# insight-platform/Similari

Hardware: NVIDIA H100
Metric: pair_associations_per_sec (higher is better)
Workload: dtype f32

## Files before the change

### similari_b200/csrc/engine.cu

```cuda
#include <cuda_runtime.h>

#include <algorithm>
#include <array>
#include <chrono>
#include <cmath>
#include <cstddef>
#include <cstdlib>
#include <cstdio>
#include <cstring>
#include <map>
#include <string>
#include <type_traits>
#include <unordered_map>
#include <utility>
#include <vector>

#include "../../include/similari_b200.h"
#include "sb_blob.cuh"
#include "sb_engine.cuh"
#include "sb_host.cuh"
#include "sb_wstore.cuh"

#include <atomic>

namespace sb {
static std::atomic<unsigned long long> g_launches{0};
void note_launch(int n) { g_launches.fetch_add((unsigned long long)n, std::memory_order_relaxed); }
unsigned long long launch_count() { return g_launches.load(std::memory_order_relaxed); }
}

using sb::DBuf;
using sb::HBuf;
using sb::fail;

namespace {

enum ColRows { kRowTrack, kRowBlock, kRowFree, kRowWasted, kRowHistTop, kRowHistFree, kRowTrackHist };
enum ColBlob { kBlobNo, kBlobAll, kBlobTrackerOnly };
enum ColTag { kTagNone, kTagFblk, kTagHblk, kTagObsN, kTagObsPhys, kTagOwner, kTagFree };
struct Col {
  DBuf* buf;
  void (*point)(sb200_tracker&, void*);
  size_t w;
  bool zero = false;
  int rows = kRowTrack;
  int blob = kBlobAll;
  int tag = kTagNone;
};

int make_params(const sb200_options& o, sb::Params* out) {
  sb::Params p;
  memset(&p, 0, sizeof(p));
  if (o.kind < 0 || o.kind > 3) return fail(SB200_ERR_INVALID, "unknown tracker kind %d", o.kind);
  if (o.positional_kind != SB200_POS_MAHA && o.positional_kind != SB200_POS_IOU)
    return fail(SB200_ERR_INVALID, "unknown positional metric %d", o.positional_kind);
  p.kind = o.kind;
  p.positional_kind = o.positional_kind;
  p.visual_kind = o.visual_kind;
  p.iou_threshold = o.iou_threshold;
  p.min_confidence = o.min_confidence;
  p.pos_weight = o.kalman_position_weight;
  p.vel_weight = o.kalman_velocity_weight;
  p.max_idle_epochs = o.max_idle_epochs;
  if (o.max_idle_epochs < 0) return fail(SB200_ERR_INVALID, "max_idle_epochs must be >= 0");
  if (o.n_constraints < 0 || o.n_constraints > SB200_MAX_CONSTRAINTS)
    return fail(SB200_ERR_INVALID, "at most %d spatio-temporal constraints", SB200_MAX_CONSTRAINTS);
  std::vector<std::pair<int, float>> c;
  for (int i = 0; i < o.n_constraints; ++i) {
    if (!(o.constraint_max_dist[i] > 0.0f))
      return fail(SB200_ERR_INVALID, "The distance is expected to be a positive float");
    c.emplace_back(o.constraint_epochs[i], o.constraint_max_dist[i]);
  }
  std::stable_sort(c.begin(), c.end(), [](const std::pair<int, float>& a, const std::pair<int, float>& b) { return a.first < b.first; });
  c.erase(std::unique(c.begin(), c.end(), [](const std::pair<int, float>& a, const std::pair<int, float>& b) { return a.first == b.first; }), c.end());
  p.n_constraints = (int)c.size();
  for (size_t i = 0; i < c.size(); ++i) { p.constraint_epochs[i] = c[i].first; p.constraint_max_dist[i] = c[i].second; }
  p.is_visual = o.kind == SB200_KIND_VISUAL_SORT || o.kind == SB200_KIND_BATCH_VISUAL_SORT;
  p.is_batch = o.kind == SB200_KIND_BATCH_SORT || o.kind == SB200_KIND_BATCH_VISUAL_SORT;
  if (p.is_visual) {
    if (o.visual_kind != SB200_VIS_EUCLIDEAN && o.visual_kind != SB200_VIS_COSINE)
      return fail(SB200_ERR_INVALID, "unknown visual metric %d", o.visual_kind);
    if (o.feature_dim <= 0) return fail(SB200_ERR_INVALID, "feature_dim must be > 0 for visual trackers");
    if (o.visual_max_observations < 1 || o.visual_max_observations > sb::kMaxObsWide)
      return fail(SB200_ERR_CAPACITY, "visual_max_observations must be in [1, %d]", sb::kMaxObsWide);
    p.visual_threshold = o.visual_threshold;
    p.feature_dim = o.feature_dim;
    p.d8 = (o.feature_dim + 7) / 8 * 8;
    p.vis_rel_err = sb::screen_rel_err(o.feature_dim);
    p.vis_rel_err8 = sb::screen_rel_err_fp8(o.feature_dim);
    p.max_obs = o.visual_max_observations;
    p.min_votes = o.visual_min_votes;
    p.min_track_length = o.visual_minimal_track_length;
    p.min_area = o.visual_minimal_area;
    p.min_quality_use = o.visual_minimal_quality_use;
    p.min_quality_collect = o.visual_minimal_quality_collect;
    p.min_own_use = o.visual_minimal_own_area_percentage_use;
    p.min_own_collect = o.visual_minimal_own_area_percentage_collect;
    p.use_own_area = (o.visual_minimal_own_area_percentage_collect + o.visual_minimal_own_area_percentage_use) > 0.0f;
  } else {
    p.max_obs = 1;
    p.d8 = 8;
  }
  *out = p;
  return 0;
}

}

struct sb200_tracker {
  sb200_options opts{};
  sb::Params P{};
  int device = 0;
  cudaStream_t stream = nullptr;
  cudaStream_t user_stream = nullptr;
  bool has_user_stream = false;
  bool join_per_call = true;
  cudaEvent_t ev_join_req = nullptr;
  cudaEvent_t ev_user_in = nullptr, ev_user_out = nullptr;
  cudaStream_t prep_stream = nullptr;
  cudaEvent_t ev_prep_done = nullptr, ev_set_free[2]{}, ev_inputs = nullptr;
  cudaEvent_t ev_cost_done = nullptr;
  bool cost_done_valid = false;
  bool set_busy[2]{};
  unsigned long long frame_seq = 0;
  float kernel_ms[2]{};
  bool tc_timed = false;
  cudaStream_t copy_stream = nullptr;
  static constexpr int kDepth = 3;
  struct FrameBack {
    sb::FrameDyn dyn;
    int dense_scenes;
    int hpool[2];
    int screen[3];
  };
  static_assert(offsetof(FrameBack, dense_scenes) == sizeof(sb::FrameDyn) && sizeof(FrameBack) == sizeof(sb::FrameDyn) + 24,
                "FrameBack: FrameDyn followed by the counters, without padding");
  static size_t back_offset(int n_scenes) { return ((size_t)n_scenes * 16 + 15) / 16 * 16; }
  struct Pending {
    bool active = false;
    int n_scenes = 0, total = 0;
    std::vector<int> slots, m;
    long long live_ub = 0;
    HBuf h_req;
    HBuf h_out;
    FrameBack* back() const { return reinterpret_cast<FrameBack*>(h_out.as<char>() + back_offset(n_scenes)); }
    cudaEvent_t done = nullptr;
    cudaEvent_t ev[6]{}, ev_k[3]{}, ev_pos[2]{};
    bool tc_timed = false, pos_forked = false;
    int mode = 0;
    bool fp8 = false;
  } pend[kDepth];
  int pend_head = 0, pend_count = 0;
  std::vector<int> pending_add;
  long long inflight_live_ub = 0;
  int async_rc = 0;
  std::string async_err;
  unsigned long long acc_units_mn = 0, acc_units_rows = 0, acc_frames = 0;
  double host_ms_total = 0.0, host_ms_blocked = 0.0;
  unsigned long long host_calls = 0;
  double acc_stage_ms[5]{}, acc_kernel_ms[2]{};
  unsigned long long acc_tc_frames = 0;
  static constexpr int kFp8Hold = 64;
  int fp8_hold = 0;
  unsigned long long acc_screen[4] = {0, 0, 0, 0};
  cudaStream_t side_stream = nullptr;
  cudaEvent_t ev_fork[2]{}, ev_join = nullptr;
  float stage_ms[5]{};
  std::unordered_map<uint64_t, int> slot_of;
  std::vector<uint64_t> scene_of_slot;
  std::vector<uint32_t> epoch;
  std::vector<int> n_tracks;
  std::vector<int> n_hidden;
  std::vector<int> arena_top;
  std::vector<uint64_t> last_req_scenes;
  std::vector<int> last_req_slots;
  int64_t revealed = 0;
  int scene_cap = 0, track_cap = 0;
  DBuf b_idc;
  int auto_waste_counter = 100, auto_waste_periodicity = 100;
  int64_t wasted_count = 0;
  sb::TrackStore ts{};
  DBuf b_id, b_epoch, b_length, b_custom, b_vt, b_pred, b_obs, b_radius, b_kst, b_vert, b_hpred, b_hobs, b_feat, b_feat_bf16, b_fnorm2, b_obs_phys,
      b_feat_fp8, b_fscale, b_obs_hasf, b_obs_q, b_obs_n, b_feat_cnt, b_fblk, b_blk_owner, b_blk_free;
  DBuf b_ntracks, b_cur_epoch, b_scene_ids, b_nfree, b_atop;
  sb::WastedBuf wb{};
  DBuf w_count, w_id, w_scene, w_epoch, w_length, w_pred, w_obs, w_hpred, w_hobs;
  int hist_len = 1;
  bool fhist_on = false;
  DBuf b_hblk, b_hrows, b_hpresent, b_hfree, b_hpool, w_hblk, f_histdst;
  long long hpool_cap = 0;
  long long hpool_top = 0;
  long long hpool_free = 0;
  long long hpool_pend = 0;
  enum InColumn { kBoxes, kFeat, kHasf, kQuality, kCustom, kOwn, kInCols };
  using InPtrs = std::array<const void*, kInCols>;
  InPtrs in_ptrs(const void* boxes, const void* feat, const void* hasf, const void* quality, const void* custom,
                 const void* own) const {
    if (!P.is_visual) return {boxes, nullptr, nullptr, nullptr, custom, nullptr};
    return {boxes, feat, feat ? hasf : nullptr, quality, custom, own};
  }
  template <auto F> static void to_frame(sb::Frame& f, const void* p) { f.*F = static_cast<std::remove_reference_t<decltype(f.*F)>>(const_cast<void*>(p)); }
  struct InCol { void (*bind)(sb::Frame&, const void*); size_t w; const char* name; };
  std::array<InCol, kInCols> in_cols() const {
    using F = sb::Frame;
    return {{{to_frame<&F::in_boxes>, 24, "S.boxes"}, {to_frame<&F::in_feat>, (size_t)P.feature_dim * feat_bytes(), "S.feat"},
             {to_frame<&F::in_hasf>, 1, "S.hasf"}, {to_frame<&F::in_quality>, 4, "S.quality"},
             {to_frame<&F::in_custom>, 8, "S.custom"}, {to_frame<&F::in_own>, 4, "S.own"}}};
  }
  static constexpr int kOutCols = 6;
  struct OutCol { void* host; void (*bind)(sb::Frame&, const void*); size_t w; const char* name; };
  static std::array<OutCol, kOutCols> out_cols(const sb200_predict_out& o) {
    using F = sb::Frame;
    return {{{o.ids, to_frame<&F::o_ids>, 8, "o_ids"}, {o.epochs, to_frame<&F::o_epochs>, 4, "o_epochs"},
             {o.lengths, to_frame<&F::o_lengths>, 4, "o_lengths"}, {o.voting_types, to_frame<&F::o_vt>, 1, "o_vt"},
             {o.predicted_boxes, to_frame<&F::o_pred>, 24, "o_pred"}, {o.observed_boxes, to_frame<&F::o_obs>, 24, "o_obs"}}};
  }
  long long hint_dets(int n_scenes) const { return (long long)std::max(opts.max_scenes_hint, n_scenes) * opts.max_dets_per_scene_hint; }
  size_t frame_rows(int total, int n_scenes) const { return (size_t)std::max<long long>(std::max(total, 1), hint_dets(n_scenes)); }
  int hint_tracks() const { return opts.max_tracks_per_scene_hint > 0 ? track_cap : 0; }
  struct Staging {
    DBuf col[kInCols];
    InPtrs key{};
    int total = -1;
    int type = sb::kFeatF32;
    bool pending = false;
    cudaEvent_t ev = nullptr;
    cudaEvent_t ev0 = nullptr;
    cudaEvent_t ev_read = nullptr;
    bool read_pending = false;
  } stg[2];
  int stg_last = 1;
  struct CandBufs { DBuf box, radius, conf, vert, flags, norm2, bf16, decided, fp8, scale; } cand[2];
  DBuf f_winner, f_cvt, f_pos, f_vis, f_scenes, f_newcount,
      f_status, f_featdst, f_apprank, f_appmeta, f_frameout, f_excl, f_prewin, f_own, f_ownovf, f_dyn, f_ws, f_tmeta, f_rowinfo, f_slabc, f_slabm, f_slabmask,
      f_dscene, f_maxc, f_maxcval, f_drowb, f_dcolb, f_slabk, f_scene_max, f_tiles, f_pairs, f_colmeta, f_colgeo, f_colb, f_colvalid, f_rowmeta, f_poslist, f_counters, f_visval, f_colsb;
  int num_sms = 132;
  DBuf o_col[kOutCols];
  HBuf h_small;
  bool adapt_dense = false;
  unsigned long long acc_dense_scenes = 0;
  int last_dense_scenes = 0;
  bool seen_features = false;
  int feat_type = sb::kFeatF32;
  size_t feat_bytes() const { return feat_type == sb::kFeatF32 ? 4 : 2; }
  bool transferred = false;
  int last_n_scenes = 0;

  ~sb200_tracker() {
    cudaSetDevice(device);
    for (cudaStream_t s : {stream, prep_stream, side_stream, copy_stream}) if (s) cudaStreamSynchronize(s);
    for (auto& g : stg)
      for (cudaEvent_t e : {g.ev, g.ev0, g.ev_read}) if (e) cudaEventDestroy(e);
    for (auto& q : pend) {
      if (q.done) cudaEventDestroy(q.done);
      for (auto& e : q.ev) if (e) cudaEventDestroy(e);
      for (auto& e : q.ev_k) if (e) cudaEventDestroy(e);
      for (auto& e : q.ev_pos) if (e) cudaEventDestroy(e);
    }
    if (copy_stream) cudaStreamDestroy(copy_stream);
    if (side_stream) cudaStreamDestroy(side_stream);
    if (prep_stream) cudaStreamDestroy(prep_stream);
    for (cudaEvent_t e : {ev_user_in, ev_user_out, ev_prep_done, ev_set_free[0], ev_set_free[1], ev_inputs, ev_join_req, ev_cost_done}) if (e) cudaEventDestroy(e);
    for (auto& e : ev_fork) if (e) cudaEventDestroy(e);
    if (ev_join) cudaEventDestroy(ev_join);
    if (stream) cudaStreamDestroy(stream);
  }

  template <auto F> static void in_ts(sb200_tracker& t, void* p) { t.ts.*F = static_cast<std::remove_reference_t<decltype(t.ts.*F)>>(p); }
  template <auto F> static void in_wb(sb200_tracker& t, void* p) { t.wb.*F = static_cast<std::remove_reference_t<decltype(t.wb.*F)>>(p); }

  std::vector<Col> store_table() {
    using TS = sb::TrackStore;
    const size_t K = (size_t)P.max_obs, d8 = (size_t)P.d8, H = (size_t)hist_len;
    std::vector<Col> c = {{&b_id, in_ts<&TS::id>, 8}, {&b_epoch, in_ts<&TS::epoch>, 4}, {&b_length, in_ts<&TS::length>, 4},
                          {&b_custom, in_ts<&TS::custom>, 8}, {&b_vt, in_ts<&TS::vt>, 1}, {&b_pred, in_ts<&TS::pred>, 24},
                          {&b_obs, in_ts<&TS::obs>, 24}, {&b_radius, in_ts<&TS::radius>, 4},
                          {&b_kst, in_ts<&TS::kst>, 4 * (size_t)sb::kStateStride}};
    if (P.positional_kind == SB200_POS_IOU) c.push_back({&b_vert, in_ts<&TS::vert>, 64});
    if (H > 1) {
      c.push_back({&b_hpred, in_ts<&TS::hist_pred>, 24 * H, true});
      c.push_back({&b_hobs, in_ts<&TS::hist_obs>, 24 * H, true});
    }
    if (P.is_visual) {
      c.push_back({&b_obs_phys, in_ts<&TS::obs_phys>, K, false, kRowTrack, kBlobAll, kTagObsPhys});
      c.push_back({&b_obs_hasf, in_ts<&TS::obs_hasf>, K});
      c.push_back({&b_obs_q, in_ts<&TS::obs_q>, 4 * K});
      c.push_back({&b_obs_n, in_ts<&TS::obs_n>, 1, false, kRowTrack, kBlobAll, kTagObsN});
      c.push_back({&b_feat_cnt, in_ts<&TS::feat_cnt>, 1});
      c.push_back({&b_fblk, in_ts<&TS::fblk>, 4, false, kRowTrack, kBlobAll, kTagFblk});
      if (fhist_on) c.push_back({&b_hblk, in_ts<&TS::hblk>, 4, false, kRowTrack, kBlobTrackerOnly, kTagHblk});
      c.push_back({&b_feat, in_ts<&TS::feat>, 4 * K * d8, true, kRowBlock});
      c.push_back({&b_feat_bf16, in_ts<&TS::feat_bf16>, 2 * K * d8, true, kRowBlock});
      c.push_back({&b_fnorm2, in_ts<&TS::fnorm2>, 4 * K, false, kRowBlock});
      if (P.d8 <= sb::kFp8MaxD8) {
        c.push_back({&b_feat_fp8, in_ts<&TS::feat_fp8>, K * sb::fp8_pitch(P.d8), false, kRowBlock, kBlobNo});
        c.push_back({&b_fscale, in_ts<&TS::fscale>, 4 * K, false, kRowBlock, kBlobNo});
      }
      c.push_back({&b_blk_owner, in_ts<&TS::blk_owner>, 4, false, kRowBlock, kBlobAll, kTagOwner});
      c.push_back({&b_blk_free, in_ts<&TS::blk_free>, 4, false, kRowFree, kBlobAll, kTagFree});
    }
    return c;
  }

  std::vector<Col> slot_table() {
    using TS = sb::TrackStore;
    return {{&b_ntracks, nullptr, 4, true}, {&b_cur_epoch, nullptr, 4, true}, {&b_scene_ids, nullptr, 8, true},
            {&b_nfree, in_ts<&TS::n_free>, 4, true}, {&b_atop, in_ts<&TS::arena_top>, 4, true}};
  }

  std::vector<Col> wasted_table() {
    using WB = sb::WastedBuf;
    const size_t H = (size_t)hist_len;
    std::vector<Col> c = {{&w_id, in_wb<&WB::id>, 8, false, kRowWasted}, {&w_scene, in_wb<&WB::scene>, 8, false, kRowWasted},
                          {&w_epoch, in_wb<&WB::epoch>, 4, false, kRowWasted}, {&w_length, in_wb<&WB::length>, 4, false, kRowWasted},
                          {&w_pred, in_wb<&WB::pred>, 24, false, kRowWasted}, {&w_obs, in_wb<&WB::obs>, 24, false, kRowWasted}};
    if (H > 1) {
      c.push_back({&w_hpred, in_wb<&WB::hist_pred>, 24 * H, false, kRowWasted});
      c.push_back({&w_hobs, in_wb<&WB::hist_obs>, 24 * H, false, kRowWasted});
    }
    if (fhist_on) c.push_back({&w_hblk, in_wb<&WB::hblk>, 4, false, kRowWasted, kBlobAll, kTagHblk});
    return c;
  }

  std::vector<Col> pool_table() {
    using TS = sb::TrackStore;
    const size_t H = (size_t)hist_len;
    return {{&b_hrows, in_ts<&TS::hrows>, H * (size_t)P.d8 * 4, false, kRowHistTop},
            {&b_hpresent, in_ts<&TS::hpresent>, H, true, kRowHistTop},
            {&b_hfree, in_ts<&TS::hfree>, 4, false, kRowHistFree, kBlobAll, kTagHblk}};
  }

  int regrow(DBuf& b, size_t w, size_t groups, size_t rows, size_t old_groups, size_t old_rows, bool zero) {
    const size_t bytes = std::max<size_t>(1, groups * rows * w);
    DBuf nb;
    int rc = nb.ensure(bytes);
    if (rc) return rc;
    if (zero) CU(cudaMemsetAsync(nb.p, 0, bytes, stream));
    if (b.p && old_groups > 0 && old_rows > 0) {
      if (old_groups == 1)
        CU(cudaMemcpyAsync(nb.p, b.p, old_rows * w, cudaMemcpyDeviceToDevice, stream));
      else
        CU(cudaMemcpy2DAsync(nb.p, rows * w, b.p, old_rows * w, old_rows * w, old_groups, cudaMemcpyDeviceToDevice, stream));
      CU(cudaStreamSynchronize(stream));
    }
    b = std::move(nb);
    return 0;
  }

  int grow(const std::vector<Col>& cols, size_t groups, size_t rows, size_t old_groups, size_t old_rows) {
    for (const Col& c : cols) {
      const int rc = regrow(*c.buf, c.w, groups, rows, old_groups, old_rows, c.zero || c.blob != kBlobNo);
      if (rc) return rc;
      if (c.point) c.point(*this, c.buf->p);
    }
    return 0;
  }

  int regen_fp8(int slot, int top) {
    if (!ts.feat_fp8 || top <= 0) return 0;
    const long long r0 = (long long)slot * track_cap * P.max_obs, rows = (long long)top * P.max_obs;
    sb::launch_to_fp8(ts.feat + r0 * P.d8, P.d8, P.d8, P.d8, rows, ts.feat_fp8 + r0 * sb::fp8_pitch(P.d8), ts.fscale + r0, stream);
    return cudaGetLastError() == cudaSuccess ? 0 : fail(SB200_ERR_CUDA, "e4m3 row conversion failed");
  }

  static constexpr long long kBf16LogCap = 1 << 18;
  DBuf b_bf16log;
  long long bf16_log_n = 0;
  bool bf16_stale_all = false;
  int regen_bf16() {
    if (bf16_stale_all) sb::launch_bf16_regen(ts, P.d8, P.max_obs, nullptr, 0, scene_cap, stream);
    else if (bf16_log_n > 0) sb::launch_bf16_regen(ts, P.d8, P.max_obs, b_bf16log.as<int>(), bf16_log_n, 0, stream);
    else return 0;
    bf16_log_n = 0;
    bf16_stale_all = false;
    return cudaGetLastError() == cudaSuccess ? 0 : fail(SB200_ERR_CUDA, "BF16 row conversion failed");
  }

  int ensure_store(int need_scenes, int need_tracks) {
    if (need_scenes <= scene_cap && need_tracks <= track_cap) return 0;
    int ns = scene_cap, nt = track_cap;
    if (need_scenes > ns) ns = std::max(need_scenes, std::max(4, ns * 2));
    if (need_tracks > nt) nt = std::max(need_tracks, std::max(64, nt * 2));
    int rc = regen_bf16();
    if (rc) return rc;
    rc = grow(store_table(), ns, nt, scene_cap, track_cap);
    if (rc) return rc;
    if (ns != scene_cap && (rc = grow(slot_table(), ns, 1, scene_cap, 1))) return rc;
    ts.kst_stride = sb::kStateStride;
    if (hist_len > 1) ts.hist_len = hist_len;
    scene_cap = ns;
    track_cap = nt;
    ts.track_cap = nt;
    return 0;
  }

  int slot_for(uint64_t scene_id, bool create) {
    auto it = slot_of.find(scene_id);
    if (it != slot_of.end()) return it->second;
    if (!create) return -1;
    int s = (int)scene_of_slot.size();
    slot_of[scene_id] = s;
    scene_of_slot.push_back(scene_id);
    epoch.push_back(0);
    n_tracks.push_back(0);
    n_hidden.push_back(0);
    arena_top.push_back(0);
    pending_add.push_back(0);
    return s;
  }

  int ensure_wasted(int64_t need) {
    if (need <= wb.cap) return 0;
    int64_t ncap = std::max<int64_t>(need, std::max<int64_t>(1024, (int64_t)wb.cap * 3));
    int rc = grow(wasted_table(), 1, (size_t)ncap, 1, (size_t)wasted_count);
    if (rc) return rc;
    if (!w_count.p) {
      if ((rc = w_count.ensure(sizeof(int)))) return rc;
      CU(cudaMemsetAsync(w_count.p, 0, sizeof(int), stream));
    }
    wb.cap = (int)ncap;
    wb.count = w_count.as<int>();
    return 0;
  }

  int run_waste() {
    int n_slots = (int)scene_of_slot.size();
    if (n_slots == 0) return 0;
    int64_t active = 0;
    int max_n = 0;
    for (int v : n_tracks) { active += v; max_n = std::max(max_n, v); }
    if (active == 0) {
      revealed = wasted_count;
      std::fill(n_hidden.begin(), n_hidden.end(), 0);
      return 0;
    }
    int rc = ensure_wasted(wasted_count + active);
    if (rc) return rc;
    if ((rc = h_small.ensure((size_t)n_slots * 16))) return rc;
    unsigned int* he = h_small.as<unsigned int>();
    for (int s = 0; s < n_slots; ++s) he[s] = epoch[s];
    CU(cudaMemcpyAsync(b_cur_epoch.p, he, sizeof(unsigned int) * n_slots, cudaMemcpyHostToDevice, stream));
    CU(cudaStreamSynchronize(stream));
    unsigned long long* hs = h_small.as<unsigned long long>();
    for (int s = 0; s < n_slots; ++s) hs[s] = scene_of_slot[s];
    CU(cudaMemcpyAsync(b_scene_ids.p, hs, sizeof(unsigned long long) * n_slots, cudaMemcpyHostToDevice, stream));
    sb::launch_waste(P, ts, n_slots, b_cur_epoch.as<unsigned int>(), b_scene_ids.as<unsigned long long>(),
                     b_ntracks.as<int>(), wb, max_n, stream);
    CU(cudaGetLastError());
    int* hn = h_small.as<int>();
    CU(cudaStreamSynchronize(stream));
    CU(cudaMemcpyAsync(hn, b_ntracks.p, sizeof(int) * n_slots, cudaMemcpyDeviceToHost, stream));
    int hc = 0;
    CU(cudaMemcpyAsync(&hc, w_count.p, sizeof(int), cudaMemcpyDeviceToHost, stream));
    CU(cudaStreamSynchronize(stream));
    for (int s = 0; s < n_slots; ++s) n_tracks[s] = hn[s];
    wasted_count = hc;
    revealed = wasted_count;
    std::fill(n_hidden.begin(), n_hidden.end(), 0);
    return 0;
  }

  int drop_wasted_front(int64_t n) {
    if (n <= 0 || !w_count.p) return 0;
    n = std::min(n, wasted_count);
    const int64_t rest = wasted_count - n;
    cudaStream_t st = stream;
    int rc = 0;
    if (fhist_on) {
// ... 33 lines not shown
    int rc = grow(pool_table(), 1, (size_t)ncap, 1, (size_t)hpool_top);
    if (rc) return rc;
    hpool_cap = ncap;
    return 0;
  }

  int set_feature_history(bool on) {
    if (on == fhist_on) return 0;
    CU(cudaSetDevice(device));
    CU(cudaStreamSynchronize(stream));
    fhist_on = true;
    const int rc = on ? add_feature_history() : 0;
    if (on && rc == 0) return 0;
    std::vector<Col> cols = pool_table();
    for (const Col& c : store_table()) if (c.tag == kTagHblk) cols.push_back(c);
    for (const Col& c : wasted_table()) if (c.tag == kTagHblk) cols.push_back(c);
    for (const Col& c : cols) { c.buf->release(); c.point(*this, nullptr); }
    b_hpool.release();
    f_histdst.release();
    ts.hpool = nullptr;
    ts.fhist_len = 0;
    fhist_on = false;
    hpool_cap = hpool_top = hpool_free = hpool_pend = 0;
    return rc;
  }
  int add_feature_history() {
    int rc;
    if ((rc = b_hpool.ensure(2 * sizeof(int)))) return rc;
    CU(cudaMemsetAsync(b_hpool.p, 0, 2 * sizeof(int), stream));
    for (const Col& c : store_table())
      if (c.tag == kTagHblk && scene_cap > 0 && (rc = grow({c}, scene_cap, track_cap, 0, 0))) return rc;
    for (const Col& c : wasted_table())
      if (c.tag == kTagHblk && wb.cap > 0 && (rc = grow({c}, 1, wb.cap, 0, 0))) return rc;
    CU(cudaStreamSynchronize(stream));
    ts.hpool = b_hpool.as<int>();
    ts.fhist_len = hist_len;
    return 0;
  }

  int predict(int32_t n_scenes, const uint64_t* scene_ids, const int32_t* det_offsets, const float* boxes,
              const float* features, const uint8_t* has_feature, const float* quality, const int64_t* custom_ids,
              const float* own_area, const sb200_predict_out* out, bool device_io, bool wait);
  int absorb_oldest(bool block);
  int poll();
  int drain(const char* why = nullptr);
  int ens(DBuf& b, size_t need, const char* name = "") {
    if (need <= b.bytes) return 0;
    static const bool trace_ens = getenv("SB200_TRACE") != nullptr;
    if (trace_ens) fprintf(stderr, "[sb200] %s grows: %zu -> %zu bytes\n", name, b.bytes, need);
    int rc = drain("frame buffer grows");
    if (rc) return rc;
    return b.ensure(need);
  }
  template <class T> int ens(DBuf& b, size_t need, T*& to, const char* name) {
    const int rc = ens(b, need, name);
    if (rc == 0) to = static_cast<T*>(b.p);
    return rc;
  }
  static constexpr int kDenseVoteCap = 8192;

  struct Request {
    int n_scenes = 0, total = 0;
    const uint64_t* scene_ids = nullptr;
    const int32_t* det_offsets = nullptr;
    InPtrs in{};
    sb200_predict_out out{};
    bool device_io = false, same_req = false;
  };
  struct FramePlan {
    std::vector<int> m_of, nb_ub;
    int max_m = 0, max_n = 0, max_nb = 0, need_tracks = 0;
    long long live_ub = 0, pos_total = 0, vis_total = 0, col_total = 0, work = 0;
    long long pos_ub = 0, posl_total = 0, visl_total = 0;
    size_t T = 0;
    int cset = 0, vote_cap = 0, mstep = 0, cstep = 256;
    bool want_tc = false, want_dense = false, want_fp8 = false;
    Staging* sin = nullptr;
    bool prefetched = false, fork = false, derive_own = false;
  };
  void unbook(Pending& q) {
    for (int s = 0; s < q.n_scenes; ++s) pending_add[q.slots[s]] -= q.m[s];
    inflight_live_ub -= q.live_ub;
    if (fhist_on) hpool_pend -= q.total;
    q.active = false;
    pend_count -= 1;
  }
  struct Rollback { sb200_tracker* t; Pending* q; bool armed; ~Rollback() { if (armed) t->unbook(*q); } };
  int check_request(Request& rq) {
    const int n_scenes = rq.n_scenes;
    const uint64_t* scene_ids = rq.scene_ids;
    const int32_t* det_offsets = rq.det_offsets;
    if (n_scenes < 0) return fail(SB200_ERR_INVALID, "n_scenes must be >= 0");
    if (n_scenes > 0 && (!scene_ids || !det_offsets)) return fail(SB200_ERR_INVALID, "scene_ids / det_offsets are NULL");
    rq.total = n_scenes > 0 ? det_offsets[n_scenes] : 0;
    if (n_scenes > 0 && det_offsets[0] != 0) return fail(SB200_ERR_INVALID, "det_offsets[0] must be 0");
    for (int s = 0; s < n_scenes; ++s)
      if (det_offsets[s + 1] < det_offsets[s]) return fail(SB200_ERR_INVALID, "det_offsets must be non-decreasing");
    if (rq.total > 0 && !rq.in[kBoxes]) return fail(SB200_ERR_INVALID, "boxes is NULL");
    int rc = 0;
    poll();
    if (async_rc) { if ((rc = drain("error of an earlier frame"))) return rc; }
    rq.same_req = (int)last_req_scenes.size() == n_scenes && n_scenes > 0 &&
                memcmp(last_req_scenes.data(), scene_ids, sizeof(uint64_t) * (size_t)n_scenes) == 0;
    if (!rq.same_req && n_scenes > 0) {
      std::unordered_map<uint64_t, int> seen;
      for (int s = 0; s < n_scenes; ++s)
        if (!seen.emplace(scene_ids[s], s).second) return fail(SB200_ERR_INVALID, "scene %llu appears twice in one request", (unsigned long long)scene_ids[s]);
    }
    int max_m0 = 0, max_n0 = 0;
    auto fits = [&] {
      max_m0 = max_n0 = 0;
      for (int s = 0; s < n_scenes; ++s) {
        int slot = -1;
        if (rq.same_req) slot = last_req_slots[s];
        else { auto it = slot_of.find(scene_ids[s]); if (it != slot_of.end()) slot = it->second; }
        max_m0 = std::max(max_m0, det_offsets[s + 1] - det_offsets[s]);
        max_n0 = std::max(max_n0, slot >= 0 ? n_tracks[slot] + pending_add[slot] : 0);
      }
      return sb::voting_smem_need(max_m0, max_n0, P.is_visual ? kDenseVoteCap : 0) <= sb::kVotingSmemLimit;
    };
    bool ok = fits();
    if (!ok && pend_count > 0) { if ((rc = drain("assignment solver bound"))) return rc; ok = fits(); }
    if (!ok) return fail(SB200_ERR_CAPACITY, "scene too large for the on-chip assignment solver (m=%d, n=%d)", max_m0, max_n0);
    return 0;
  }

  void bounds(const Request& rq, FramePlan& pl) const {
    const int n_scenes = rq.n_scenes, K = P.max_obs;
    pl.m_of.resize(n_scenes);
    pl.nb_ub.resize(n_scenes);
    pl.max_m = pl.max_n = pl.max_nb = pl.need_tracks = 0;
    pl.live_ub = pl.pos_total = pl.vis_total = pl.col_total = pl.work = 0;
    for (int s = 0; s < n_scenes; ++s) {
      const int slot = last_req_slots[s];
      const int m = rq.det_offsets[s + 1] - rq.det_offsets[s];
      const int n = n_tracks[slot] + pending_add[slot];
      pl.m_of[s] = m;
      pl.nb_ub[s] = P.is_visual ? arena_top[slot] + pending_add[slot] : 0;
      pl.live_ub += n;
      pl.pos_total += (long long)m * n;
      if (P.is_visual) pl.vis_total += (long long)m * n * K;
      pl.col_total += ((long long)pl.nb_ub[s] * K + 127) / 128 * 128;
      pl.work += (long long)m * n * K;
      pl.max_m = std::max(pl.max_m, m);
      pl.max_n = std::max(pl.max_n, n);
      pl.max_nb = std::max(pl.max_nb, pl.nb_ub[s]);
      pl.need_tracks = std::max(pl.need_tracks, n + m);
    }
  }

  int reserve_state(const Request& rq, FramePlan& pl) {
    const int n_scenes = rq.n_scenes, total = rq.total;
    int rc = 0;
    bounds(rq, pl);
    const int pipe_room = kDepth * std::max(pl.max_m, opts.max_dets_per_scene_hint);
    int hint_s = std::max((int)scene_of_slot.size(), opts.max_scenes_hint);
    if (hint_s > scene_cap || pl.need_tracks > track_cap) {
      if ((rc = drain("track store bound"))) return rc;
      bounds(rq, pl);
      const int want_t = std::max(pl.need_tracks, opts.max_tracks_per_scene_hint) + pipe_room;
      if (hint_s > scene_cap || pl.need_tracks > track_cap)
        if ((rc = ensure_store(hint_s, std::max(want_t, track_cap + track_cap / 2)))) return rc;
    }
    if (wasted_count + inflight_live_ub + pl.live_ub + 1 > wb.cap) {
      const long long pipe_need = inflight_live_ub + pl.live_ub;
      if ((rc = drain("wasted buffer bound"))) return rc;
      bounds(rq, pl);
      const long long dets = std::max<long long>(total, hint_dets(n_scenes));
      const long long ring_need = (long long)(kDepth + 1) * (pl.live_ub + (long long)kDepth * dets);
      const long long rec_bytes = 72 + (hist_len > 1 ? 48ll * hist_len : 0);
      const long long base_need = std::max<long long>(ring_need, 2 * pipe_need);
      const long long mult = std::max<long long>(1, std::min<long long>(8, (2ll << 30) / std::max<long long>(1, base_need * rec_bytes)));
      if ((rc = ensure_wasted(2 * wasted_count + mult * base_need + 1))) return rc;
    }
    if (fhist_on && total > 0 && hpool_top + std::max<long long>(0, hpool_pend + total - hpool_free) > hpool_cap) {
      const long long frames = pend_count + 1;
      if ((rc = drain("feature history pool bound"))) return rc;
      const long long want = hpool_top + std::max<long long>(0, frames * total - hpool_free);
      if (want > hpool_cap && (rc = ensure_hpool(std::max<long long>(want, hpool_cap + hpool_cap / 2)))) return rc;
    }
    if (!b_idc.p) {
      if ((rc = b_idc.ensure(8))) return rc;
      CU(cudaMemsetAsync(b_idc.p, 0, 8, stream));
    }
    return 0;
  }

  int plan_frame(const Request& rq, Pending& q, FramePlan& pl) {
    const int n_scenes = rq.n_scenes, total = rq.total, K = P.max_obs;
    int rc = 0;
    if ((rc = q.h_req.ensure(sizeof(sb::SceneReq) * (size_t)n_scenes)) ||
        (rc = q.h_out.ensure(back_offset(n_scenes) + sizeof(FrameBack))))
      return rc;
    if (P.is_visual && rq.in[kFeat] != nullptr && total > 0) {
      const sb::VisKernel vk = sb::vis_kernel_env();
      const bool selective = sb::vis_selective(P.visual_kind == SB200_VIS_EUCLIDEAN, P.visual_threshold);
      const bool big = sb::vis_tc_worth(P.d8, pl.work);
      const bool dense_ok = P.n_constraints == 0;
      pl.want_dense = big && dense_ok && (!selective || adapt_dense);
      pl.want_tc = selective && big && !pl.want_dense;
      if (vk == sb::kVisSimt) { pl.want_tc = false; pl.want_dense = false; }
      else if (vk == sb::kVisTc || vk == sb::kVisTc8 || vk == sb::kVisTc16) { pl.want_tc = pl.work > 0; pl.want_dense = false; }
      else if (vk == sb::kVisDense) { pl.want_dense = pl.work > 0 && dense_ok; pl.want_tc = pl.work > 0 && !pl.want_dense; }
      const bool can8 = pl.want_tc && P.d8 <= sb::kFp8MaxD8 && ts.feat_fp8 != nullptr;
      const bool forced = vk == sb::kVisTc8 || vk == sb::kVisTc16;
      pl.want_fp8 = can8 && (forced ? vk == sb::kVisTc8 : fp8_hold == 0);
      if (!forced && can8 && fp8_hold > 0) fp8_hold -= 1;
    }
    pl.vote_cap = pl.want_dense ? kDenseVoteCap : sb::kVoteVisCap;
    sb::SceneReq* hreq = q.h_req.as<sb::SceneReq>();
    for (int s = 0; s < n_scenes; ++s) {
      sb::SceneReq& r = hreq[s];
      r.slot = last_req_slots[s];
      r.m = pl.m_of[s];
      r.det_base = rq.det_offsets[s];
      r.epoch = epoch[r.slot] + 1;
      r.scene_id = rq.scene_ids[s];
      r.pos_lbase = (int)pl.posl_total;
      r.pos_lcap = sb::pos_lcap(r.m);
      pl.posl_total += r.pos_lcap;
      r.vis_lbase = (int)pl.visl_total;
      r.vis_lcap = P.is_visual ? sb::vis_lcap(r.m, pl.vote_cap) : 0;
      pl.visl_total += r.vis_lcap;
    }
    pl.T = frame_rows(total, n_scenes);
    pl.pos_ub = pl.pos_total;
    const long long hint_pos = hint_dets(n_scenes) * hint_tracks();
    pl.pos_total = std::max(pl.pos_total, hint_pos);
    if (P.is_visual) pl.vis_total = std::max(pl.vis_total, hint_pos * K);
    pl.cset = (int)(frame_seq & 1);
    if (!pl.want_tc && !pl.want_dense) return 0;
    pl.mstep = 256;
    pl.cstep = pl.want_dense ? (256 / K) * K : sb::vis_screen_ucols(P.d8, num_sms, n_scenes, pl.m_of.data(), pl.nb_ub.data(), K);
    return 0;
  }

#define ENS(b, ...) ens(b, __VA_ARGS__, #b)
  int bind_frame(const Request& rq, FramePlan& pl, sb::Frame& f, sb::TcArgs& tc) {
    const int n_scenes = rq.n_scenes, total = rq.total, K = P.max_obs;
    const size_t T = pl.T;
    CandBufs& cb = cand[pl.cset];
    int rc = 0;
    if ((rc = ENS(cb.box, T * 24, f.c_box)) || (rc = ENS(cb.radius, T * 4, f.c_radius)) || (rc = ENS(cb.conf, T * 4, f.c_conf)) ||
        (rc = ENS(f_winner, T * 4, f.winner)) || (rc = ENS(f_cvt, T, f.c_vt)) ||
        (rc = ENS(f_scenes, sizeof(sb::SceneDesc) * n_scenes, f.scenes)) || (rc = ENS(f_newcount, 4 * (size_t)n_scenes, f.new_count)) ||
        (rc = ENS(f_dyn, sizeof(sb::FrameDyn), f.dyn)) || (rc = ENS(f_apprank, T * 8, f.app_rank)) ||
        (rc = ENS(f_appmeta, 16 * (size_t)n_scenes, f.app_meta)) || (rc = ENS(f_pos, std::max<size_t>(4, (size_t)pl.pos_total * 4), f.pos)))
      return rc;
    if (P.positional_kind == SB200_POS_IOU && (rc = ENS(cb.vert, T * 64, f.c_vert))) return rc;
    if (P.is_visual) {
      if (fhist_on && (rc = ENS(f_histdst, T * 4, f.hist_dst))) return rc;
      if ((rc = ENS(cb.flags, T, f.c_flags)) || (rc = ENS(cb.norm2, T * 4, f.c_norm2)) || (rc = ENS(f_featdst, T * 4, f.feat_dst)) ||
          (rc = ENS(f_vis, std::max<size_t>(4, (size_t)pl.vis_total * 4), f.vis)) ||
          (rc = ENS(f_scene_max, 4 * (size_t)n_scenes, f.scene_max)))
        return rc;
    }
    tc.num_sms = num_sms;
    const int hint_tr = hint_tracks();
    const long long hs = std::max(opts.max_scenes_hint, n_scenes), visl_alloc = std::max(pl.visl_total, hint_dets(n_scenes) * 64);
    if (pl.want_tc || pl.want_dense) {
      tc.use_tc = true;
      tc.dense = pl.want_dense;
// ... 13 lines not shown
      const bool alloc8 = !pl.want_dense && P.d8 <= sb::kFp8MaxD8 && ts.feat_fp8 != nullptr;
      if (alloc8 && ((rc = ENS(cb.fp8, T * sb::fp8_pitch(P.d8))) || (rc = ENS(cb.scale, T * 4)) || (rc = ENS(b_bf16log, kBf16LogCap * 4))))
        return rc;
      if ((rc = ENS(cb.bf16, T * P.d8 * 2)) ||
          (rc = ENS(f_tiles, sizeof(sb::TcTile) * (size_t)std::max<long long>(1, tiles_alloc), tc.d_tiles)) ||
          (rc = ENS(f_rowmeta, sizeof(sb::VisRowMeta) * (T + 256), tc.rowmeta)))
        return rc;
      tc.max_rows = pl.max_nb * K;
      tc.d_n_tiles = &f_dyn.as<sb::FrameDyn>()->n_tiles;
      tc.a_rows = total;
      tc.b_rows = (long long)scene_cap * track_cap * K;
      if (!tc.dense) {
        const size_t cols = (size_t)std::max(pl.col_total, hs * (((long long)hint_tr * K + 127) / 128 * 128));
        if ((rc = ENS(f_colmeta, sizeof(sb::VisColMeta) * (cols + 256), tc.colmeta)) || (rc = ENS(f_colb, 4 * (cols + 256), tc.colb)) ||
            (rc = ENS(f_colvalid, (cols + 256) / 8 + 16, tc.colvalid)) ||
            (rc = ENS(f_colgeo, sizeof(sb::VisColGeo) * std::max<size_t>(1, P.n_constraints > 0 ? cols : 1), tc.colgeo)))
          return rc;
        tc.total_cols = (int)pl.col_total;
        if (alloc8 && P.visual_kind != SB200_VIS_COSINE) {
          if ((rc = ENS(f_colsb, 4 * (cols + 256)))) return rc;
          if (pl.want_fp8) tc.colsb = f_colsb.as<float>();
        }
        tc.fp8 = pl.want_fp8;
      } else {
        const long long hd0 = std::max(opts.max_dets_per_scene_hint, 0);
        ws_ub = std::max(ws_ub, hs * (hint_tr + 256) * ((hd0 + 127) / 128 * 128));
        blk_ub = std::max(blk_ub, hs * (hint_tr + 256));
        slabs_ub = std::max(slabs_ub, hs * (((long long)hint_tr * K + cstep - 1) / cstep + 1));
        const size_t slabs = (size_t)std::max<long long>(1, slabs_ub), blks = (size_t)std::max<long long>(1, blk_ub);
        const size_t visl = (size_t)std::max<long long>(1, visl_alloc);
        if ((rc = ENS(f_drowb, 4 * 5 * T, tc.d_rowb)) || (rc = ENS(f_dcolb, 4 * blks, tc.d_colb)) ||
            (rc = ENS(f_slabk, 4 * 256 * slabs, tc.slab_ktf)) || (rc = ENS(f_ws, 4 * (size_t)std::max<long long>(1, ws_ub), tc.ws)) ||
            (rc = ENS(f_tmeta, sizeof(sb::DenseTrackMeta) * blks, tc.tmeta)) ||
            (rc = ENS(f_rowinfo, 8 * (size_t)std::max<long long>(1, blk_ub * K), tc.rowinfo)) ||
            (rc = ENS(f_slabc, 4 * 256 * slabs, tc.slab_colc)) || (rc = ENS(f_slabm, 4 * 256 * slabs, tc.slab_cmax)) ||
            (rc = ENS(f_slabmask, 2 * 32 * slabs, tc.slab_vmask)) || (rc = ENS(f_dscene, dscene_bytes(n_scenes))) ||
            (rc = ENS(f_maxc, sizeof(sb::VisPair) * visl, tc.maxc)) || (rc = ENS(f_maxcval, 4 * visl, tc.maxc_val)))
          return rc;
        tc.max_blocks = pl.max_nb;
        tc.n_slabs_ub = (int)slabs_ub;
        tc.blk_ub = blk_ub;
        tc.slab_bmask = tc.slab_vmask + (size_t)slabs_ub * 8;
        carve_dscene(f_dscene.p, n_scenes, tc);
      }
    }
    f.total = total;
    f.pos_total = pl.pos_ub;
    f.id_counter = b_idc.as<unsigned long long>();
    f.id_add = P.is_batch ? (long long)total : -1;
    f.dense_bad = tc.dense ? tc.dense_bad : nullptr;
    f.pos_dense_all = getenv("SB200_FULL_COSTS") != nullptr;
    f.feat_type = feat_type;
    const std::array<InCol, kInCols> ic = in_cols();
    if (rq.device_io) {
      for (int c = 0; c < kInCols; ++c) ic[c].bind(f, rq.in[c]);
    } else {
      int use = -1;
      for (int k = 0; k < 2; ++k)
        if (stg[k].pending && stg[k].total == total && stg[k].type == feat_type && stg[k].key == rq.in)
          use = k;
      if (use >= 0) {
        pl.prefetched = true;
        stg[use].pending = false;
        CU(cudaStreamWaitEvent(stream, stg[use].ev, 0));
      } else {
        use = stg[0].pending ? 1 : (stg[1].pending ? 0 : 1 - stg_last);
        stg[use].pending = false;
      }
      stg_last = use;
      Staging& S = stg[use];
      pl.sin = &S;
      for (int c = 0; c < kInCols; ++c) {
        if (c != kBoxes && !(rq.in[c] && total > 0)) continue;
        if (S.col[c].bytes < T * ic[c].w) pl.prefetched = false;
        if ((rc = ens(S.col[c], T * ic[c].w, ic[c].name))) return rc;
        ic[c].bind(f, S.col[c].p);
      }
    }
    f.new_count_all = f.new_count;
    if ((rc = ENS(f_frameout, sizeof(int) * 3 * (size_t)n_scenes, f.frame_out))) return rc;
    f.c_bf16 = tc.use_tc && !tc.fp8 ? cb.bf16.p : nullptr;
    f.c_fp8 = tc.fp8 ? cb.fp8.as<unsigned char>() : nullptr;
    f.c_scale = tc.fp8 ? cb.scale.as<float>() : nullptr;
    if ((rc = ENS(f_poslist, sizeof(sb::PosEntry) * (size_t)std::max<long long>(1, std::max(pl.posl_total, hint_dets(n_scenes) * 32)), f.pos_list)) ||
        (rc = ENS(f_counters, sizeof(int) * sb::counter_ints(n_scenes))))
      return rc;
    if (P.is_visual && ((rc = ENS(f_pairs, sizeof(sb::VisPair) * (size_t)std::max<long long>(1, visl_alloc), f.vis_pairs)) ||
                        (rc = ENS(f_visval, sizeof(float) * (size_t)std::max<long long>(1, visl_alloc), f.vis_val))))
      return rc;
    sb::carve_counters(f_counters.as<int>(), n_scenes, f);
    if (!tc.use_tc || tc.dense) f.screen_cnt = nullptr;
    const std::array<OutCol, kOutCols> oc = out_cols(rq.out);
    for (int c = 0; c < kOutCols; ++c) {
      if (!oc[c].host) continue;
      if (rq.device_io) { oc[c].bind(f, oc[c].host); continue; }
      if ((rc = ens(o_col[c], T * oc[c].w, oc[c].name))) return rc;
      oc[c].bind(f, o_col[c].p);
    }
    pl.fork = P.is_visual && tc.use_tc && tc.n_tiles > 0 && !f.pos_dense_all;
    if (pl.fork && ((rc = ENS(cb.decided, T, f.decided)) || (rc = ENS(f_excl, (size_t)scene_cap * track_cap + 16, f.excl)) ||
                    (rc = ENS(f_prewin, T * 4, f.pre_winner))))
      return rc;
    pl.derive_own = P.is_visual && P.use_own_area && f.in_own == nullptr && total > 0;
    if (pl.derive_own && ((rc = ENS(f_own, T * 4)) || (rc = ENS(f_ownovf, 16 + T * sizeof(int2))))) return rc;
    return 0;
  }
#undef ENS

  Rollback commit(const Request& rq, const FramePlan& pl, Pending& q) {
    const int n_scenes = rq.n_scenes;
    for (int s = 0; s < n_scenes; ++s) epoch[last_req_slots[s]] += 1;
    if (rq.in[kFeat] != nullptr && rq.total > 0) seen_features = true;
    frame_seq += 1;
    q.active = true;
    q.n_scenes = n_scenes;
    q.total = rq.total;
    q.slots.assign(last_req_slots.begin(), last_req_slots.end());
    q.m = pl.m_of;
    q.live_ub = pl.live_ub;
    q.tc_timed = false;
    q.pos_forked = false;
    q.mode = pl.want_dense ? 2 : (pl.want_tc ? 1 : 0);
    q.fp8 = pl.want_fp8;
    for (int s = 0; s < n_scenes; ++s) pending_add[last_req_slots[s]] += pl.m_of[s];
    inflight_live_ub += pl.live_ub;
    if (fhist_on) hpool_pend += rq.total;
    pend_count += 1;
    last_n_scenes = n_scenes;
    return Rollback{this, &q, true};
  }

  int enqueue(const Request& rq, const FramePlan& pl, Pending& q, sb::Frame& f, sb::TcArgs& tc) {
    const int n_scenes = rq.n_scenes, total = rq.total, max_m = pl.max_m, max_n = pl.max_n, cset = pl.cset;
    sb::Params Pf = P;
    Pf.vote_vis_cap = pl.vote_cap;
    if (has_user_stream) {
      CU(cudaEventRecord(ev_user_in, user_stream));
      CU(cudaStreamWaitEvent(stream, ev_user_in, 0));
    }
    if (!rq.device_io && !pl.prefetched && total > 0) {
      const std::array<InCol, kInCols> ic = in_cols();
      for (int c = 0; c < kInCols; ++c)
        if (rq.in[c]) CU(cudaMemcpyAsync(pl.sin->col[c].p, rq.in[c], (size_t)total * ic[c].w, cudaMemcpyHostToDevice, stream));
    }
    if (q.fp8 && f.in_feat) {
      f.skip_bf16 = true;
      if (!bf16_stale_all && bf16_log_n + total <= kBf16LogCap) {
        f.bf16_log = b_bf16log.as<int>() + bf16_log_n;
        bf16_log_n += total;
      } else {
        bf16_stale_all = true;
      }
    } else if (tc.use_tc && !tc.fp8) {
      if (const int rc = regen_bf16()) return rc;
    }
    const bool prep_ahead = !pl.derive_own && total > 0;
    const bool side_setup = !pl.derive_own && total > 0;
    cudaStream_t s_setup = stream;
    if (side_setup) {
      CU(cudaEventRecord(ev_fork[0], stream));
      CU(cudaStreamWaitEvent(side_stream, ev_fork[0], 0));
      s_setup = side_stream;
    }
    sb::launch_frame_setup(P, ts, f, reinterpret_cast<const sb::SceneReq*>(q.h_req.dp), n_scenes, b_ntracks.as<int>(), pl.mstep,
                           pl.cstep, tc.dense, f_tiles.as<sb::TcTile>(), f_dyn.as<sb::FrameDyn>(), f_counters.as<int>(),
                           (int)sb::counter_ints(n_scenes), s_setup);
    tc.max_init_done = 1;
    if (side_setup && Pf.is_visual && tc.use_tc && !tc.dense && tc.n_tiles > 0 && max_m > 0 && max_n > 0 && f.in_feat) {
      sb::launch_vis_colmeta(Pf, ts, f, n_scenes, max_n, tc, side_stream);
      tc.colmeta_done = 1;
    }
    if (side_setup) CU(cudaEventRecord(ev_join, side_stream));
    CU(cudaEventRecord(q.ev[0], stream));
    if (pl.derive_own) {
      sb::launch_own_area(f, n_scenes, max_m, f.in_boxes, f_own.as<float>(), f_ownovf.as<int>(),
                          reinterpret_cast<int2*>(f_ownovf.as<char>() + 16), stream);
      f.in_own = f_own.as<float>();
    }
    if (prep_ahead) {
      if (has_user_stream) CU(cudaStreamWaitEvent(prep_stream, ev_user_in, 0));
      if (!rq.device_io) {
        if (pl.prefetched) CU(cudaStreamWaitEvent(prep_stream, pl.sin->ev, 0));
        else { CU(cudaEventRecord(ev_inputs, stream)); CU(cudaStreamWaitEvent(prep_stream, ev_inputs, 0)); }
      }
      if (set_busy[cset]) CU(cudaStreamWaitEvent(prep_stream, ev_set_free[cset], 0));
      if (cost_done_valid) CU(cudaStreamWaitEvent(prep_stream, ev_cost_done, 0));
      sb::launch_prep(Pf, f, n_scenes, max_m, prep_stream);
      CU(cudaEventRecord(ev_prep_done, prep_stream));
      CU(cudaStreamWaitEvent(stream, ev_prep_done, 0));
    } else {
      sb::launch_prep(Pf, f, n_scenes, max_m, stream);
    }
    if (side_setup) CU(cudaStreamWaitEvent(stream, ev_join, 0));
    CU(cudaEventRecord(q.ev[1], stream));
    sb::TcArgs tcc = tc;
    if (tc.use_tc && tc.n_tiles > 0) { tcc.ev_screen0 = q.ev_k[0]; tcc.ev_screen1 = q.ev_k[1]; tcc.ev_refine1 = q.ev_k[2]; q.tc_timed = true; }
    if (!pl.fork) {
      sb::launch_pos_cost(Pf, ts, f, n_scenes, max_m, max_n, stream);
      CU(cudaEventRecord(q.ev[2], stream));
      int vr0 = sb::launch_vis_cost(Pf, ts, f, n_scenes, max_m, max_n, tcc, stream);
      if (vr0 != 0) return fail(SB200_ERR_CUDA, "visual cost launch failed (%d)", vr0);
      if (!f.pos_dense_all) sb::launch_pos_scan_lazy(Pf, ts, f, n_scenes, max_m, max_n, 1, stream);
    } else {
      CU(cudaEventRecord(q.ev[2], stream));
      {
        int vr0 = sb::launch_vis_cost_a(Pf, ts, f, n_scenes, max_m, max_n, tcc, stream);
        if (vr0 != 0) return fail(SB200_ERR_CUDA, "visual cost launch failed (%d)", vr0);
        vr0 = sb::launch_vote_masks(Pf, ts, f, n_scenes, max_m, max_n, stream);
        if (vr0 != 0) return fail(SB200_ERR_CUDA, "voting launch failed: %s", cudaGetErrorString((cudaError_t)vr0));
      }
      CU(cudaEventRecord(q.ev_pos[0], stream));
      sb::launch_pos_scan_lazy(Pf, ts, f, n_scenes, max_m, max_n, 0, stream);
      CU(cudaEventRecord(q.ev_pos[1], stream));
      int vr1 = sb::launch_vis_cost_b(Pf, ts, f, n_scenes, max_m, max_n, tcc, stream);
      if (vr1 != 0) return fail(SB200_ERR_CUDA, "visual cost launch failed (%d)", vr1);
      sb::launch_pos_scan_lazy(Pf, ts, f, n_scenes, max_m, max_n, 1, stream);
      q.pos_forked = true;
    }
    CU(cudaEventRecord(q.ev[3], stream));
    CU(cudaEventRecord(ev_cost_done, stream));
    cost_done_valid = true;
    int vr = sb::launch_voting(Pf, ts, f, n_scenes, max_m, max_n, stream);
    if (vr != 0) return fail(SB200_ERR_CUDA, "voting launch failed: %s", cudaGetErrorString((cudaError_t)vr));
    CU(cudaEventRecord(q.ev[4], stream));
    sb::launch_apply(Pf, ts, f, n_scenes, max_m, 0ull, b_ntracks.as<int>(), stream);
    const bool side_sweep = Pf.is_visual && f.in_feat && total > 0;
    if (side_sweep) {
      CU(cudaEventRecord(ev_fork[1], stream));
      CU(cudaStreamWaitEvent(side_stream, ev_fork[1], 0));
      sb::launch_frame_sweep(Pf, ts, f, n_scenes, b_ntracks.as<int>(), wb, side_stream);
      CU(cudaEventRecord(ev_join, side_stream));
      sb::launch_feat_store(Pf, ts, f, stream);
      CU(cudaStreamWaitEvent(stream, ev_join, 0));
    } else {
      sb::launch_feat_store(Pf, ts, f, stream);
      sb::launch_frame_sweep(Pf, ts, f, n_scenes, b_ntracks.as<int>(), wb, stream);
    }
    CU(cudaEventRecord(q.ev[5], stream));
    CU(cudaGetLastError());

    if (!rq.device_io && total > 0) {
      const std::array<OutCol, kOutCols> oc = out_cols(rq.out);
      for (int c = 0; c < kOutCols; ++c)
        if (oc[c].host) CU(cudaMemcpyAsync(oc[c].host, o_col[c].p, (size_t)total * oc[c].w, cudaMemcpyDeviceToHost, stream));
    }
    FrameBack* back = q.back();
    sb::Frame cnt{};
    sb::carve_counters(f_counters.as<int>(), n_scenes, cnt);
    CU(cudaMemcpyAsync(q.h_out.p, f.frame_out, 12 * (size_t)n_scenes, cudaMemcpyDeviceToHost, stream));
    CU(cudaMemcpyAsync(q.h_out.as<char>() + 12 * (size_t)n_scenes, cnt.status, 4 * (size_t)n_scenes, cudaMemcpyDeviceToHost, stream));
    CU(cudaMemcpyAsync(&back->dyn, f_dyn.p, sizeof(back->dyn), cudaMemcpyDeviceToHost, stream));
    CU(cudaMemcpyAsync(&back->dense_scenes, cnt.dense_cnt, sizeof(back->dense_scenes), cudaMemcpyDeviceToHost, stream));
    if (fhist_on) CU(cudaMemcpyAsync(back->hpool, ts.hpool, sizeof(back->hpool), cudaMemcpyDeviceToHost, stream));
    CU(cudaMemcpyAsync(back->screen, cnt.screen_cnt, sizeof(back->screen), cudaMemcpyDeviceToHost, stream));
    static const bool trace_dense = getenv("SB200_TRACE") != nullptr && atoi(getenv("SB200_TRACE")) >= 2;
    if (trace_dense && tc.dense && tc.n_tiles > 0) {
      int hc[8] = {0};
      CU(cudaMemcpyAsync(hc, tc.dbg_counts, sizeof(hc), cudaMemcpyDeviceToHost, stream));
      CU(cudaStreamSynchronize(stream));
      std::vector<int> vcnt((size_t)n_scenes);
      CU(cudaMemcpy(vcnt.data(), f.vis_cnt, 4 * (size_t)n_scenes, cudaMemcpyDeviceToHost));
      long long tot = 0; int mx = 0;
      for (int v : vcnt) { tot += v; mx = std::max(mx, v); }
      fprintf(stderr, "[sb200] dense frame: fallback reasons threshold %d, max-list overflow %d, no maximum %d; max candidates %d; pairs to refine %lld (largest scene %d)\n",
              hc[0], hc[1], hc[2], hc[3], tot, mx);
    }
    CU(cudaEventRecord(q.done, stream));
    CU(cudaEventRecord(ev_set_free[cset], stream));
    set_busy[cset] = true;
    if (has_user_stream && join_per_call) {
      CU(cudaEventRecord(ev_user_out, stream));
      CU(cudaStreamWaitEvent(user_stream, ev_user_out, 0));
    }
    return 0;
  }

  static size_t dscene_bytes(int n) { return 4 * 6 * (size_t)n + 128; }
  static void carve_dscene(void* p, int n, sb::TcArgs& tc) {
    using A = sb::TcArgs;
    int* A::* const ints[] = {&A::maxc_cnt, &A::maxc_next, &A::dense_bad, &A::zeros};
    for (int i = 0; i < 4; ++i) tc.*ints[i] = static_cast<int*>(p) + (size_t)i * n;
    tc.scene_l0 = reinterpret_cast<float*>(tc.maxc_cnt + 4 * (size_t)n);
    tc.scene_cmax = tc.scene_l0 + n;
    tc.dbg_counts = reinterpret_cast<int*>(tc.scene_cmax + n) + 4;
  }
};

int sb200_tracker::absorb_oldest(bool block) {
  if (pend_count == 0) return 1;
  Pending& q = pend[pend_head];
  cudaError_t e;
  if (block) {
    const auto w0 = std::chrono::steady_clock::now();
    e = cudaEventSynchronize(q.done);
    host_ms_blocked += std::chrono::duration<double, std::milli>(std::chrono::steady_clock::now() - w0).count();
  } else {
    e = cudaEventQuery(q.done);
  }
  if (e == cudaErrorNotReady) { cudaGetLastError(); return 1; }
  const int n = q.n_scenes;
  if (e != cudaSuccess) {
    cudaGetLastError();
    if (!async_rc) { async_rc = SB200_ERR_CUDA; async_err = std::string("a frame in flight failed: ") + cudaGetErrorString(e); }
  } else {
    const int* h_fo = q.h_out.as<int>();
    const int* h_status = h_fo + 3 * (size_t)n;
    const FrameBack& back = *q.back();
    for (int s = 0; s < n; ++s) {
      const int slot = q.slots[s];
      if (h_status[s] && !async_rc) {
        async_rc = (h_status[s] & 2) ? SB200_ERR_CAPACITY : SB200_ERR_INTERNAL;
        char buf[160];
        snprintf(buf, sizeof(buf), (h_status[s] & 2) ? "more than 2800 boxes overlap one detection of scene %llu (own-area shares)"
                                                      : "track store overflow in scene %llu",
                 (unsigned long long)scene_of_slot[slot]);
        async_err = buf;
      }
      n_tracks[slot] = h_fo[3 * s];
      arena_top[slot] = h_fo[3 * s + 1];
      n_hidden[slot] += h_fo[3 * s + 2];
      wasted_count += h_fo[3 * s + 2];
    }
    if (fhist_on) {
      hpool_free = back.hpool[0];
      hpool_top = back.hpool[1];
    }
    acc_units_mn += back.dyn.units_mn;
    acc_units_rows += back.dyn.units_rows;
    acc_frames += 1;
    {
      const int dense_scenes = back.dense_scenes;
      if (q.mode != 0) acc_dense_scenes += (unsigned long long)dense_scenes;
      last_dense_scenes = dense_scenes;
      if (q.mode == 1 && !q.fp8 && n >= 1 && dense_scenes * 4 > n) adapt_dense = true;
      if (q.mode == 2 && n >= 1 && dense_scenes * 4 > n) adapt_dense = false;
      if (q.mode == 1) {
        const unsigned long long kept = (unsigned int)back.screen[0], cut = (unsigned int)back.screen[1],
                                 ovf = (unsigned int)back.screen[2];
        acc_screen[q.fp8 ? 0 : 1] += 1;
        acc_screen[2] += kept;
        acc_screen[3] += cut;
        if (q.fp8 && (ovf > 0 || 2 * cut > kept)) fp8_hold = kFp8Hold;
      }
    }
    for (int i = 0; i < 5; ++i) cudaEventElapsedTime(&stage_ms[i], q.ev[i], q.ev[i + 1]);
    if (q.pos_forked) {
      float fill_ms = stage_ms[1], scan_ms = 0.0f;
      cudaEventElapsedTime(&scan_ms, q.ev_pos[0], q.ev_pos[1]);
      stage_ms[1] = scan_ms;
      stage_ms[2] += fill_ms - scan_ms;
    }
    tc_timed = q.tc_timed;
    kernel_ms[0] = kernel_ms[1] = 0.0f;
    if (tc_timed) { cudaEventElapsedTime(&kernel_ms[0], q.ev_k[0], q.ev_k[1]); cudaEventElapsedTime(&kernel_ms[1], q.ev_k[1], q.ev_k[2]); }
    for (int i = 0; i < 5; ++i) acc_stage_ms[i] += stage_ms[i];
    if (tc_timed) { acc_kernel_ms[0] += kernel_ms[0]; acc_kernel_ms[1] += kernel_ms[1]; acc_tc_frames += 1; }
    static const bool trace_abs = getenv("SB200_TRACE") != nullptr;
    if (trace_abs)
      fprintf(stderr, "[sb200] frame absorbed: mode %d, %d of %d scenes on the exact SIMT fallback; prep %.3f pos %.3f vis %.3f vote %.3f apply %.3f ms (main kernel %.3f, refine %.3f)\n",
              q.mode, last_dense_scenes, n, stage_ms[0], stage_ms[1], stage_ms[2], stage_ms[3], stage_ms[4], kernel_ms[0], kernel_ms[1]);
    cudaGetLastError();
  }
  unbook(q);
  pend_head = (pend_head + 1) % kDepth;
  return 0;
}

int sb200_tracker::poll() {
  while (pend_count > 0 && absorb_oldest(false) == 0) {}
  return 0;
}

int sb200_tracker::drain(const char* why) {
  static const bool trace_dr = getenv("SB200_TRACE") != nullptr;
  if (trace_dr && why && pend_count > 0) fprintf(stderr, "[sb200] predict waits for %d frame(s) in flight: %s\n", pend_count, why);
  while (pend_count > 0) absorb_oldest(true);
  if (async_rc) {
    const int rc = async_rc;
    async_rc = 0;
    return fail(rc, "%s", async_err.c_str());
  }
  return 0;
}

int sb200_tracker::predict(int32_t n_scenes, const uint64_t* scene_ids, const int32_t* det_offsets, const float* boxes,
                           const float* features, const uint8_t* has_feature, const float* quality,
                           const int64_t* custom_ids, const float* own_area, const sb200_predict_out* out,
                           bool device_io, bool wait) {
  CU(cudaSetDevice(device));
  static const bool trace = getenv("SB200_TRACE") != nullptr;
  const auto t_begin = std::chrono::steady_clock::now();
  auto since = [&] { return std::chrono::duration<double, std::milli>(std::chrono::steady_clock::now() - t_begin).count(); };
  Request rq{n_scenes, 0, scene_ids, det_offsets, in_ptrs(boxes, features, has_feature, quality, custom_ids, own_area),
             out ? *out : sb200_predict_out{}, device_io};
  int rc = check_request(rq);
  if (rc) return rc;
  if (auto_waste_counter == 0) {
    if ((rc = drain("auto-waste tick"))) return rc;
    if ((rc = run_waste())) return rc;
    auto_waste_counter = auto_waste_periodicity;
  } else auto_waste_counter -= 1;
  if (n_scenes == 0) return wait ? drain() : 0;

  if (!rq.same_req) {
    last_req_slots.resize(n_scenes);
// ... 77 lines not shown
  cudaError_t e = cudaStreamCreateWithPriority(&t->stream, cudaStreamNonBlocking, prio_hi < prio_lo ? prio_hi + 1 : prio_lo);
  if (e != cudaSuccess) { delete t; return fail(SB200_ERR_CUDA, "cudaStreamCreate failed: %s", cudaGetErrorString(e)); }
  for (auto& g : t->stg) {
    e = cudaEventCreate(&g.ev);
    if (e == cudaSuccess) e = cudaEventCreate(&g.ev0);
    if (e == cudaSuccess) e = cudaEventCreateWithFlags(&g.ev_read, cudaEventDisableTiming);
    if (e != cudaSuccess) { delete t; return fail(SB200_ERR_CUDA, "cudaEventCreate failed: %s", cudaGetErrorString(e)); }
  }
  e = cudaStreamCreateWithPriority(&t->side_stream, cudaStreamNonBlocking, prio_hi);
  if (e == cudaSuccess) e = cudaStreamCreateWithPriority(&t->prep_stream, cudaStreamNonBlocking, prio_lo);
  for (cudaEvent_t* p : {&t->ev_fork[0], &t->ev_fork[1], &t->ev_join, &t->ev_prep_done, &t->ev_inputs, &t->ev_cost_done,
                         &t->ev_set_free[0], &t->ev_set_free[1], &t->ev_user_in, &t->ev_user_out})
    if (e == cudaSuccess) e = cudaEventCreateWithFlags(p, cudaEventDisableTiming);
  for (auto& q : t->pend) {
    if (e == cudaSuccess) e = cudaEventCreateWithFlags(&q.done, cudaEventDisableTiming);
    for (auto& x : q.ev) if (e == cudaSuccess) e = cudaEventCreate(&x);
    for (auto& x : q.ev_k) if (e == cudaSuccess) e = cudaEventCreate(&x);
    for (auto& x : q.ev_pos) if (e == cudaSuccess) e = cudaEventCreate(&x);
  }
  if (e != cudaSuccess) { delete t; return fail(SB200_ERR_CUDA, "stream / event creation failed: %s", cudaGetErrorString(e)); }
  if (opts->max_scenes_hint > 0 || opts->max_tracks_per_scene_hint > 0) {
    rc = t->ensure_store(std::max(1, opts->max_scenes_hint),
                         std::max(64, opts->max_tracks_per_scene_hint + sb200_tracker::kDepth * std::max(0, opts->max_dets_per_scene_hint)));
    if (rc) { delete t; return rc; }
  }
  *out = t;
  return 0;
}

void sb200_tracker_destroy(sb200_tracker* t) { delete t; }

int sb200_tracker_set_stream(sb200_tracker* t, void* cuda_stream) {
  if (!t) return fail(SB200_ERR_INVALID, "tracker is NULL");
  CU(cudaSetDevice(t->device));
  int rc = t->drain();
  if (rc) return rc;
  CU(cudaStreamSynchronize(t->stream));
  t->user_stream = reinterpret_cast<cudaStream_t>(cuda_stream);
  t->has_user_stream = true;
  return 0;
}

int sb200_set_stream_join(sb200_tracker* t, int32_t per_call) {
  if (!t) return fail(SB200_ERR_INVALID, "tracker is NULL");
  t->join_per_call = per_call != 0;
  return 0;
}

int sb200_stream_join(sb200_tracker* t, void* cuda_stream) {
  if (!t) return fail(SB200_ERR_INVALID, "tracker is NULL");
  CU(cudaSetDevice(t->device));
  if (!t->ev_join_req) CU(cudaEventCreateWithFlags(&t->ev_join_req, cudaEventDisableTiming));
  CU(cudaEventRecord(t->ev_join_req, t->stream));
  CU(cudaStreamWaitEvent(reinterpret_cast<cudaStream_t>(cuda_stream), t->ev_join_req, 0));
  return 0;
}

int sb200_predict_batch(sb200_tracker* t, int32_t n_scenes, const uint64_t* scene_ids, const int32_t* det_offsets,
                        const float* boxes, const float* features, const uint8_t* has_feature, const float* quality,
                        const int64_t* custom_ids, const float* own_area, const sb200_predict_out* out) {
  if (!t) return fail(SB200_ERR_INVALID, "tracker is NULL");
  return t->predict(n_scenes, scene_ids, det_offsets, boxes, features, has_feature, quality, custom_ids, own_area, out, false, true);
}

int sb200_predict_batch_async(sb200_tracker* t, int32_t n_scenes, const uint64_t* scene_ids, const int32_t* det_offsets,
                              const float* boxes, const float* features, const uint8_t* has_feature, const float* quality,
                              const int64_t* custom_ids, const float* own_area, const sb200_predict_out* out) {
  if (!t) return fail(SB200_ERR_INVALID, "tracker is NULL");
  return t->predict(n_scenes, scene_ids, det_offsets, boxes, features, has_feature, quality, custom_ids, own_area, out, false, false);
}

int sb200_set_feature_dim(sb200_tracker* t, int32_t feature_dim) {
  if (!t || feature_dim <= 0) return fail(SB200_ERR_INVALID, "bad arguments");
  if (!t->P.is_visual) return fail(SB200_ERR_INVALID, "not a visual tracker");
  if (feature_dim == t->P.feature_dim) return 0;
  if (t->seen_features) return fail(SB200_ERR_INVALID, "features of dimension %d are already stored", t->P.feature_dim);
  CU(cudaSetDevice(t->device));
  int rc = t->drain();
  if (rc) return rc;
  CU(cudaStreamSynchronize(t->stream));
  auto d8_cols = [t] {
    std::vector<std::pair<Col, size_t>> v;
    for (const Col& c : t->store_table())
      if (c.buf == &t->b_feat || c.buf == &t->b_feat_bf16 || c.buf == &t->b_feat_fp8 || c.buf == &t->b_fscale)
        v.push_back({c, (size_t)t->scene_cap * t->track_cap});
    if (t->fhist_on)
      for (const Col& c : t->pool_table()) if (c.buf == &t->b_hrows) v.push_back({c, (size_t)t->hpool_cap});
    return v;
  };
  for (const auto& [c, rows] : d8_cols()) { c.buf->release(); c.point(*t, nullptr); }
  for (auto& cb : t->cand) { cb.bf16.release(); cb.fp8.release(); }
  t->P.feature_dim = feature_dim;
  t->P.d8 = (feature_dim + 7) / 8 * 8;
  t->P.vis_rel_err = sb::screen_rel_err(feature_dim);
  t->P.vis_rel_err8 = sb::screen_rel_err_fp8(feature_dim);
  t->opts.feature_dim = feature_dim;
  for (const auto& [c, rows] : d8_cols()) {
    if (rows == 0) continue;
    if ((rc = c.buf->ensure(rows * c.w))) return rc;
    c.point(*t, c.buf->p);
  }
  for (auto& g : t->stg) g.col[sb200_tracker::kFeat].release();
  return 0;
}

int sb200_feature_history_pool(sb200_tracker* t, int64_t* out3) {
  if (!t || !out3) return fail(SB200_ERR_INVALID, "bad arguments");
  if (!t->fhist_on) return fail(SB200_ERR_INVALID, "the feature history is off (sb200_set_feature_history)");
  CU(cudaSetDevice(t->device));
  { int rc_ = t->drain(); if (rc_) return rc_; }
  int h[2] = {0, 0};
  CU(cudaMemcpyAsync(h, t->ts.hpool, sizeof(h), cudaMemcpyDeviceToHost, t->stream));
  CU(cudaStreamSynchronize(t->stream));
  out3[0] = t->hpool_cap;
  out3[1] = h[1];
  out3[2] = h[0];
  return 0;
}

int sb200_set_feature_history(sb200_tracker* t, int32_t on) {
  if (!t) return fail(SB200_ERR_INVALID, "tracker is NULL");
  if (!t->P.is_visual) return fail(SB200_ERR_INVALID, "the feature history belongs to the visual trackers");
  if (t->frame_seq > 0 || t->transferred)
    return fail(SB200_ERR_INVALID, "the feature history is switched before the first predict, load or import");
  return t->set_feature_history(on != 0);
}

static_assert(SB200_FEATURE_F32 == sb::kFeatF32 && SB200_FEATURE_F16 == sb::kFeatF16 && SB200_FEATURE_BF16 == sb::kFeatBF16,
              "feature type codes of the ABI and the kernels differ");

int sb200_set_feature_type(sb200_tracker* t, int32_t type) {
  if (!t) return fail(SB200_ERR_INVALID, "tracker is NULL");
  if (!t->P.is_visual) return fail(SB200_ERR_INVALID, "the feature type belongs to the visual trackers");
  if (type != SB200_FEATURE_F32 && type != SB200_FEATURE_F16 && type != SB200_FEATURE_BF16)
    return fail(SB200_ERR_INVALID, "unknown feature type %d", (int)type);
  t->feat_type = type;
  return 0;
}

int sb200_sync(sb200_tracker* t) {
  if (!t) return fail(SB200_ERR_INVALID, "tracker is NULL");
  CU(cudaSetDevice(t->device));
  return t->drain();
}

int sb200_frames_in_flight(sb200_tracker* t) {
  if (!t) return fail(SB200_ERR_INVALID, "tracker is NULL");
  CU(cudaSetDevice(t->device));
  t->poll();
  return t->pend_count;
}

int sb200_work_counters(sb200_tracker* t, uint64_t* out3 , double* ms7 ) {
  if (!t) return fail(SB200_ERR_INVALID, "tracker is NULL");
  CU(cudaSetDevice(t->device));
  int rc = t->drain();
  if (rc) return rc;
  if (out3) { out3[0] = t->acc_units_mn; out3[1] = t->acc_units_rows; out3[2] = t->acc_frames; out3[3] = t->acc_dense_scenes; }
  if (ms7) {
    for (int i = 0; i < 5; ++i) ms7[i] = t->acc_stage_ms[i];
    ms7[5] = t->acc_kernel_ms[0]; ms7[6] = t->acc_kernel_ms[1]; ms7[7] = (double)t->acc_tc_frames;
  }
  return 0;
}

int sb200_screen_counters(sb200_tracker* t, uint64_t* out4) {
  if (!t || !out4) return fail(SB200_ERR_INVALID, "bad arguments");
  CU(cudaSetDevice(t->device));
  int rc = t->drain();
  if (rc) return rc;
  for (int i = 0; i < 4; ++i) out4[i] = t->acc_screen[i];
  return 0;
}

// ... 335 lines not shown
    const float qnan = std::nanf("");
    for (int64_t i = 0; i < cnt; ++i) out[i] = qnan;
    for (const sb::PosEntry& e : ents) {
      const int64_t idx = (int64_t)e.m * d.n + e.n;
      if (idx < cnt) out[idx] = e.v;
    }
    return cnt;
  }
  return 0;
}

int sb200_last_stage_ms(sb200_tracker* t, float* out5) {
  if (!t || !out5) return fail(SB200_ERR_INVALID, "bad arguments");
  { int rc_ = t->drain(); if (rc_) return rc_; }
  memcpy(out5, t->stage_ms, sizeof(float) * 5);
  return 0;
}

int sb200_last_kernel_ms(sb200_tracker* t, float* out2) {
  if (!t || !out2) return fail(SB200_ERR_INVALID, "bad arguments");
  { int rc_ = t->drain(); if (rc_) return rc_; }
  out2[0] = t->kernel_ms[0];
  out2[1] = t->kernel_ms[1];
  return 0;
}

}

namespace {

constexpr uint32_t kBlobMagic = 0x42534253u;
constexpr uint32_t kBlobVersion = 1;
constexpr uint32_t kBlobTracker = 1, kBlobScenes = 2;
constexpr int kMaxSections = 48;

struct BlobHeader {
  uint32_t magic, version, type, n_sections;
  uint64_t total_bytes;
  sb200_options opts;
  int32_t feature_history, hist_len, d8, n_scenes;
  int32_t seen_features, adapt_dense, auto_waste_counter, auto_waste_periodicity;
  int32_t scene_cap, track_cap, pad0, pad1;
  int64_t live_total, blk_total, free_total, wasted_count, revealed, hpool_top, hpool_free, hpool_cap;
  uint64_t id_counter;
  uint64_t sec_off[kMaxSections], sec_bytes[kMaxSections];
};
struct BlobScene { uint64_t scene_id; uint32_t epoch; int32_t n_tracks, n_hidden, arena_top; };

std::vector<Col> blob_cols(sb200_tracker* t, uint32_t type) {
  const bool tracker_blob = type == kBlobTracker;
  std::vector<Col> b;
  for (const Col& c : t->store_table())
    if (c.blob == kBlobAll || (c.blob == kBlobTrackerOnly && tracker_blob)) b.push_back(c);
  if (tracker_blob) {
    for (const Col& c : t->wasted_table()) b.push_back(c);
    if (t->fhist_on) for (const Col& c : t->pool_table()) b.push_back(c);
  } else if (t->fhist_on) {
    for (const Col& c : t->pool_table())
      if (c.rows == kRowHistTop) b.push_back({c.buf, nullptr, c.w, false, kRowTrackHist});
  }
  return b;
}

std::vector<uint64_t> section_bytes(sb200_tracker* t, uint32_t type, int64_t n_scenes, int64_t live, int64_t blk,
                                    int64_t fre, int64_t wasted, int64_t top, int64_t hfree) {
  std::vector<uint64_t> b = {(uint64_t)n_scenes * sizeof(BlobScene)};
  const int64_t cnt[] = {live, blk, fre, wasted, top, hfree, live};
  for (const Col& c : blob_cols(t, type)) b.push_back((uint64_t)cnt[c.rows] * c.w);
  return b;
}

int64_t tracker_rows(const BlobHeader& h, int rows) {
  return rows == kRowWasted ? h.wasted_count : (rows == kRowHistTop ? h.hpool_top : h.hpool_free);
}

struct SlotRows { int slot, n, blk, fre; };

int move_store(sb200_tracker* t, int dir, uint32_t type, const BlobHeader& h, char* dblob, const std::vector<SlotRows>& rows,
               int hist_base) {
  const size_t tc = (size_t)t->track_cap;
  std::vector<sb::XferSeg> segs;
  const std::vector<Col> cols = blob_cols(t, type);
  size_t hist_sec = 0;
  for (size_t c = 0; c < cols.size(); ++c) {
    const Col& col = cols[c];
    char* sec = dblob + h.sec_off[1 + c];
    if (col.rows == kRowTrackHist) {
      if (!hist_sec) hist_sec = 1 + c;
      continue;
    }
    if (col.rows >= kRowWasted) {
      sb::add_segment(segs, dir, col.buf->as<char>(), sec, (uint64_t)tracker_rows(h, col.rows) * col.w);
      continue;
    }
    int64_t pre = 0;
    for (const SlotRows& r : rows) {
      const int64_t cnt = col.rows == kRowTrack ? r.n : (col.rows == kRowBlock ? r.blk : r.fre);
      sb::add_segment(segs, dir, col.buf->as<char>() + (size_t)r.slot * tc * col.w, sec + (uint64_t)pre * col.w,
                      (uint64_t)cnt * col.w);
      pre += cnt;
    }
  }
  const cudaStream_t st = t->stream;
  if (int rc = sb::copy_segments(segs, t->num_sms, st)) return rc;
  if (type == kBlobScenes && t->fhist_on && h.live_total > 0) {
    std::vector<int> tab(2 * rows.size() + 1, 0);
    for (size_t i = 0; i < rows.size(); ++i) { tab[i] = rows[i].slot; tab[rows.size() + i + 1] = tab[rows.size() + i] + rows[i].n; }
    DBuf d_tab;
    int rc = d_tab.ensure(tab.size() * sizeof(int));
    if (rc) return rc;
    CU(cudaMemcpyAsync(d_tab.p, tab.data(), tab.size() * sizeof(int), cudaMemcpyHostToDevice, st));
    const int e = sb::launch_xfer_hist(t->ts, t->P.d8, d_tab.as<int>(), d_tab.as<int>() + rows.size(), (int)rows.size(),
                                       (int)h.live_total, dir, reinterpret_cast<float*>(dblob + h.sec_off[hist_sec]),
                                       reinterpret_cast<unsigned char*>(dblob + h.sec_off[hist_sec + 1]), hist_base, t->num_sms, st);
    if (e) return fail(SB200_ERR_CUDA, "history copy launch failed: %s", cudaGetErrorString((cudaError_t)e));
    CU(cudaStreamSynchronize(st));
  }
  return 0;
}

int check_indices(sb200_tracker* t, uint32_t type, const BlobHeader& h, const char* dblob,
                  const std::vector<BlobScene>& table) {
  std::vector<sb::XferCheck> ck;
  const std::vector<Col> cols = blob_cols(t, type);
  const int K = t->P.max_obs;
  const char* obs_n_sec = nullptr;
  for (size_t c = 0; c < cols.size(); ++c)
    if (cols[c].tag == kTagObsN) obs_n_sec = dblob + h.sec_off[1 + c];
  for (size_t c = 0; c < cols.size(); ++c) {
    const Col& col = cols[c];
    if (col.tag == kTagNone) continue;
    const char* sec = dblob + h.sec_off[1 + c];
    if (col.rows >= kRowWasted) {
      ck.push_back({sec, nullptr, tracker_rows(h, col.rows), 0, (int)h.hpool_top, 0});
      continue;
    }
    int64_t pre = 0;
    for (const BlobScene& s : table) {
      const int fre = s.arena_top - s.n_tracks;
      const int64_t cnt = col.rows == kRowTrack ? s.n_tracks : (col.rows == kRowBlock ? s.arena_top : fre);
      const char* p = sec + (uint64_t)pre * col.w;
      switch (col.tag) {
        case kTagFblk: case kTagFree: ck.push_back({p, nullptr, cnt, 0, s.arena_top, 0}); break;
        case kTagOwner: ck.push_back({p, nullptr, cnt, -1, s.n_tracks, 0}); break;
        case kTagHblk: ck.push_back({p, nullptr, cnt, 0, (int)h.hpool_top, 0}); break;
        case kTagObsN: ck.push_back({p, nullptr, cnt, 0, K + 1, 1}); break;
        case kTagObsPhys: ck.push_back({p, reinterpret_cast<const unsigned char*>(obs_n_sec) + pre, cnt, 0, K, 2}); break;
        default: break;
      }
      pre += cnt;
    }
  }
  ck.erase(std::remove_if(ck.begin(), ck.end(), [](const sb::XferCheck& x) { return x.n <= 0; }), ck.end());
  if (ck.empty()) return 0;
  DBuf d;
  int rc = d.ensure(ck.size() * sizeof(sb::XferCheck) + 16);
  if (rc) return rc;
  int* d_bad = reinterpret_cast<int*>(d.as<char>() + ck.size() * sizeof(sb::XferCheck));
  CU(cudaMemcpyAsync(d.p, ck.data(), ck.size() * sizeof(sb::XferCheck), cudaMemcpyHostToDevice, t->stream));
  CU(cudaMemsetAsync(d_bad, 0, sizeof(int), t->stream));
  const int e = sb::launch_xfer_check(d.as<sb::XferCheck>(), (int)ck.size(), K, d_bad, t->stream);
  if (e) return fail(SB200_ERR_CUDA, "index check launch failed: %s", cudaGetErrorString((cudaError_t)e));
  int bad = 0;
  CU(cudaMemcpyAsync(&bad, d_bad, sizeof(int), cudaMemcpyDeviceToHost, t->stream));
  CU(cudaStreamSynchronize(t->stream));
  if (bad) return fail(SB200_ERR_INVALID, "the blob holds %d out-of-range block or observation indices", bad);
  return 0;
}

int set_slots(sb200_tracker* t, const std::vector<sb::XferSlot>& tab, int free0, int free_add, int top_add,
              unsigned long long id_min, bool raise_ids) {
  if (tab.empty()) return 0;
  DBuf d_tab;
  int rc = d_tab.ensure(tab.size() * sizeof(sb::XferSlot));
  if (rc) return rc;
  CU(cudaMemcpyAsync(d_tab.p, tab.data(), tab.size() * sizeof(sb::XferSlot), cudaMemcpyHostToDevice, t->stream));
  const int e = sb::launch_xfer_slots(d_tab.as<sb::XferSlot>(), (int)tab.size(), t->b_ntracks.as<int>(), t->ts.n_free,
                                      t->ts.arena_top, t->ts, free0, free_add, top_add,
                                      raise_ids ? t->b_idc.as<unsigned long long>() : nullptr, id_min, t->stream);
  if (e) return fail(SB200_ERR_CUDA, "slot update launch failed: %s", cudaGetErrorString((cudaError_t)e));
  CU(cudaStreamSynchronize(t->stream));
  return 0;
}

uint64_t read_id_counter(sb200_tracker* t, int* rc) {
  uint64_t v = 0;
  *rc = 0;
// ... 154 lines not shown
  o.max_scenes_hint = o.max_tracks_per_scene_hint = o.max_dets_per_scene_hint = 0;
  sb200_tracker* t = nullptr;
  if ((rc = sb200_tracker_create(&o, &t))) return rc;
  struct Guard { sb200_tracker* t; ~Guard() { if (t) sb200_tracker_destroy(t); } } guard{t};
  t->opts = h.opts;
  t->opts.device = device;
  if (h.feature_history && !t->P.is_visual) return fail(SB200_ERR_INVALID, "feature history on a non-visual tracker");
  if (h.feature_history && (rc = t->set_feature_history(true))) return rc;
  if (h.hist_len != t->hist_len || h.d8 != t->P.d8) return fail(SB200_ERR_INVALID, "the blob's row sizes do not match its options");
  if ((rc = check_sections(t, h))) return rc;
  int max_rows = 0;
  for (const BlobScene& s : table) max_rows = std::max(max_rows, std::max(s.n_tracks, s.arena_top));
  if ((h.scene_cap > 0 || !table.empty()) &&
      (rc = t->ensure_store(std::max<int>(h.scene_cap, (int)table.size()), std::max(std::max(h.track_cap, max_rows), 64))))
    return rc;
  if (h.wasted_count > 0 && (rc = t->ensure_wasted(h.wasted_count))) return rc;
  if (t->fhist_on && h.hpool_cap > 0 && (rc = t->ensure_hpool(std::max(h.hpool_cap, h.hpool_top)))) return rc;
  if ((rc = t->b_idc.ensure(8))) return rc;
  const char* dblob = nullptr;
  DBuf tmp;
  if ((rc = sb::blob_on_device(src, h.total_bytes, t->device, t->stream, tmp, &dblob))) return rc;
  if ((rc = check_indices(t, h.type, h, dblob, table))) return rc;
  std::vector<SlotRows> rows(table.size());
  std::vector<sb::XferSlot> st(table.size());
  for (size_t i = 0; i < table.size(); ++i) {
    const BlobScene& s = table[i];
    const int fre = t->P.is_visual ? s.arena_top - s.n_tracks : 0;
    rows[i] = {(int)i, s.n_tracks, s.arena_top, fre};
    st[i] = {(int)i, s.n_tracks, fre, s.arena_top, 0, 0};
  }
  if ((rc = move_store(t, 1, kBlobTracker, h, const_cast<char*>(dblob), rows, 0))) return rc;
  if ((rc = set_slots(t, st, 0, 0, 0, 0, false))) return rc;
  for (size_t i = 0; i < table.size(); ++i)
    if ((rc = t->regen_fp8((int)i, table[i].arena_top))) return rc;
  CU(cudaMemcpyAsync(t->b_idc.p, &h.id_counter, 8, cudaMemcpyHostToDevice, t->stream));
  if (h.wasted_count > 0) {
    const int wc = (int)h.wasted_count;
    CU(cudaMemcpyAsync(t->w_count.p, &wc, sizeof(int), cudaMemcpyHostToDevice, t->stream));
  }
  if (t->fhist_on) {
    const int hp[2] = {(int)h.hpool_free, (int)h.hpool_top};
    CU(cudaMemcpyAsync(t->ts.hpool, hp, sizeof(hp), cudaMemcpyHostToDevice, t->stream));
  }
  CU(cudaStreamSynchronize(t->stream));
  for (const BlobScene& s : table) {
    const int slot = t->slot_for(s.scene_id, true);
    t->epoch[slot] = s.epoch; t->n_tracks[slot] = s.n_tracks; t->n_hidden[slot] = s.n_hidden; t->arena_top[slot] = s.arena_top;
  }
  t->wasted_count = h.wasted_count; t->revealed = h.revealed;
  t->hpool_top = h.hpool_top; t->hpool_free = h.hpool_free;
  t->auto_waste_counter = h.auto_waste_counter; t->auto_waste_periodicity = h.auto_waste_periodicity;
  t->adapt_dense = h.adapt_dense != 0; t->seen_features = h.seen_features != 0;
  t->transferred = true;
  guard.t = nullptr;
  *out = t;
  return 0;
}

int sb200_scenes_export(sb200_tracker* t, int32_t n_scenes, const uint64_t* scene_ids, int32_t remove, void* dst,
                        size_t cap, size_t* bytes) {
  if (!t || !bytes || n_scenes < 1 || !scene_ids) return fail(SB200_ERR_INVALID, "bad arguments");
  int rc = sb::check_device(0);
  if (rc) return rc;
  CU(cudaSetDevice(t->device));
  if ((rc = t->drain())) return rc;
  std::vector<int> slots((size_t)n_scenes);
  std::unordered_map<uint64_t, int> seen;
  for (int i = 0; i < n_scenes; ++i) {
    if (!seen.emplace(scene_ids[i], i).second) return fail(SB200_ERR_INVALID, "scene %llu is listed twice", (unsigned long long)scene_ids[i]);
    slots[i] = t->slot_for(scene_ids[i], false);
    if (slots[i] < 0) return fail(SB200_ERR_INVALID, "unknown scene %llu", (unsigned long long)scene_ids[i]);
  }
  if ((rc = join_caller(t))) return rc;
  if ((rc = save_blob(t, kBlobScenes, slots, dst, cap, bytes))) return rc;
  if (!remove) return 0;
  std::vector<sb::XferSlot> st((size_t)n_scenes);
  int pushed = 0;
  for (int i = 0; i < n_scenes; ++i) {
    const int n = t->fhist_on ? t->n_tracks[slots[i]] : 0;
    st[i] = {slots[i], 0, 0, 0, n, pushed};
    pushed += n;
  }
  if ((rc = set_slots(t, st, (int)t->hpool_free, pushed, 0, 0, false))) return rc;
  for (int s : slots) { t->n_tracks[s] = 0; t->arena_top[s] = 0; t->epoch[s] = 0; }
  t->hpool_free += pushed;
  return 0;
}

int sb200_scenes_import(sb200_tracker* t, const void* src, size_t bytes) {
  if (!t || !src) return fail(SB200_ERR_INVALID, "tracker / src is NULL");
  int rc = sb::check_device(0);
  if (rc) return rc;
  CU(cudaSetDevice(t->device));
  if ((rc = t->drain())) return rc;
  BlobHeader h;
  std::vector<BlobScene> table;
  if ((rc = join_caller(t))) return rc;
  if ((rc = parse_blob(src, bytes, kBlobScenes, t->stream, &h, &table))) return rc;
  if (!same_options(h.opts, t->opts)) return fail(SB200_ERR_INVALID, "the blob's tracker options differ from this tracker's");
  if ((h.feature_history != 0) != t->fhist_on)
    return fail(SB200_ERR_INVALID, "the feature history is %s in the blob and %s here", h.feature_history ? "on" : "off", t->fhist_on ? "on" : "off");
  if ((rc = check_sections(t, h))) return rc;
  std::vector<int> dst_slot(table.size());
  int next = (int)t->scene_of_slot.size(), max_rows = 0;
  for (size_t i = 0; i < table.size(); ++i) {
    const int s = t->slot_for(table[i].scene_id, false);
    if (s >= 0 && (t->epoch[s] != 0 || t->n_tracks[s] != 0 || t->arena_top[s] != 0))
      return fail(SB200_ERR_INVALID, "scene %llu already exists in this tracker", (unsigned long long)table[i].scene_id);
    dst_slot[i] = s >= 0 ? s : next++;
    max_rows = std::max(max_rows, std::max(table[i].n_tracks, table[i].arena_top));
  }
  if ((rc = t->ensure_store(std::max(next, t->scene_cap), std::max(std::max(max_rows, t->track_cap), 64)))) return rc;
  if (!t->b_idc.p) {
    if ((rc = t->b_idc.ensure(8))) return rc;
    CU(cudaMemsetAsync(t->b_idc.p, 0, 8, t->stream));
  }
  const long long hist_base = t->fhist_on ? t->hpool_top : 0;
  if (t->fhist_on && hist_base + h.live_total > t->hpool_cap &&
      (rc = t->ensure_hpool(std::max(hist_base + h.live_total, t->hpool_cap + t->hpool_cap / 2))))
    return rc;
  const char* dblob = nullptr;
  DBuf tmp;
  if ((rc = sb::blob_on_device(src, h.total_bytes, t->device, t->stream, tmp, &dblob))) return rc;
  if ((rc = check_indices(t, h.type, h, dblob, table))) return rc;
  std::vector<SlotRows> rows(table.size());
  std::vector<sb::XferSlot> st(table.size());
  for (size_t i = 0; i < table.size(); ++i) {
    const BlobScene& s = table[i];
    const int fre = t->P.is_visual ? s.arena_top - s.n_tracks : 0;
    rows[i] = {dst_slot[i], s.n_tracks, s.arena_top, fre};
    st[i] = {dst_slot[i], s.n_tracks, fre, s.arena_top, 0, 0};
  }
  if ((rc = move_store(t, 1, kBlobScenes, h, const_cast<char*>(dblob), rows, (int)hist_base))) return rc;
  if ((rc = set_slots(t, st, 0, 0, t->fhist_on ? (int)h.live_total : 0, h.id_counter, true))) return rc;
  for (size_t i = 0; i < table.size(); ++i)
    if ((rc = t->regen_fp8(dst_slot[i], table[i].arena_top))) return rc;
  for (size_t i = 0; i < table.size(); ++i) {
    const int slot = t->slot_for(table[i].scene_id, true);
    t->epoch[slot] = table[i].epoch; t->n_tracks[slot] = table[i].n_tracks; t->arena_top[slot] = table[i].arena_top;
  }
  if (t->fhist_on) t->hpool_top += h.live_total;
  if (h.seen_features) t->seen_features = true;
  t->transferred = true;
  return 0;
}

int sb200_tracker_options(sb200_tracker* t, sb200_options* out, int32_t* feature_dim_fixed) {
  if (!t || !out) return fail(SB200_ERR_INVALID, "tracker / out is NULL");
  *out = t->opts;
  if (feature_dim_fixed) *feature_dim_fixed = t->seen_features ? 1 : 0;
  return 0;
}

void* sb200_host_alloc(size_t bytes) {
  void* p = nullptr;
  if (cudaMallocHost(&p, bytes) != cudaSuccess) { cudaGetLastError(); fail(SB200_ERR_CUDA, "cudaMallocHost failed"); return nullptr; }
  return p;
}
void sb200_host_free(void* p) { if (p) cudaFreeHost(p); }

}

namespace sb {

TrackerFeatureInfo tracker_feature_info(sb200_tracker* t) {
  return {t->device, t->P.is_visual, t->fhist_on, t->P.feature_dim, t->seen_features};
// ... 23 lines not shown
```

### similari_b200/csrc/kernels_cost.cu

```cuda
#include <cuda_bf16.h>

#include <algorithm>
#include <cstdlib>
#include <type_traits>

#include "sb_engine.cuh"

namespace sb {

__global__ void prep_kernel(Params p, Frame f) {
  int i = blockIdx.x * blockDim.x + threadIdx.x;
  if (i >= f.total) return;
  i += f.det0;
  if (f.decided) f.decided[i] = 0;
  const float* b = f.in_boxes + (size_t)i * 6;
  float xc = b[0], yc = b[1], ang = b[2], asp = b[3], h = b[4], conf = b[5];
  if (ang == 0.0f) ang = nanf("");
  float* cb = f.c_box + (size_t)i * 6;
  cb[0] = xc; cb[1] = yc; cb[2] = ang; cb[3] = asp; cb[4] = h; cb[5] = conf;
  f.c_radius[i] = box_radius(asp, h);
  f.c_conf[i] = conf < p.min_confidence ? p.min_confidence : conf;
  if (p.positional_kind == 1) box_vertices(xc, yc, ang, asp, h, f.c_vert + (size_t)i * 8);
  if (p.is_visual) {
    bool hasf = f.in_feat != nullptr && (f.in_hasf == nullptr || f.in_hasf[i] != 0);
    float q = f.in_quality ? f.in_quality[i] : 1.0f;
    bool ok = q >= p.min_quality_use;
    if (p.use_own_area && f.in_own) ok = ok && (f.in_own[i] >= p.min_own_use);
    ok = ok && (box_area(asp, h) >= p.min_area);
    f.c_flags[i] = (unsigned char)((hasf ? 1 : 0) | ((hasf && ok) ? 2 : 0));
  }
}

template <class T>
__global__ void cand_norm_kernel(Params p, Frame f, __nv_bfloat16* __restrict__ bf16_out) {
  int w = (blockIdx.x * blockDim.x + threadIdx.x) >> 5;
  int lane = threadIdx.x & 31;
  if (w >= f.total) return;
  w += f.det0;
  const int nblk = p.d8 / 8;
  const T* __restrict__ row = static_cast<const T*>(f.in_feat) + (size_t)w * p.feature_dim;
  constexpr bool kF32 = std::is_same<T, float>::value;
  const bool vec = (p.feature_dim % (kF32 ? 4 : 8) == 0) && (reinterpret_cast<uintptr_t>(f.in_feat) & 15) == 0;
  float acc = 0.0f;
  for (int base = 0; base < nblk; base += 64) {
    float x[2][8];
    bool have[2];
#pragma unroll
    for (int h = 0; h < 2; ++h) {
      const int blk = base + h * 32 + lane;
      have[h] = blk < nblk;
#pragma unroll
      for (int l = 0; l < 8; ++l) x[h][l] = 0.0f;
      if (have[h]) {
        if (vec && blk * 8 + 8 <= p.feature_dim) {
          if constexpr (kF32) {
            const float4 a = __ldcs(reinterpret_cast<const float4*>(row + blk * 8));
            const float4 b = __ldcs(reinterpret_cast<const float4*>(row + blk * 8 + 4));
            x[h][0] = a.x; x[h][1] = a.y; x[h][2] = a.z; x[h][3] = a.w; x[h][4] = b.x; x[h][5] = b.y; x[h][6] = b.z; x[h][7] = b.w;
          } else {
            feat_widen8(__ldcs(reinterpret_cast<const uint4*>(row + blk * 8)), row, x[h]);
          }
        } else {
#pragma unroll
          for (int l = 0; l < 8; ++l) { int d = blk * 8 + l; x[h][l] = d < p.feature_dim ? feat_elem(row, d) : 0.0f; }
        }
      }
    }
    if (f.c_fp8) {
      const float s = fp8_row_store(x, p.d8, f.c_fp8 + (size_t)w * fp8_pitch(p.d8));
      if (lane == 0) f.c_scale[w] = s;
    }
#pragma unroll
    for (int h = 0; h < 2; ++h) {
      float bs = 0.0f;
      if (have[h]) {
        const int blk = base + h * 32 + lane;
        float t[8];
#pragma unroll
        for (int l = 0; l < 8; ++l) t[l] = x[h][l] * x[h][l];
        bs = reduce_add8(t);
        if (bf16_out) {
          __nv_bfloat162 hh[4];
#pragma unroll
          for (int l = 0; l < 4; ++l) hh[l] = __floats2bfloat162_rn(x[h][2 * l], x[h][2 * l + 1]);
          *reinterpret_cast<uint4*>(bf16_out + (size_t)w * p.d8 + blk * 8) = *reinterpret_cast<uint4*>(hh);
        }
      }
      const int cnt = min(32, nblk - (base + h * 32));
      for (int j = 0; j < cnt; ++j) {
        float v = __shfl_sync(0xffffffffu, bs, j);
        acc = acc + v;
      }
    }
  }
  if (lane == 0) f.c_norm2[w] = acc;
}

void launch_prep(const Params& p, const Frame& f, int n_scenes, int max_m, cudaStream_t st) {
  (void)n_scenes; (void)max_m;
  if (f.total == 0) return;
  prep_kernel<<<(f.total + 255) / 256, 256, 0, st>>>(p, f);
  note_launch();
  if (p.is_visual && f.in_feat) {
    long long threads = (long long)f.total * 32;
    feat_dispatch(f.feat_type, [&](auto t) {
      cand_norm_kernel<decltype(t)><<<(unsigned)((threads + 255) / 256), 256, 0, st>>>(p, f, reinterpret_cast<__nv_bfloat16*>(f.c_bf16));
    });
    note_launch();
  }
}

constexpr int TN = 128;
constexpr int TM = 16;
constexpr int TY = 2;

struct CandTile {
  float xc[TM], yc[TM], ang0[TM], asp[TM], h[TM], r[TM], conf[TM];
  double vert[TM][8];
};

template <int POS>
__global__ void __launch_bounds__(TN * TY) pos_cost_kernel(Params p, TrackStore ts, Frame f) {
  const SceneDesc sc = f.scenes[blockIdx.z];
  const int n0 = blockIdx.x * TN, m0 = blockIdx.y * TM;
  if (n0 >= sc.n || m0 >= sc.m) return;
  __shared__ CandTile ct;
  const int tid = threadIdx.y * TN + threadIdx.x;
  for (int i = tid; i < TM; i += TN * TY) {
    int m = m0 + i;
    if (m < sc.m) {
      int g = sc.det_base + m;
      const float* cb = f.c_box + (size_t)g * 6;
      ct.xc[i] = cb[0]; ct.yc[i] = cb[1]; ct.ang0[i] = angle_or0(cb[2]); ct.asp[i] = cb[3]; ct.h[i] = cb[4];
      ct.r[i] = f.c_radius[g]; ct.conf[i] = f.c_conf[g];
    }
  }
  if (POS == 1) {
    for (int i = tid; i < TM * 8; i += TN * TY) {
      int m = m0 + i / 8;
      if (m < sc.m) ct.vert[i / 8][i % 8] = f.c_vert[(size_t)(sc.det_base + m) * 8 + (i % 8)];
    }
  }
  __syncthreads();
  const int n = n0 + threadIdx.x;
  if (n >= sc.n) return;
  const size_t ti = (size_t)sc.slot * ts.track_cap + n;
  const float* tb = ts.pred + ti * 6;
  const float txc = tb[0], tyc = tb[1], tasp = tb[3], th = tb[4];
  const float tr = ts.radius[ti];
  const unsigned int tep = ts.epoch[ti];
  float mean5[5], l5[5];
  double tv[8];
  if (POS == 0) {
    const float* st = ts.kst + ti * ts.kst_stride;
    const float hh = st[4];
#pragma unroll
    for (int i = 0; i < 5; ++i) {
      mean5[i] = st[i];
      l5[i] = sqrtf(kalman_proj_var(p.pos_weight, hh, st[10 + 4 * i], i));
    }
  } else {
#pragma unroll
    for (int i = 0; i < 8; ++i) tv[i] = ts.vert[ti * 8 + i];
// ... 320 lines not shown
}

constexpr int VM = 64, VN = 64, VK = 32, VT = 256;

template <class T>
__device__ void vis_cost_tile(const Params& p, const TrackStore& ts, const Frame& f, int scene, int bx, int by);

template <class T>
__global__ void __launch_bounds__(VT) vis_cost_kernel(Params p, TrackStore ts, Frame f, int n_scenes, int tiles_x, int tiles_y) {
  if (f.dense_cnt && *f.dense_cnt == 0) return;
  const long long per_scene = (long long)tiles_x * tiles_y;
  for (int scene = 0; scene < n_scenes; ++scene) {
    if (f.scene_mode[scene] == 0) continue;
    for (long long t = blockIdx.x; t < per_scene; t += gridDim.x) {
      vis_cost_tile<T>(p, ts, f, scene, (int)(t % tiles_x), (int)(t / tiles_x));
      __syncthreads();
    }
  }
}

template <class T>
__device__ void vis_cost_tile(const Params& p, const TrackStore& ts, const Frame& f, int scene, int bx, int by) {
  const SceneDesc sc = f.scenes[scene];
  const int K = p.max_obs;
  const int ncols = sc.n * K;
  const int c0 = bx * VN, m0 = by * VM;
  if (c0 >= ncols || m0 >= sc.m) return;
  __shared__ float sa[VM][VK + 1];
  __shared__ float sb_[VN][VK + 1];
  __shared__ int col_row[VN];
  __shared__ float col_norm[VN];
  __shared__ unsigned char col_ok[VN];
  __shared__ unsigned char row_ok[VM];
  __shared__ float row_norm[VM];
  const int tid = threadIdx.x;
  const bool cosine = p.visual_kind == 1;
  if (tid < VN) {
    int c = c0 + tid;
    int row = -1; float nrm = 0.0f; unsigned char ok = 0;
    if (c < ncols) {
      int n = c / K, k = c % K;
      size_t ti = (size_t)sc.slot * ts.track_cap + n;
      if (k < ts.obs_n[ti] && ts.obs_hasf[ti * K + k] && ts.feat_cnt[ti] >= p.min_track_length) {
        int phys = ts.obs_phys[ti * K + k];
        row = (int)(feat_block(ts, sc.slot, ti) * K + phys);
        nrm = cosine ? ts.fnorm2[row] : 0.0f;
        ok = 1;
      }
    }
    col_row[tid] = row; col_norm[tid] = nrm; col_ok[tid] = ok;
  }
  if (tid >= 64 && tid < 64 + VM) {
    int i = tid - 64;
    int m = m0 + i;
    unsigned char ok = 0; float nrm = 0.0f;
    if (m < sc.m) {
      int g = sc.det_base + m;
      ok = (f.c_flags[g] & 2) ? 1 : 0;
      nrm = cosine ? f.c_norm2[g] : 0.0f;
    }
    row_ok[i] = ok; row_norm[i] = nrm;
  }
  __syncthreads();
  const int tx = tid % 16, ty = tid / 16;
  float acc[4][4];
#pragma unroll
  for (int a = 0; a < 4; ++a)
#pragma unroll
    for (int b = 0; b < 4; ++b) acc[a][b] = 0.0f;
  const int D = p.feature_dim, D8 = p.d8;
  for (int k0 = 0; k0 < D8; k0 += VK) {
    for (int e = tid; e < VM * VK; e += VT) {
      int r = e / VK, c = e % VK;
      int m = m0 + r, d = k0 + c;
      float v = 0.0f;
      if (m < sc.m && d < D && row_ok[r]) v = feat_elem(static_cast<const T*>(f.in_feat), (size_t)(sc.det_base + m) * D + d);
      sa[r][c] = v;
    }
    for (int e = tid; e < VN * VK; e += VT) {
      int r = e / VK, c = e % VK;
      int d = k0 + c;
      float v = 0.0f;
      int row = col_row[r];
      if (row >= 0 && d < D8) v = ts.feat[(size_t)row * D8 + d];
      sb_[r][c] = v;
    }
    __syncthreads();
#pragma unroll
    for (int blk = 0; blk < VK / 8; ++blk) {
      float av[4][8], bv[4][8];
#pragma unroll
      for (int a = 0; a < 4; ++a)
#pragma unroll
        for (int l = 0; l < 8; ++l) av[a][l] = sa[ty * 4 + a][blk * 8 + l];
#pragma unroll
      for (int b = 0; b < 4; ++b)
#pragma unroll
        for (int l = 0; l < 8; ++l) bv[b][l] = sb_[tx * 4 + b][blk * 8 + l];
#pragma unroll
      for (int a = 0; a < 4; ++a)
#pragma unroll
        for (int b = 0; b < 4; ++b) {
          float t[8];
          if (cosine) {
#pragma unroll
            for (int l = 0; l < 8; ++l) t[l] = av[a][l] * bv[b][l];
          } else {
#pragma unroll
            for (int l = 0; l < 8; ++l) { float df = av[a][l] - bv[b][l]; t[l] = df * df; }
          }
          acc[a][b] = acc[a][b] + reduce_add8(t);
        }
    }
    __syncthreads();
  }
  float* out = f.vis + sc.vis_off;
  const float qnan = nanf("");
#pragma unroll
  for (int a = 0; a < 4; ++a) {
    int r = ty * 4 + a, m = m0 + r;
    if (m >= sc.m) continue;
    int g = sc.det_base + m;
    const float cx = f.c_box[(size_t)g * 6], cy = f.c_box[(size_t)g * 6 + 1], cr = f.c_radius[g];
#pragma unroll
    for (int b = 0; b < 4; ++b) {
      int cc = tx * 4 + b, c = c0 + cc;
      if (c >= ncols) continue;
      float v = qnan;
      if (row_ok[r] && col_ok[cc]) {
        int n = c / K;
        size_t ti = (size_t)sc.slot * ts.track_cap + n;
        const float* tb = ts.pred + ti * 6;
        if (compat_ok(p, sc.epoch, ts.epoch[ti], cx, cy, cr, tb[0], tb[1], ts.radius[ti])) {
          if (cosine) {
            float d = acc[a][b] / sqrtf(row_norm[r] * col_norm[cc]);
            if (d >= p.visual_threshold) v = 1.0f - d;
          } else {
            float d = sqrtf(acc[a][b]);
            if (d <= p.visual_threshold) v = d;
          }
        }
      }
      out[(size_t)m * ncols + c] = v;
    }
  }
}

int launch_vis_cost_a(const Params& p, const TrackStore& ts, const Frame& f, int n_scenes, int max_m, int max_n,
                      const TcArgs& tc, cudaStream_t st) {
  if (n_scenes == 0 || !p.is_visual) return 0;
  const bool any = max_m > 0 && max_n > 0 && f.in_feat != nullptr;
  const bool use_tc = tc.use_tc && any;
  if (!tc.max_init_done) launch_scene_max(p, f, n_scenes, true, st);
  if (use_tc && tc.dense) {
    int rc = launch_vis_dense(p, ts, f, n_scenes, max_m, tc, st);
    if (rc != 0) return rc;
  } else if (use_tc) {
    int rc = launch_vis_cost_tc(p, ts, f, n_scenes, max_n, tc, 0, st);
    if (rc != 0) return rc;
  }
  launch_vis_mode(p, f, n_scenes, use_tc, st);
  if (use_tc) {
    int rc = launch_vis_cost_tc(p, ts, f, n_scenes, max_n, tc, 1, st);
    if (rc != 0) return rc;
  }
  return 0;
}
// ... 31 lines not shown
```

### similari_b200/csrc/kernels_feat_dense.cu

```cuda
#include <cuda.h>
#include <cuda_bf16.h>
#include <cuda_fp16.h>
#include <cuda_runtime.h>
#include <stdint.h>

#include <algorithm>
#include <cstdlib>
#include <cstring>

#include "sb_engine.cuh"
#include "sb_tc.cuh"

namespace sb {

__device__ __forceinline__ float dense_err(const Params& p) { return p.vis_rel_err + 2e-4f; }

__device__ __forceinline__ bool dense_norm_ok(const Params& p, float n2) {
  return n2 <= 0.25f * 3.402823466e38f && (p.visual_kind != 1 || n2 > 0.0f);
}

constexpr int DS_STAGES = 4;
constexpr int DS_STAGE_BYTES = TC_A_BYTES + TC_B_BYTES;
constexpr int DS_CH = 16;
constexpr int DS_PITCH = DS_CH + 1;
// ... 386 lines not shown
  float cmax = use ? nb2 : 0.0f;
#pragma unroll
  for (int o = 16; o > 0; o >>= 1) cmax = fmaxf(cmax, __shfl_xor_sync(all, cmax, o));
  const int kt = __popc(__ballot_sync(all, use));
  __syncwarp();
  if (lane == 0) {
    DenseTrackMeta tm;
    tm.n = n; tm.kt = n >= 0 ? kt : 0; tm.cmax = n >= 0 ? cmax : 0.0f; tm.pad = 0;
    tmeta[sc.blk_off + b] = tm;
    if (cmax > 0.0f) atomicMax(reinterpret_cast<int*>(scene_cmax) + s, __float_as_int(cmax));
  }
  const int need_votes = p.min_votes > 1 ? p.min_votes : 1;
  const float ktf = (n >= 0 && kt >= need_votes) ? (float)kt : 0.0f;
  const int ph = lane;
  if (ph < K) {
    const int2 ri = s_ri[wi][ph];
    const int prow = b * K + ph;
    rowinfo[(size_t)sc.blk_off * K + prow] = ri;
    const int j = prow / cstep, cc = prow - j * cstep;
    const size_t slab = (size_t)sc.slab_off + j;
    slab_colc[slab * TC_BN + cc] = s_colc[wi][ph];
    slab_cmax[slab * TC_BN + cc] = cmax;
    slab_ktf[slab * TC_BN + cc] = ktf;
    if (ri.y >= 0) atomicOr(&slab_vmask[slab * (TC_BN / 32) + (cc >> 5)], 1u << (cc & 31));
    if (ph == K - 1) atomicOr(&slab_bmask[slab * (TC_BN / 32) + (cc >> 5)], 1u << (cc & 31));
  }
}

__global__ void vis_dense_rowmeta_kernel(Params p, Frame f, VisRowMeta* rowmeta) {
  int g = blockIdx.x * blockDim.x + threadIdx.x;
  if (g >= f.total) return;
  g += f.det0;
  const float na = f.c_norm2[g];
  VisRowMeta rm;
  rm.ok = (f.c_flags[g] & 2) ? 1 : 0;
  rm.rowk = p.visual_kind == 1 ? rsqrtf(na) : na;
  rm.rowi = 1.0f; rm.pad = 0;
  rowmeta[g] = rm;
}

constexpr int DSAMP = 32;
template <class T>
__global__ void __launch_bounds__(256) vis_dense_sample_kernel(Params p, TrackStore ts, Frame f, const int2* rowinfo, float* scene_l0,
                                                                int* dense_bad) {
  __shared__ int s_q[DSAMP], s_r[DSAMP];
  __shared__ int s_nq, s_nr;
  __shared__ float s_w[8];
  const int s = blockIdx.x;
  const SceneDesc sc = f.scenes[s];
  const int K = p.max_obs;
  const int tid = threadIdx.x, lane = tid & 31, wid = tid >> 5;
  if (tid == 0) { s_nq = 0; s_nr = 0; }
  __syncthreads();
  const int rows = sc.nb * K;
  for (int i = tid; i < sc.m; i += 256) {
    const int g = sc.det_base + i;
    if ((f.c_flags[g] & 2) && !dense_norm_ok(p, f.c_norm2[g])) dense_bad[s] = 1;
  }
  if (tid < DSAMP) {
    if (sc.m > 0) {
      const int m = (int)(((long long)tid * sc.m) / DSAMP);
      const bool dup = tid > 0 && (int)(((long long)(tid - 1) * sc.m) / DSAMP) == m;
      if (!dup && (f.c_flags[sc.det_base + m] & 2)) s_q[atomicAdd(&s_nq, 1)] = sc.det_base + m;
    }
  } else if (tid < 2 * DSAMP) {
    const int i = tid - DSAMP;
    if (rows > 0) {
      int pr = (int)(((long long)i * rows) / DSAMP);
      int fr = -1;
      for (int step = 0; step < 2 * K && pr < rows; ++step, ++pr) {
        fr = rowinfo[(size_t)sc.blk_off * K + pr].y;
        if (fr >= 0) break;
      }
      if (fr >= 0) s_r[atomicAdd(&s_nr, 1)] = fr;
    }
  }
  __syncthreads();
  const int nq = s_nq, nr = s_nr;
  float best = 0.0f;
  const int D = p.feature_dim;
  for (int pi = wid; pi < nq * nr; pi += 8) {
    const int g = s_q[pi / nr], fr = s_r[pi % nr];
    const T* a = static_cast<const T*>(f.in_feat) + (size_t)g * D;
    const float* b = ts.feat + (size_t)fr * p.d8;
    float dot = 0.0f;
    for (int d = lane; d < D; d += 32) dot = __fmaf_rn(feat_elem(a, d), b[d], dot);
#pragma unroll
    for (int o = 16; o > 0; o >>= 1) dot += __shfl_xor_sync(0xffffffffu, dot, o);
    const float na = f.c_norm2[g], nb2 = ts.fnorm2[fr];
    float v;
    if (p.visual_kind == 1) v = 1.0f - dot * rsqrtf(na) * rsqrtf(nb2) - 1e-4f;
    else v = (na + nb2 - 2.0f * dot) - 1e-4f * (na + nb2);
    best = fmaxf(best, v);
  }
  if (lane == 0) s_w[wid] = best;
  __syncthreads();
  if (tid == 0) {
    for (int w = 1; w < 8; ++w) best = fmaxf(best, s_w[w]);
    scene_l0[s] = best;
  }
}

constexpr int SEL_T = 512;
template <bool WIDE>
__global__ void __launch_bounds__(SEL_T) vis_dense_select_kernel(Params p, Frame f, const __half2* ws, const DenseTrackMeta* tmeta,
                                                                 const int2* rowinfo, const int* maxc_cnt, const int* max_nan,
                                                                 int* dense_bad, int* dbg_counts, const unsigned int* rowb,
                                                                 const unsigned int* colb, int fused) {
  extern __shared__ unsigned char sel_smem[];
  const int s = blockIdx.x;
  const SceneDesc sc = f.scenes[s];
  const int tid = threadIdx.x, lane = tid & 31;
  const int K = p.max_obs;
  const int nb = sc.nb, M = sc.m;
  if (M == 0 || nb == 0) return;
  const unsigned int um = f.scene_max[s];
  const float maxd = __uint_as_float((um & 0x80000000u) ? (um & 0x7fffffffu) : ~um);
  const int reason = (max_nan[s] != 0 ? 1 : 0) | (maxc_cnt[s] > sc.vis_lcap ? 2 : 0) | (!(maxd >= 0.0f) ? 4 : 0);
  if (tid == 0) {
    if (reason & 1) atomicAdd(&dbg_counts[0], 1);
    if (reason & 2) atomicAdd(&dbg_counts[1], 1);
    if (reason & 4) atomicAdd(&dbg_counts[2], 1);
    atomicAdd(&dbg_counts[3], maxc_cnt[s]);
  }
  if (reason) { if (tid == 0) dense_bad[s] = reason; return; }
  unsigned int* lcol = reinterpret_cast<unsigned int*>(sel_smem);
  short* kt = reinterpret_cast<short*>(lcol + nb);
  const int need_votes = p.min_votes > 1 ? p.min_votes : 1;
  for (int b = tid; b < nb; b += SEL_T) {
    const DenseTrackMeta tm = tmeta[sc.blk_off + b];
    const int kb = (tm.n >= 0 && tm.kt >= need_votes) ? tm.kt : 0;
    kt[b] = (short)kb;
    unsigned int u = 0x00800000u;
    if (fused && kb > 0) {
      const unsigned int cb = colb[sc.blk_off + b];
      if (cb != 0u) u = enc_ord(((float)kb * maxd * (1.0f - 2e-6f) - 1e-7f) + dec_ord(cb));
    }
    lcol[b] = u;
  }
  __syncthreads();
  const int mpad = (M + 127) / 128 * 128;
  const __half2* w0 = ws + sc.ws_off;
  const float fneg = -3.0e38f;
  for (int pass = fused ? 1 : 0; pass < 2; ++pass) {
    for (int m0 = 0; m0 < mpad; m0 += SEL_T) {
      const int m = m0 + tid;
      const bool row_ok = m < M && (f.c_flags[sc.det_base + m] & 2);
      float lrow = fneg;
      if (pass == 1 && row_ok) {
        if (!fused) lrow = f.vis_val[sc.vis_lbase + m];
        else {
          const unsigned int* rb = rowb + (size_t)(sc.det_base + m) * kDenseKClasses;
#pragma unroll
          for (int kc = 0; kc < kDenseKClasses; ++kc) {
            const unsigned int u = rb[kc];
            if (u != 0u) lrow = fmaxf(lrow, ((float)(kc + 1) * maxd * (1.0f - 2e-6f) - 1e-7f) + dec_ord(u));
          }
        }
      }
      const __half2* wrow = w0 + m;
      constexpr int UB = 8;
      for (int b0 = 0; b0 < nb; b0 += UB) {
        int kk[UB];
        float2 ee[UB];
#pragma unroll
        for (int u = 0; u < UB; ++u) {
          kk[u] = b0 + u < nb ? (int)kt[b0 + u] : 0;
// ... 157 lines not shown
```

### similari_b200/csrc/kernels_feat_tc.cu

```cuda
#include <cuda.h>
#include <cuda_bf16.h>
#include <cuda_runtime.h>
#include <stdint.h>

#include <algorithm>
#include <cstdlib>
#include <cstring>

#include "sb_engine.cuh"
#include "sb_tc.cuh"

namespace sb {

constexpr int TC_STAGES = 4;
constexpr int TC_STAGE_BYTES = TC_A_BYTES + TC_B_BYTES;

struct TcHdr { int scene, m0, ncols_left, m, det_base, col0, epoch, vis_lbase, vis_lcap, pad; };
struct TcSmem {
  unsigned char stage[TC_STAGES][TC_STAGE_BYTES];
  VisColMeta meta[4][TC_BN];
  VisRowMeta rowm[4][TC_BM];
  float colb[4][TC_BN];
  unsigned int colvalid[4][TC_BN / 32];
  TcHdr hdr[4];
// ... 448 lines not shown
              }
            }
          }
        }
      }
      __syncwarp();
      if (lane == 0) mbar_arrive(&S.meta_empty[ms]);
    }
  }
  __syncthreads();
  cluster_sync_all();
}


constexpr int RF_WARPS = 4;
constexpr int RF_SEG = 64;
constexpr int RF_PITCH = RF_SEG + 1;
constexpr int RF_CLAIM = 16;

template <bool TAIL>
__device__ __forceinline__ void refine_load_a(const float* __restrict__ a, int blk, int D, float* av) {
  if (!TAIL) {
    const float4 a0 = *reinterpret_cast<const float4*>(a + blk * 8);
    const float4 a1 = *reinterpret_cast<const float4*>(a + blk * 8 + 4);
    av[0] = a0.x; av[1] = a0.y; av[2] = a0.z; av[3] = a0.w; av[4] = a1.x; av[5] = a1.y; av[6] = a1.z; av[7] = a1.w;
  } else {
#pragma unroll
    for (int l = 0; l < 8; ++l) av[l] = blk * 8 + l < D ? a[blk * 8 + l] : 0.0f;
  }
}
template <bool TAIL, class T>
__device__ __forceinline__ void refine_load_a(const T* __restrict__ a, int blk, int D, float* av) {
  if (!TAIL) {
    feat_widen8(*reinterpret_cast<const uint4*>(a + blk * 8), a, av);
  } else {
#pragma unroll
    for (int l = 0; l < 8; ++l) av[l] = blk * 8 + l < D ? feat_elem(a, blk * 8 + l) : 0.0f;
  }
}
template <bool COSINE>
__device__ __forceinline__ float refine_block_sum(const float* av, const float* __restrict__ b, int blk) {
  const float4 b0 = *reinterpret_cast<const float4*>(b + blk * 8);
  const float4 b1 = *reinterpret_cast<const float4*>(b + blk * 8 + 4);
  const float bb[8] = {b0.x, b0.y, b0.z, b0.w, b1.x, b1.y, b1.z, b1.w};
  float t[8];
#pragma unroll
  for (int l = 0; l < 8; ++l) {
    if (COSINE) t[l] = av[l] * bb[l];
    else { const float df = av[l] - bb[l]; t[l] = df * df; }
  }
  return reduce_add8(t);
}

template <bool COSINE, bool TAIL, class T>
__global__ void __launch_bounds__(RF_WARPS * 32, 8) vis_refine_kernel(Params p, TrackStore ts, Frame f, int* nan_flag) {
  __shared__ float s_bs[RF_WARPS][RF_CLAIM][RF_PITCH];
  __shared__ int s_cnt[2];
  const int scene = blockIdx.y;
  if (f.vis_mode[scene] != 0) {
    if (f.screen_cnt && blockIdx.x == 0 && threadIdx.x == 0) atomicAdd(f.screen_cnt + 2, 1);
    return;
  }
  const SceneDesc sc = f.scenes[scene];
  const int lane = threadIdx.x & 31, w = threadIdx.x >> 5;
  if (f.screen_cnt) {
    if (threadIdx.x < 2) s_cnt[threadIdx.x] = 0;
    __syncthreads();
  }
  int n_ref = 0, n_cut = 0;
  const int n_pairs = min(f.vis_cnt[scene], sc.vis_lcap);
  const int nblk = p.d8 / 8;
  const int D = p.feature_dim;
  float (*bs)[RF_PITCH] = s_bs[w];
  float vmax = nanf("");
  for (;;) {
    int i0 = 0;
    if (lane == 0) i0 = atomicAdd(f.refine_next + scene, RF_CLAIM);
    i0 = __shfl_sync(0xffffffffu, i0, 0);
    if (i0 >= n_pairs) break;
    const int npair = min(RF_CLAIM, n_pairs - i0);
    VisPair mine;
    mine.g = 0; mine.row = 0; mine.scene = 0; mine.outcol = 0;
    if (lane < npair) mine = f.vis_pairs[sc.vis_lbase + i0 + lane];
    float acc = 0.0f;
    for (int seg0 = 0; seg0 < nblk; seg0 += RF_SEG) {
      const int segn = min(RF_SEG, nblk - seg0);
      int g_prev = -1;
      float av[RF_SEG / 32][8];
#pragma unroll 4
      for (int pp = 0; pp < npair; ++pp) {
        const int g = __shfl_sync(0xffffffffu, mine.g, pp);
        const int row = __shfl_sync(0xffffffffu, mine.row, pp);
        const float* b = ts.feat + (size_t)row * p.d8;
        if (g != g_prev) {
          const T* a = static_cast<const T*>(f.in_feat) + (size_t)g * D;
#pragma unroll
          for (int h = 0; h < RF_SEG / 32; ++h)
            if (h * 32 + lane < segn) refine_load_a<TAIL>(a, seg0 + h * 32 + lane, D, av[h]);
          g_prev = g;
        }
#pragma unroll
        for (int h = 0; h < RF_SEG / 32; ++h) {
          const int j = h * 32 + lane;
          if (j < segn) bs[pp][j] = refine_block_sum<COSINE>(av[h], b, seg0 + j);
        }
      }
      __syncwarp();
      if (lane < npair)
        for (int j = 0; j < segn; ++j) acc = acc + bs[lane][j];
      __syncwarp();
    }
    if (lane < npair) {
      float v = nanf("");
      if (COSINE) {
        const float d = acc / sqrtf(f.c_norm2[mine.g] * ts.fnorm2[mine.row]);
        if (d >= p.visual_threshold) v = 1.0f - d;
      } else {
        const float d = sqrtf(acc);
        if (d <= p.visual_threshold) v = d;
      }
      f.vis_val[sc.vis_lbase + i0 + lane] = v;
      n_ref += 1;
      n_cut += is_nan(v) ? 1 : 0;
      if (!is_nan(v) && !(v <= vmax)) vmax = v;
      if (nan_flag && is_nan(v)) nan_flag[scene] = 1;
    }
  }
  unsigned int u = 0u;
  if (!is_nan(vmax)) {
    u = __float_as_uint(vmax);
    u = (u & 0x80000000u) ? ~u : (u | 0x80000000u);
  }
#pragma unroll
  for (int o = 16; o > 0; o >>= 1) u = max(u, __shfl_xor_sync(0xffffffffu, u, o));
  if (lane == 0 && u != 0u) atomicMax(f.scene_max + scene, u);
  if (f.screen_cnt) {
    n_ref = __reduce_add_sync(0xffffffffu, n_ref);
    n_cut = __reduce_add_sync(0xffffffffu, n_cut);
    if (lane == 0 && n_ref) { atomicAdd(&s_cnt[0], n_ref); atomicAdd(&s_cnt[1], n_cut); }
    __syncthreads();
    if (threadIdx.x == 0 && s_cnt[0]) { atomicAdd(f.screen_cnt, s_cnt[0]); if (s_cnt[1]) atomicAdd(f.screen_cnt + 1, s_cnt[1]); }
  }
}

__global__ void vis_fill_none_kernel(Params p, Frame f) {
  const int scene = blockIdx.y;
  if (f.scene_mode[scene] != 0) return;
  const SceneDesc sc = f.scenes[scene];
  const long long cnt = (long long)sc.m * sc.n * p.max_obs;
  float* out = f.vis + sc.vis_off;
  const float qnan = nanf("");
  for (long long i = (long long)blockIdx.x * blockDim.x + threadIdx.x; i < cnt; i += (long long)gridDim.x * blockDim.x) out[i] = qnan;
}
__global__ void vis_scatter_kernel(Params p, Frame f) {
  const int scene = blockIdx.y;
  if (f.scene_mode[scene] != 0) return;
  const SceneDesc sc = f.scenes[scene];
  const int n_pairs = min(f.vis_cnt[scene], sc.vis_lcap);
  float* out = f.vis + sc.vis_off;
  for (int i = blockIdx.x * blockDim.x + threadIdx.x; i < n_pairs; i += gridDim.x * blockDim.x) {
    const VisPair vp = f.vis_pairs[sc.vis_lbase + i];
    out[(size_t)(vp.g - sc.det_base) * (sc.n * p.max_obs) + vp.outcol] = f.vis_val[sc.vis_lbase + i];
  }
}
void launch_vis_densify(const Params& p, const Frame& f, int n_scenes, cudaStream_t st) {
  if (n_scenes == 0) return;
  dim3 grid(64, n_scenes);
  vis_fill_none_kernel<<<grid, 256, 0, st>>>(p, f);
  vis_scatter_kernel<<<grid, 256, 0, st>>>(p, f);
  note_launch(2);
}

__global__ void to_bf16_kernel(const float* src, int src_pitch, int d, int d8, long long rows, __nv_bfloat16* dst) {
  long long i = (long long)blockIdx.x * blockDim.x + threadIdx.x;
  if (i >= rows * d8) return;
  long long r = i / d8;
  int c = (int)(i - r * d8);
  float x = c < d ? src[r * src_pitch + c] : 0.0f;
  dst[i] = __float2bfloat16_rn(x);
}

void launch_to_bf16(const float* src, int src_pitch, int d, int d8, long long rows, void* dst, cudaStream_t st) {
  if (rows == 0) return;
  long long n = rows * d8;
  to_bf16_kernel<<<(unsigned)((n + 255) / 256), 256, 0, st>>>(src, src_pitch, d, d8, rows, (__nv_bfloat16*)dst);
  note_launch();
}

__global__ void to_fp8_kernel(const float* src, int src_pitch, int d, int d8, long long rows, unsigned char* dst, float* scale) {
  const long long r = ((long long)blockIdx.x * blockDim.x + threadIdx.x) >> 5;
  if (r >= rows) return;
  const float s = fp8_row_from(src + r * src_pitch, d, d8, dst + r * fp8_pitch(d8));
  if ((threadIdx.x & 31) == 0) scale[r] = s;
}

void launch_to_fp8(const float* src, int src_pitch, int d, int d8, long long rows, unsigned char* dst, float* scale,
                   cudaStream_t st) {
  if (rows == 0) return;
  to_fp8_kernel<<<(unsigned)((rows * 32 + 255) / 256), 256, 0, st>>>(src, src_pitch, d, d8, rows, dst, scale);
  note_launch();
}

typedef CUresult (*EncodeTiledFn)(CUtensorMap*, CUtensorMapDataType, cuuint32_t, void*, const cuuint64_t*, const cuuint64_t*,
                                  const cuuint32_t*, const cuuint32_t*, CUtensorMapInterleave, CUtensorMapSwizzle,
                                  CUtensorMapL2promotion, CUtensorMapFloatOOBfill);

static EncodeTiledFn get_encode() {
  static EncodeTiledFn fn = nullptr;
  if (!fn) {
    void* p = nullptr;
    cudaDriverEntryPointQueryResult qr;
    if (cudaGetDriverEntryPoint("cuTensorMapEncodeTiled", &p, cudaEnableDefault, &qr) == cudaSuccess && p) fn = (EncodeTiledFn)p;
  }
  return fn;
}

int make_map(CUtensorMap* m, const void* base, long long rows, int d8, int box_rows, bool fp8) {
  EncodeTiledFn enc = get_encode();
  if (!enc) return -1;
  cuuint64_t dims[2] = {(cuuint64_t)d8, (cuuint64_t)rows};
  cuuint64_t strides[1] = {fp8 ? (cuuint64_t)fp8_pitch(d8) : (cuuint64_t)d8 * 2};
  cuuint32_t box[2] = {(cuuint32_t)(fp8 ? 2 * TC_BK : TC_BK), (cuuint32_t)box_rows};
  cuuint32_t estr[2] = {1, 1};
  CUresult r = enc(m, fp8 ? CU_TENSOR_MAP_DATA_TYPE_UINT8 : CU_TENSOR_MAP_DATA_TYPE_BFLOAT16, 2, (void*)base, dims, strides, box, estr, CU_TENSOR_MAP_INTERLEAVE_NONE,
                   CU_TENSOR_MAP_SWIZZLE_128B, CU_TENSOR_MAP_L2_PROMOTION_L2_256B, CU_TENSOR_MAP_FLOAT_OOB_FILL_NONE);
  return r == CUDA_SUCCESS ? 0 : -2;
}

static bool screen_fp8(const Params& p, const TcArgs& tc) { return tc.fp8 && !tc.dense && p.d8 <= kFp8MaxD8; }

__global__ void vis_meta_kernel(Params p, TrackStore ts, Frame f, int n_scenes, int max_rows, VisColMeta* colmeta,
                                VisColGeo* colgeo, float* colb, float* colsb, unsigned int* colvalid, bool fp8) {
  const int s = blockIdx.y;
  const SceneDesc sc = f.scenes[s];
  const int K = p.max_obs;
  const int prow = blockIdx.x * blockDim.x + threadIdx.x;
  const bool in = prow < sc.nb * K && prow < max_rows;
  VisColMeta cm;
  cm.colb = 0.0f; cm.colc = 0.0f; cm.outcol = -1; cm.row = -1;
  float csb = 1.0f;
  if (in) {
    const int b = prow / K, ph = prow - b * K;
    const size_t sbase = (size_t)sc.slot * ts.track_cap;
    const int n = ts.blk_owner ? ts.blk_owner[sbase + b] : b;
    const size_t ti = sbase + (n >= 0 ? n : 0);
    const size_t frow = (sbase + b) * K + ph;
    unsigned int tep = 0u;
    if (n >= 0) {
      const int on = ts.obs_n[ti];
      int k_of = -1, live_mask = 0;
      for (int k = 0; k < K; ++k) {
        if (k < on && ts.obs_hasf[ti * K + k]) {
          int pp = ts.obs_phys[ti * K + k];
          live_mask |= 1 << pp;
          if (pp == ph) k_of = k;
        }
      }
      tep = ts.epoch[ti];
      if (k_of >= 0) {
        const unsigned int delta = sc.epoch > tep ? sc.epoch - tep : tep - sc.epoch;
        cm.outcol = n * K + k_of;
        const bool valid = (ts.feat_cnt[ti] >= p.min_track_length) && ((unsigned int)p.max_idle_epochs >= delta);
        const float nb = ts.fnorm2[frow];
        const float E = fp8 ? p.vis_rel_err8 : p.vis_rel_err;
        cm.colb = p.visual_kind == 1 ? sqrtf(nb) : 0.5f * nb * (1.0f - 1e-5f - E);
        if (fp8) {
          if (fp8_norm_ok(nb)) { csb = ts.fscale[frow]; cm.colb *= csb; }
          else cm.colb = nanf("");
        }
        cm.row = valid ? (int)frow : -1;
      } else {
        int dead_rank = 0;
        for (int pp = 0; pp < ph; ++pp) dead_rank += ((live_mask >> pp) & 1) ? 0 : 1;
        int seen = 0;
        for (int k = 0; k < K; ++k) {
          bool lv = k < on && ts.obs_hasf[ti * K + k];
          if (!lv) { if (seen == dead_rank) { cm.outcol = n * K + k; break; } ++seen; }
        }
      }
    }
    colmeta[sc.col_off + prow] = cm;
    colb[sc.col_off + prow] = cm.colb;
// ... 145 lines not shown
```

### similari_b200/csrc/kernels_state.cu

```cuda
#include <cuda_bf16.h>

#include <algorithm>
#include <type_traits>

#include "sb_engine.cuh"

namespace sb {

constexpr int AT = 512;

__device__ __forceinline__ void write_box(float* dst, const Box& b) {
  dst[0] = b.xc; dst[1] = b.yc; dst[2] = b.angle; dst[3] = b.aspect; dst[4] = b.height; dst[5] = b.conf;
}
__device__ __forceinline__ void write_box_row(float* dst, const Box& b) {
  float2* d2 = reinterpret_cast<float2*>(dst);
  d2[0] = make_float2(b.xc, b.yc); d2[1] = make_float2(b.angle, b.aspect); d2[2] = make_float2(b.height, b.conf);
}

__global__ void __launch_bounds__(AT) apply_rank_kernel(Params p, TrackStore ts, Frame f, int n_scenes, int* n_tracks) {
  __shared__ int s_warp[AT / 32];
  __shared__ int s_carry;
  __shared__ int s_newbefore;
  const int sidx = blockIdx.x;
  const SceneDesc sc = f.scenes[sidx];
// ... 237 lines not shown
      ts.hpresent[hrow] = flags & 1;
      f.hist_dst[g] = (flags & 1) ? (int)hrow : -1;
    }
    if (ts.hist_len > 1) {
      const size_t hslot = (idx * ts.hist_len + (size_t)((o_len - 1u) % (unsigned int)ts.hist_len)) * 6;
      write_box_row(ts.hist_pred + hslot, pred);
      if (isnew) {
        const float* rb2 = f.in_boxes + (size_t)g * 6;
        write_box_row(ts.hist_obs + hslot, Box{rb2[0], rb2[1], rb2[2], rb2[3], rb2[4], rb2[5]});
      } else write_box_row(ts.hist_obs + hslot, cb);
    }
    if (f.o_ids) f.o_ids[g] = o_id;
    if (f.o_epochs) f.o_epochs[g] = sc.epoch;
    if (f.o_lengths) f.o_lengths[g] = o_len;
    if (f.o_vt) f.o_vt[g] = p.is_visual ? (o_vt < 0 ? (unsigned char)1 : (unsigned char)o_vt) : (unsigned char)1;
    if (f.o_pred) write_box(f.o_pred + (size_t)g * 6, pred);
    if (f.o_obs) write_box(f.o_obs + (size_t)g * 6, isnew ? Box{f.in_boxes[(size_t)g * 6], f.in_boxes[(size_t)g * 6 + 1], f.in_boxes[(size_t)g * 6 + 2], f.in_boxes[(size_t)g * 6 + 3], f.in_boxes[(size_t)g * 6 + 4], f.in_boxes[(size_t)g * 6 + 5]} : cb);
  }
}

__global__ void __launch_bounds__(256) apply_obs_wide_kernel(Params p, TrackStore ts, Frame f) {
  const int w = (int)((blockIdx.x * blockDim.x + threadIdx.x) >> 5), lane = threadIdx.x & 31;
  if (w >= f.total) return;
  const int g = f.det0 + w;
  const int win = f.winner[g];
  if (win < 0) return;
  const int K = p.max_obs;
  const unsigned int all = 0xffffffffu;
  const SceneDesc& sc = f.scenes[f.app_rank[g].x];
  const size_t idx = (size_t)sc.slot * ts.track_cap + win;
  const unsigned char flags = f.c_flags[g];
  const float quality = f.in_quality ? f.in_quality[g] : 1.0f;
  bool keep = (flags & 1) != 0;
  if (keep) {
    const float* cbp = f.c_box + (size_t)g * 6;
    bool ok = quality >= p.min_quality_collect;
    if (p.use_own_area && f.in_own) ok = ok && (f.in_own[g] >= p.min_own_collect);
    ok = ok && (box_area(cbp[3], cbp[4]) >= p.min_area);
    keep = ok;
  }
  const int on = ts.obs_n[idx];
  const bool have = lane < on && lane < K;
  const bool retain = have && ts.obs_hasf[idx * K + lane];
  const int ph0 = retain ? ts.obs_phys[idx * K + lane] : 0;
  const float q0 = retain ? ts.obs_q[idx * K + lane] : 0.0f;
  const unsigned int rmask = __ballot_sync(all, retain);
  int cnt = __popc(rmask);
  int src = 0;
  for (int b = 16; b > 0; b >>= 1)
    if (__popc(rmask & ((2u << (src + b - 1)) - 1u)) < lane + 1) src += b;
  int ph = __shfl_sync(all, ph0, src);
  float q = __shfl_sync(all, q0, src);
  for (int a = 1; a < cnt; ++a) {
    const float qa = __shfl_sync(all, q, a);
    const int pa = __shfl_sync(all, ph, a);
    const unsigned int stop = __ballot_sync(all, lane < a && !(q < qa));
    const int pos = stop ? 32 - __clz((int)stop) : 0;
    const float qu = __shfl_up_sync(all, q, 1);
    const int pu = __shfl_up_sync(all, ph, 1);
    if (lane > pos && lane <= a) { q = qu; ph = pu; }
    if (lane == pos) { q = qa; ph = pa; }
  }
  if (cnt >= K && cnt > 0) --cnt;
  const unsigned int used = __reduce_or_sync(all, lane < cnt ? 1u << ph : 0u);
  const int freep = __ffs((int)~used) - 1;
  unsigned char hasf = lane < cnt ? 1 : 0;
  if (lane == cnt) { ph = freep; q = quality; hasf = keep ? 1 : 0; }
  ++cnt;
  const int from = lane == 0 ? cnt - 1 : (lane == cnt - 1 ? 0 : lane);
  ph = __shfl_sync(all, ph, from);
  q = __shfl_sync(all, q, from);
  hasf = (unsigned char)__shfl_sync(all, (int)hasf, from);
  if (lane < cnt) {
    ts.obs_phys[idx * K + lane] = (unsigned char)ph; ts.obs_q[idx * K + lane] = q; ts.obs_hasf[idx * K + lane] = hasf;
  }
  const int fc = __popc(__ballot_sync(all, lane < cnt && hasf));
  if (lane == 0) {
    ts.obs_n[idx] = (unsigned char)cnt;
    ts.feat_cnt[idx] = (unsigned char)fc;
    if (f.feat_dst) f.feat_dst[g] = keep ? (int)(feat_block(ts, sc.slot, idx) * K + freep) : -1;
  }
}

template <class T>
__global__ void feat_store_kernel(Params p, TrackStore ts, Frame f) {
  int w = (blockIdx.x * blockDim.x + threadIdx.x) >> 5;
  int lane = threadIdx.x & 31;
  if (w >= f.total) return;
  if (lane == 0 && f.bf16_log) f.bf16_log[w] = f.feat_dst[f.det0 + w];
  w += f.det0;
  const int dst = f.feat_dst[w];
  const int hdst = f.hist_dst ? f.hist_dst[w] : -1;
  if (dst < 0 && hdst < 0) return;
  const T* src = static_cast<const T*>(f.in_feat) + (size_t)w * p.feature_dim;
  float* d = ts.feat + (size_t)max(dst, 0) * p.d8;
  __nv_bfloat16* db = reinterpret_cast<__nv_bfloat16*>(ts.feat_bf16) + (size_t)max(dst, 0) * p.d8;
  const bool wb = dst >= 0 && !f.skip_bf16;
  float* hd = hdst >= 0 ? ts.hrows + (size_t)hdst * p.d8 : nullptr;
  unsigned char* d8p = dst >= 0 && ts.feat_fp8 ? ts.feat_fp8 + (size_t)dst * fp8_pitch(p.d8) : nullptr;
  if constexpr (!std::is_same<T, float>::value) {
    if (p.feature_dim == p.d8 && (reinterpret_cast<uintptr_t>(f.in_feat) & 15) == 0) {
      const uint4* s8 = reinterpret_cast<const uint4*>(src);
      float4* d4 = reinterpret_cast<float4*>(d);
      float4* h4 = reinterpret_cast<float4*>(hd);
      uint4* b8 = reinterpret_cast<uint4*>(db);
      const int n8 = p.d8 >> 3;
      uint4 r[4];
      for (int i0 = 0; i0 < n8; i0 += 128) {
#pragma unroll
        for (int u = 0; u < 4; ++u) {
          const int i = i0 + u * 32 + lane;
          if (i < n8) r[u] = __ldcs(s8 + i);
        }
#pragma unroll
        for (int u = 0; u < 4; ++u) {
          const int i = i0 + u * 32 + lane;
          if (i < n8) {
            float x[8];
            feat_widen8(r[u], src, x);
            const float4 lo = make_float4(x[0], x[1], x[2], x[3]), hi = make_float4(x[4], x[5], x[6], x[7]);
            if (dst >= 0) {
              d4[2 * i] = lo;
              d4[2 * i + 1] = hi;
            }
            if (wb) {
              __nv_bfloat162 bb[4];
#pragma unroll
              for (int l = 0; l < 4; ++l) bb[l] = __floats2bfloat162_rn(x[2 * l], x[2 * l + 1]);
              b8[i] = *reinterpret_cast<const uint4*>(bb);
            }
            if (h4) { __stcs(h4 + 2 * i, lo); __stcs(h4 + 2 * i + 1, hi); }
          }
        }
      }
      if (d8p) {
        float x[2][8];
#pragma unroll
        for (int h = 0; h < 2; ++h) {
          if (h * 32 + lane < n8) feat_widen8(r[h], src, x[h]);
          else
#pragma unroll
            for (int l = 0; l < 8; ++l) x[h][l] = 0.0f;
        }
        const float s = fp8_row_store(x, p.d8, d8p);
        if (lane == 0) ts.fscale[dst] = s;
      }
    } else {
      for (int i = lane; i < p.d8; i += 32) {
        float x = i < p.feature_dim ? feat_elem(src, i) : 0.0f;
        if (dst >= 0) d[i] = x;
        if (wb) db[i] = __float2bfloat16_rn(x);
        if (hd) hd[i] = x;
      }
      if (d8p) {
        __syncwarp();
        const float s = fp8_row_from(d, p.d8, p.d8, d8p);
        if (lane == 0) ts.fscale[dst] = s;
      }
    }
  } else if (p.feature_dim == p.d8 && (reinterpret_cast<uintptr_t>(f.in_feat) & 15) == 0) {
    const float4* s4 = reinterpret_cast<const float4*>(src);
    float4* d4 = reinterpret_cast<float4*>(d);
    float4* h4 = reinterpret_cast<float4*>(hd);
    uint2* b4 = reinterpret_cast<uint2*>(db);
    const int n4 = p.d8 >> 2;
    float4 v[4];
    for (int i0 = 0; i0 < n4; i0 += 128) {
#pragma unroll
      for (int u = 0; u < 4; ++u) {
        const int i = i0 + u * 32 + lane;
        if (i < n4) v[u] = __ldcs(s4 + i);
      }
#pragma unroll
      for (int u = 0; u < 4; ++u) {
        const int i = i0 + u * 32 + lane;
        if (i < n4) {
          if (dst >= 0) d4[i] = v[u];
          if (wb) {
            const __nv_bfloat162 lo = __floats2bfloat162_rn(v[u].x, v[u].y), hi = __floats2bfloat162_rn(v[u].z, v[u].w);
            uint2 pk;
            pk.x = *reinterpret_cast<const unsigned int*>(&lo);
            pk.y = *reinterpret_cast<const unsigned int*>(&hi);
            b4[i] = pk;
          }
          if (h4) __stcs(h4 + i, v[u]);
        }
      }
    }
    if (d8p) {
      float amax = 0.0f;
#pragma unroll
      for (int u = 0; u < 4; ++u)
        if (u * 32 + lane < n4)
          amax = fmaxf(amax, fmaxf(fmaxf(fabsf(v[u].x), fabsf(v[u].y)), fmaxf(fabsf(v[u].z), fabsf(v[u].w))));
#pragma unroll
      for (int o = 16; o > 0; o >>= 1) amax = fmaxf(amax, __shfl_xor_sync(0xffffffffu, amax, o));
      const float s = fp8_row_scale(amax);
      unsigned int* o4 = reinterpret_cast<unsigned int*>(d8p);
#pragma unroll
      for (int u = 0; u < 4; ++u) {
        const int i = u * 32 + lane;
        if (i < n4) o4[i] = fp8_pack4(v[u].x, v[u].y, v[u].z, v[u].w, s);
      }
      if (lane == 0) ts.fscale[dst] = s;
    }
  } else {
    for (int i = lane; i < p.d8; i += 32) {
      float x = i < p.feature_dim ? src[i] : 0.0f;
      if (dst >= 0) d[i] = x;
      if (wb) db[i] = __float2bfloat16_rn(x);
      if (hd) hd[i] = x;
    }
    if (d8p) {
      __syncwarp();
      const float s = fp8_row_from(d, p.d8, p.d8, d8p);
      if (lane == 0) ts.fscale[dst] = s;
    }
  }
  if (lane == 0 && dst >= 0) ts.fnorm2[dst] = f.c_norm2[w];
}

__global__ void bf16_regen_kernel(TrackStore ts, int d8, int K, const int* __restrict__ rows, long long n, int n_slots) {
  const int lane = threadIdx.x & 31, wpb = blockDim.x >> 5;
  auto convert = [&](long long r) {
    const float4* s4 = reinterpret_cast<const float4*>(ts.feat + (size_t)r * d8);
    uint2* b4 = reinterpret_cast<uint2*>(reinterpret_cast<__nv_bfloat16*>(ts.feat_bf16) + (size_t)r * d8);
    for (int k = lane; k < (d8 >> 2); k += 32) {
      const float4 v = s4[k];
      const __nv_bfloat162 lo = __floats2bfloat162_rn(v.x, v.y), hi = __floats2bfloat162_rn(v.z, v.w);
      b4[k] = make_uint2(*reinterpret_cast<const unsigned int*>(&lo), *reinterpret_cast<const unsigned int*>(&hi));
    }
  };
  const long long w0 = (long long)blockIdx.x * wpb + (threadIdx.x >> 5), ws = (long long)gridDim.x * wpb;
  if (rows) {
    for (long long i = w0; i < n; i += ws)
      if (rows[i] >= 0) convert(rows[i]);
    return;
  }
  for (int s = blockIdx.y; s < n_slots; s += gridDim.y) {
    const long long r0 = (long long)s * ts.track_cap * K, nr = (long long)ts.arena_top[s] * K;
    for (long long i = w0; i < nr; i += ws) convert(r0 + i);
  }
}

void launch_bf16_regen(const TrackStore& ts, int d8, int K, const int* rows, long long n, int n_slots, cudaStream_t st) {
  if (rows ? n <= 0 : n_slots <= 0) return;
  const long long warps = rows ? n : (long long)ts.track_cap * K;
  const dim3 grid((unsigned)std::min<long long>((warps + 7) / 8, 2048), rows ? 1u : (unsigned)std::min(n_slots, 65535));
  bf16_regen_kernel<<<grid, 256, 0, st>>>(ts, d8, K, rows, n, n_slots);
  note_launch();
}

__global__ void hist_gather_kernel(TrackStore ts, int d8, const int* __restrict__ blk, const unsigned int* __restrict__ lengths,
                                   int n, int hist_cap, float* __restrict__ out_rows, unsigned char* __restrict__ out_present) {
  const long long w = ((long long)blockIdx.x * blockDim.x + threadIdx.x) >> 5;
  const int lane = threadIdx.x & 31;
  if (w >= (long long)n * hist_cap) return;
  const int i = (int)(w / hist_cap), c = (int)(w - (long long)i * hist_cap);
  const unsigned int len = lengths[i], H = (unsigned int)ts.fhist_len;
  const int cnt = (int)min(min(len, H), (unsigned int)hist_cap);
  unsigned char present = 0;
  size_t row = 0;
  if (c < cnt) {
    const unsigned int j = len - (unsigned int)cnt + (unsigned int)c;
    row = (size_t)blk[i] * H + j % H;
    present = ts.hpresent[row];
  }
  if (lane == 0) out_present[w] = present;
  const float4* s4 = reinterpret_cast<const float4*>(ts.hrows + row * d8);
  float4* d4 = reinterpret_cast<float4*>(out_rows + (size_t)w * d8);
  for (int k = lane; k < (d8 >> 2); k += 32) d4[k] = present ? s4[k] : make_float4(0.0f, 0.0f, 0.0f, 0.0f);
}

void launch_hist_gather(const TrackStore& ts, int d8, const int* blk, const unsigned int* lengths, int n, int hist_cap,
                        float* out_rows, unsigned char* out_present, cudaStream_t st) {
  const long long threads = (long long)n * hist_cap * 32;
  if (threads == 0) return;
  hist_gather_kernel<<<(unsigned)((threads + 255) / 256), 256, 0, st>>>(ts, d8, blk, lengths, n, hist_cap, out_rows,
                                                                        out_present);
  note_launch();
}

void launch_apply(const Params& p, const TrackStore& ts, const Frame& f, int n_scenes, int max_m,
                  unsigned long long id_base, int* d_n_tracks, cudaStream_t st) {
  (void)max_m;
  if (n_scenes == 0) return;
  apply_rank_kernel<<<n_scenes, AT, 0, st>>>(p, ts, f, n_scenes, d_n_tracks);
  note_launch();
  if (f.total > 0) {
    if (p.max_obs > kMaxObs) {
      apply_kernel<true><<<(f.total + 255) / 256, 256, 0, st>>>(p, ts, f, id_base);
      apply_obs_wide_kernel<<<(unsigned)(((long long)f.total * 32 + 255) / 256), 256, 0, st>>>(p, ts, f);
      note_launch(2);
    } else {
      apply_kernel<false><<<(f.total + 255) / 256, 256, 0, st>>>(p, ts, f, id_base);
      note_launch();
    }
  }
}

bool launch_feat_store(const Params& p, const TrackStore& ts, const Frame& f, cudaStream_t st) {
  if (!(p.is_visual && f.in_feat && f.total > 0)) return false;
  long long threads = (long long)f.total * 32;
  feat_dispatch(f.feat_type, [&](auto t) {
    feat_store_kernel<decltype(t)><<<(unsigned)((threads + 255) / 256), 256, 0, st>>>(p, ts, f);
  });
  note_launch();
  return true;
}

constexpr int WT = 512;
constexpr int WR = 8;

template <typename T>
__device__ __forceinline__ void compact_rows(T* arr, size_t base, int width, const int* s_dst, int first, int n) {
  T* a = arr + base * width;
  const int total = n * width;
  for (int e0 = first * width; e0 < total; e0 += WT * WR) {
    T v[WR];
    int de[WR];
#pragma unroll
    for (int r = 0; r < WR; ++r) {
      const int e = e0 + r * WT + (int)threadIdx.x;
      de[r] = -1;
      if (e < total) {
        const int j = e / width, c = e - j * width;
        const int d = s_dst[j];
        if (d >= 0 && d != j) { v[r] = a[e]; de[r] = d * width + c; }
      }
    }
    __syncthreads();
#pragma unroll
    for (int r = 0; r < WR; ++r)
      if (de[r] >= 0) a[de[r]] = v[r];
    __syncthreads();
  }
}

template <bool WIDE>
__global__ void __launch_bounds__(WT) waste_kernel(Params p, TrackStore ts, const unsigned int* cur_epoch,
                                                   const unsigned long long* scene_ids, int* n_tracks, WastedBuf wb,
                                                   const SceneDesc* scenes, int* frame_out, unsigned long long* id_counter,
                                                   long long id_add, const int* new_count, int n_scenes) {
  extern __shared__ int s_dst[];
  __shared__ int s_warp[WT / 32];
  __shared__ int s_wbase, s_wcount, s_first;
  if (id_counter && blockIdx.x == 0 && threadIdx.x == 0) {
    unsigned long long add = 0;
    if (id_add >= 0) add = (unsigned long long)id_add;
    else for (int s2 = 0; s2 < n_scenes; ++s2) add += (unsigned long long)new_count[s2];
    *id_counter += add;
  }
  if (ts.hblk && scenes && blockIdx.x == 0 && threadIdx.x == 0) {
    int add = 0;
    for (int s2 = 0; s2 < n_scenes; ++s2) add += new_count[s2];
    const int nf = ts.hpool[0];
    ts.hpool[0] = nf - min(nf, add);
    ts.hpool[1] += max(0, add - nf);
  }
  const int slot = scenes ? scenes[blockIdx.x].slot : (int)blockIdx.x;
  const int n = n_tracks[slot];
  const int tid = threadIdx.x, lane = tid & 31, wid = tid >> 5;
  const size_t base = (size_t)slot * ts.track_cap;
  const unsigned int cur = scenes ? scenes[blockIdx.x].epoch : cur_epoch[slot];
  const unsigned long long scene_id = scenes ? scenes[blockIdx.x].scene_id : scene_ids[slot];
  const int K = p.max_obs;
  const bool arena = ts.fblk != nullptr;
  if (n == 0) {
    if (frame_out && tid == 0) {
      frame_out[blockIdx.x * 3] = 0; frame_out[blockIdx.x * 3 + 1] = arena ? ts.arena_top[slot] : 0; frame_out[blockIdx.x * 3 + 2] = 0;
    }
    return;
  }
  if (tid == 0) s_first = n;
  int seen = 0;
  for (int j0 = 0; j0 < n; j0 += WT) {
    const int j = j0 + tid;
    const int w = (j < n && ts.epoch[base + j] + (unsigned int)p.max_idle_epochs < cur) ? 1 : 0;
    int x = w;
#pragma unroll
    for (int o = 1; o < 32; o <<= 1) {
      int t = __shfl_up_sync(0xffffffffu, x, o);
      if (lane >= o) x += t;
    }
    if (lane == 31) s_warp[wid] = x;
    __syncthreads();
    int woff = 0, wtot = 0;
    for (int q = 0; q < WT / 32; ++q) { if (q < wid) woff += s_warp[q]; wtot += s_warp[q]; }
    const int before = seen + woff + x - w;
// ... 330 lines not shown
```

### similari_b200/csrc/kernels_xfer.cu

```cuda
#include <cuda_runtime.h>
#include <stdint.h>

#include "sb_engine.cuh"

namespace sb {

namespace {

constexpr int kXferThreads = 256;

template <typename V>
__device__ __forceinline__ void copy_as(const char* __restrict__ s, char* __restrict__ d, size_t len) {
  const V* sv = reinterpret_cast<const V*>(s);
  V* dv = reinterpret_cast<V*>(d);
  const size_t n = len / sizeof(V);
  for (size_t i = threadIdx.x; i < n; i += kXferThreads) dv[i] = sv[i];
}

__global__ void __launch_bounds__(kXferThreads) xfer_copy_kernel(const XferSeg* __restrict__ segs,
                                                                  const long long* __restrict__ cpre, int n_seg) {
  const long long total = cpre[n_seg];
  for (long long c = blockIdx.x; c < total; c += gridDim.x) {
    int lo = 0, hi = n_seg - 1;
    while (lo < hi) {
// ... 40 lines not shown
    const float4* s = reinterpret_cast<const float4*>(dir == 0 ? ts.hrows + (size_t)blk * rw : rows + (size_t)t * rw);
    float4* d = reinterpret_cast<float4*>(dir == 0 ? rows + (size_t)t * rw : ts.hrows + (size_t)blk * rw);
    for (size_t i = threadIdx.x; i < rw / 4; i += kXferThreads) d[i] = s[i];
    const unsigned char* sp = dir == 0 ? ts.hpresent + (size_t)blk * H : pres + (size_t)t * H;
    unsigned char* dp = dir == 0 ? pres + (size_t)t * H : ts.hpresent + (size_t)blk * H;
    for (int i = threadIdx.x; i < H; i += kXferThreads) dp[i] = sp[i];
  }
}

__global__ void xfer_slots_kernel(const XferSlot* __restrict__ tab, int n, int* n_tracks, int* n_free, int* arena_top,
                                  TrackStore ts, int free0, int free_add, int top_add, unsigned long long* id_counter,
                                  unsigned long long id_min) {
  const XferSlot e = tab[blockIdx.x];
  const size_t base = (size_t)e.slot * ts.track_cap;
  if (e.push > 0)
    for (int j = threadIdx.x; j < e.push; j += blockDim.x) ts.hfree[free0 + e.push_off + j] = ts.hblk[base + j];
  if (threadIdx.x == 0) {
    n_tracks[e.slot] = e.n_tracks;
    if (n_free) n_free[e.slot] = e.n_free;
    if (arena_top) arena_top[e.slot] = e.arena_top;
    if (blockIdx.x == 0) {
      if (id_counter && *id_counter < id_min) *id_counter = id_min;
      if (ts.hpool) { ts.hpool[0] += free_add; ts.hpool[1] += top_add; }
    }
  }
}

__global__ void xfer_check_kernel(const XferCheck* __restrict__ ck, int K, int* bad) {
  const XferCheck c = ck[blockIdx.x];
  int cnt = 0;
  for (long long i = threadIdx.x; i < c.n; i += blockDim.x) {
    if (c.kind == 0) {
      const int v = static_cast<const int*>(c.p)[i];
      cnt += (v < c.lo || v >= c.hi);
    } else if (c.kind == 1) {
      const int v = static_cast<const unsigned char*>(c.p)[i];
      cnt += (v < c.lo || v >= c.hi);
    } else {
      const unsigned char* row = static_cast<const unsigned char*>(c.p) + i * K;
      const int on = min((int)c.aux[i], K);
      for (int k = 0; k < on; ++k) cnt += (row[k] < c.lo || row[k] >= c.hi);
    }
  }
  if (cnt) atomicAdd(bad, cnt);
}

}

int launch_xfer_check(const XferCheck* d_ck, int n, int K, int* bad, cudaStream_t st) {
  if (n <= 0) return 0;
  xfer_check_kernel<<<n, 256, 0, st>>>(d_ck, K, bad);
  note_launch();
  return (int)cudaGetLastError();
}

int launch_xfer_copy(const XferSeg* d_segs, const long long* d_cpre, int n_seg, long long chunks, int num_sms,
                     cudaStream_t st) {
  if (n_seg <= 0 || chunks <= 0) return 0;
  const long long grid = chunks < (long long)num_sms * 8 ? chunks : (long long)num_sms * 8;
  xfer_copy_kernel<<<(unsigned)grid, kXferThreads, 0, st>>>(d_segs, d_cpre, n_seg);
  note_launch();
  return (int)cudaGetLastError();
}

int launch_xfer_hist(const TrackStore& ts, int d8, const int* d_slots, const int* d_pre, int n, int total, int dir,
                     float* rows, unsigned char* pres, int base, int num_sms, cudaStream_t st) {
  if (n <= 0 || total <= 0) return 0;
  const int grid = total < num_sms * 8 ? total : num_sms * 8;
  xfer_hist_kernel<<<grid, kXferThreads, 0, st>>>(ts, d8, d_slots, d_pre, n, dir, rows, pres, base);
  note_launch();
  return (int)cudaGetLastError();
}

int launch_xfer_slots(const XferSlot* d_tab, int n, int* d_n_tracks, int* d_n_free, int* d_arena_top,
                      const TrackStore& ts, int free0, int free_add, int top_add, unsigned long long* id_counter,
                      unsigned long long id_min, cudaStream_t st) {
  if (n <= 0) return 0;
  xfer_slots_kernel<<<n, 128, 0, st>>>(d_tab, n, d_n_tracks, d_n_free, d_arena_top, ts, free0, free_add, top_add,
                                       id_counter, id_min);
  note_launch();
  return (int)cudaGetLastError();
}

}
```

### similari_b200/csrc/sb_engine.cuh

```cuda
#pragma once
#include <cuda_bf16.h>
#include <cuda_fp16.h>
#include <cuda_fp8.h>
#include <cuda_runtime.h>
#include <stdint.h>

#include <cstdlib>
#include <cstring>

#include "sb_math.cuh"

namespace sb {

constexpr int kMaxConstraints = 8;
constexpr int kNumSms = 132;
constexpr int kMaxObs = 8;
constexpr int kMaxObsWide = 32;
constexpr int kStateStride = 32;
constexpr int kMaxHist = 64;

inline float screen_rel_err(int d) {
  const double e = 0x1p-7 + 0x1p-16 + (double)d * 0x1p-23;
  const float floor_e = 2.1f / 256.0f;
  return e <= (double)floor_e ? floor_e : (float)(e * (1.0 + 0x1p-20));
// ... 74 lines not shown
  int slot;
  int m;
  int n;
  int det_base;
  long long pos_off;
  long long vis_off;
  unsigned int epoch;
  int col_off;
  unsigned long long scene_id;
  int pos_lbase, pos_lcap;
  int vis_lbase, vis_lcap;
  int nb;
  int pad0;
  long long ws_off;
  int blk_off;
  int slab_off;
};

struct SceneReq {
  int slot, m, det_base;
  unsigned int epoch;
  unsigned long long scene_id;
  int pos_lbase, pos_lcap, vis_lbase, vis_lcap;
};
struct FrameDyn {
  int n_tiles;
  int total_cols;
  int max_rows;
  int max_n;
  long long pos_total;
  long long vis_total;
  unsigned long long units_mn;
  unsigned long long units_rows;
  long long live_total;
  long long ws_total;
  int blk_total;
  int dense_scenes;
};

struct VisPair { int g, row, scene, outcol; };
struct PosEntry { unsigned short m, n; float v; };
constexpr int kVotePosCap = 3072;
constexpr int kVoteVisCap = 4096;

inline int pos_lcap(int m) {
  const long long c = (long long)m * 32;
  return (int)(c < 2ll * kVotePosCap ? c : 2ll * kVotePosCap);
}
inline int vis_lcap(int m, int vote_cap) {
  const long long c = (long long)m * 64;
  return (int)(c < 4ll * vote_cap ? c : 4ll * vote_cap);
}
inline bool vis_selective(bool euclidean, float threshold) { return euclidean ? threshold < 1e18f : threshold > -1.0f; }
inline bool vis_tc_worth(int d8, long long work) { return d8 >= 64 && work * d8 >= (1ll << 28); }
enum VisKernel { kVisRule, kVisSimt, kVisTc, kVisTc8, kVisTc16, kVisDense };
inline VisKernel vis_kernel_env() {
  const char* e = getenv("SB200_VIS_KERNEL");
  if (!e) return kVisRule;
  if (!strcmp(e, "simt")) return kVisSimt;
  if (!strcmp(e, "tc")) return kVisTc;
  if (!strcmp(e, "tc8")) return kVisTc8;
  if (!strcmp(e, "tc16")) return kVisTc16;
  if (!strcmp(e, "dense")) return kVisDense;
  return kVisRule;
}

struct TrackStore {
  int track_cap;
  unsigned long long* id;
  unsigned int* epoch;
  unsigned int* length;
  long long* custom;
  signed char* vt;
  float* pred;
  float* obs;
  float* radius;
  float* kst;
  int kst_stride;
  double* vert;
  int hist_len;
  float* hist_pred;
  float* hist_obs;
  float* feat;
  void* feat_bf16;
  unsigned char* feat_fp8;
  float* fscale;
  float* fnorm2;
  unsigned char* obs_phys;
  unsigned char* obs_hasf;
  float* obs_q;
  unsigned char* obs_n;
  unsigned char* feat_cnt;
  int* fblk;
  int* blk_owner;
  int* blk_free;
  int* n_free;
  int* arena_top;
  int fhist_len;
  int* hblk;
  float* hrows;
  unsigned char* hpresent;
  int* hfree;
  int* hpool;
};

__device__ __forceinline__ size_t feat_block(const TrackStore& ts, int slot, size_t ti) {
  return ts.fblk ? (size_t)slot * ts.track_cap + (size_t)ts.fblk[ti] : ti;
}

constexpr int kFeatF32 = 0, kFeatF16 = 1, kFeatBF16 = 2;

__device__ __forceinline__ float widen_f16(unsigned int h) {
  if ((h & 0x7c00u) == 0x7c00u) return __uint_as_float(((h & 0x8000u) << 16) | 0x7f800000u | ((h & 0x3ffu) << 13));
  return __half2float(__ushort_as_half((unsigned short)h));
}
__device__ __forceinline__ float widen_bf16(unsigned int b) { return __uint_as_float(b << 16); }

__device__ __forceinline__ float feat_elem(const float* p, size_t i) { return p[i]; }
__device__ __forceinline__ float feat_elem(const __half* p, size_t i) {
  return widen_f16(reinterpret_cast<const unsigned short*>(p)[i]);
}
__device__ __forceinline__ float feat_elem(const __nv_bfloat16* p, size_t i) {
  return widen_bf16(reinterpret_cast<const unsigned short*>(p)[i]);
}
__device__ __forceinline__ void feat_widen8(const uint4& r, const __half*, float* x) {
  const unsigned int w[4] = {r.x, r.y, r.z, r.w};
#pragma unroll
  for (int i = 0; i < 4; ++i) { x[2 * i] = widen_f16(w[i] & 0xffffu); x[2 * i + 1] = widen_f16(w[i] >> 16); }
}
__device__ __forceinline__ void feat_widen8(const uint4& r, const __nv_bfloat16*, float* x) {
  const unsigned int w[4] = {r.x, r.y, r.z, r.w};
#pragma unroll
  for (int i = 0; i < 4; ++i) { x[2 * i] = widen_bf16(w[i] & 0xffffu); x[2 * i + 1] = __uint_as_float(w[i] & 0xffff0000u); }
}
template <class Fn>
inline void feat_dispatch(int type, Fn&& fn) {
  if (type == kFeatF16) fn(__half());
  else if (type == kFeatBF16) fn(__nv_bfloat16());
  else fn(float());
}

struct Frame {
  int total;
  int det0;
  int scene0;
  int feat_type;
  const int* new_count_all;
  long long pos_fill_off;
  const float* in_boxes;
  const void* in_feat;
  const unsigned char* in_hasf;
  const float* in_quality;
  const long long* in_custom;
  const float* in_own;
  float* c_box;
  float* c_radius;
  float* c_conf;
  double* c_vert;
  unsigned char* c_flags;
  float* c_norm2;
  void* c_bf16;
  unsigned char* c_fp8;
  float* c_scale;
  int* screen_cnt;
  unsigned int* scene_max;
  int* winner;
  unsigned char* c_vt;
  float* pos;
  bool pos_dense_all;
  long long pos_total;
  float* vis;
  SceneDesc* scenes;
  int* new_count;
  int* status;
  int* feat_dst;
  bool skip_bf16;
  int* bf16_log;
  int* hist_dst;
  int2* app_rank;
  int4* app_meta;
  int* frame_out;
  const FrameDyn* dyn;
  unsigned long long* id_counter;
  long long id_add;
  PosEntry* pos_list;
  int* pos_cnt;
  VisPair* vis_pairs;
  float* vis_val;
  int* vis_cnt;
  int* scene_mode;
  int* vis_mode;
  unsigned char* decided;
  unsigned char* excl;
  int* pre_winner;
  int* dense_cnt;
  int* refine_next;
  const int* dense_bad;
  unsigned long long* o_ids;
  unsigned int* o_epochs;
  unsigned int* o_lengths;
  unsigned char* o_vt;
  float* o_pred;
  float* o_obs;
};

inline size_t counter_ints(int n) { return 6 * (size_t)n + 4; }
inline void carve_counters(int* c, int n, Frame& f) {
  using F = Frame;
  int* F::* const rows[] = {&F::pos_cnt, &F::vis_cnt, &F::scene_mode, &F::vis_mode, &F::refine_next, &F::status, &F::dense_cnt};
  for (int i = 0; i < 7; ++i) f.*rows[i] = c + (size_t)i * n;
  f.screen_cnt = f.dense_cnt + 1;
}

struct TcTile { int scene, m0, c0, pad; };
struct VisColMeta {
  float colb;
  float colc;
  int outcol;
  int row;
};
struct VisColGeo { float tx, ty, tr; unsigned int tep; };
struct VisRowMeta { float rowk; int ok; float rowi; int pad; };
struct DenseTrackMeta { int n; int kt; float cmax; int pad; };

void launch_prep(const Params& p, const Frame& f, int n_scenes, int max_m, cudaStream_t st);
void launch_own_area(const Frame& f, int n_scenes, int max_m, const float* d_boxes, float* d_out, int* d_ovf_cnt,
                     int2* d_ovf, cudaStream_t st);
void launch_pull(void* dst, const void* src, size_t bytes, cudaStream_t st);
void launch_frame_setup(const Params& p, const TrackStore& ts, const Frame& f, const SceneReq* req, int n_scenes,
                        const int* d_n_tracks, int mstep, int cstep, bool dense, TcTile* tiles, FrameDyn* dyn, int* zero,
                        int n_zero, cudaStream_t st);
void note_launch(int n = 1);
unsigned long long launch_count();
void launch_pos_cost(const Params& p, const TrackStore& ts, const Frame& f, int n_scenes, int max_m, int max_n,
                     cudaStream_t st);
struct TcArgs {
  int max_init_done;
  int colmeta_done;
  bool use_tc;
  const TcTile* d_tiles;
  int n_tiles;
  const int* d_n_tiles;
  long long a_rows, b_rows;
  int num_sms;
  cudaEvent_t ev_screen0, ev_screen1, ev_refine1;
  VisColMeta* colmeta;
  VisColGeo* colgeo;
  float* colb;
  unsigned int* colvalid;
  VisRowMeta* rowmeta;
  bool fp8;
  float* colsb;
  int total_cols;
  int max_rows;
  bool dense;
  int cstep;
  int max_blocks;
  int n_slabs_ub;
  void* ws;
  unsigned int* d_rowb;
  unsigned int* d_colb;
  long long blk_ub;
  float* slab_ktf;
  DenseTrackMeta* tmeta;
  int2* rowinfo;
  float* slab_colc;
  float* slab_cmax;
  unsigned int* slab_vmask;
  unsigned int* slab_bmask;
  float* scene_l0;
  float* scene_cmax;
  VisPair* maxc;
  float* maxc_val;
  int* maxc_cnt;
  int* maxc_next;
  int* dense_bad;
  int* zeros;
  int* dbg_counts;
};
int launch_vis_cost(const Params& p, const TrackStore& ts, const Frame& f, int n_scenes, int max_m, int max_n,
                    const TcArgs& tc, cudaStream_t st);
int launch_vis_dense(const Params& p, const TrackStore& ts, const Frame& f, int n_scenes, int max_m, const TcArgs& tc,
                     cudaStream_t st);
int launch_vis_cost_a(const Params& p, const TrackStore& ts, const Frame& f, int n_scenes, int max_m, int max_n,
                      const TcArgs& tc, cudaStream_t st);
int launch_vis_cost_b(const Params& p, const TrackStore& ts, const Frame& f, int n_scenes, int max_m, int max_n,
                      const TcArgs& tc, cudaStream_t st);
void launch_pos_fill(const Params& p, const Frame& f, int n_scenes, int max_m, int max_n, cudaStream_t st);
void launch_pos_scan(const Params& p, const TrackStore& ts, const Frame& f, int n_scenes, int max_m, int max_n,
                     cudaStream_t st);
void launch_pos_scan_lazy(const Params& p, const TrackStore& ts, const Frame& f, int n_scenes, int max_m, int max_n,
                          int pass, cudaStream_t st);
int launch_vote_masks(const Params& p, const TrackStore& ts, const Frame& f, int n_scenes, int max_m, int max_n,
                      cudaStream_t st);
void launch_vis_colmeta(const Params& p, const TrackStore& ts, const Frame& f, int n_scenes, int max_n, const TcArgs& tc,
                        cudaStream_t st);
int vis_screen_ucols(int d8, int num_sms, int n_scenes, const int* m, const int* nb, int K);
int launch_vis_cost_tc(const Params& p, const TrackStore& ts, const Frame& f, int n_scenes, int max_n, const TcArgs& tc,
                       int phase, cudaStream_t st);
void launch_vis_densify(const Params& p, const Frame& f, int n_scenes, cudaStream_t st);
void launch_to_bf16(const float* src, int src_pitch, int d, int d8, long long rows, void* dst, cudaStream_t st);
void launch_to_fp8(const float* src, int src_pitch, int d, int d8, long long rows, unsigned char* dst, float* scale,
                   cudaStream_t st);
constexpr int kFp8MaxD8 = 512;
void launch_scene_max(const Params& p, const Frame& f, int n_scenes, bool init_only, cudaStream_t st);
void launch_scene_mode(const Params& p, const Frame& f, int n_scenes, bool tc_used, cudaStream_t st);
void launch_vis_mode(const Params& p, const Frame& f, int n_scenes, bool tc_used, cudaStream_t st);
size_t voting_smem_need(int max_m, int max_n, int viscap = 0);
constexpr size_t kVotingSmemLimit = 220 * 1024;
int launch_voting(const Params& p, const TrackStore& ts, const Frame& f, int n_scenes, int max_m, int max_n,
                  cudaStream_t st);
void launch_apply(const Params& p, const TrackStore& ts, const Frame& f, int n_scenes, int max_m,
                  unsigned long long id_base, int* d_n_tracks, cudaStream_t st);
bool launch_feat_store(const Params& p, const TrackStore& ts, const Frame& f, cudaStream_t st);
void launch_bf16_regen(const TrackStore& ts, int d8, int K, const int* rows, long long n, int n_slots, cudaStream_t st);
struct WastedBuf {
  int cap;
  int* count;
  unsigned long long* id;
  unsigned long long* scene;
  unsigned int* epoch;
  unsigned int* length;
  float* pred;
  float* obs;
  float* hist_pred;
  float* hist_obs;
  int* hblk;
};
void launch_waste(const Params& p, const TrackStore& ts, int n_slots, const unsigned int* d_cur_epoch,
                  const unsigned long long* d_scene_ids, int* d_n_tracks, const WastedBuf& wb, int max_n,
                  cudaStream_t st);
void launch_frame_sweep(const Params& p, const TrackStore& ts, const Frame& f, int n_scenes, int* d_n_tracks,
                        const WastedBuf& wb, cudaStream_t st);
void launch_hist_gather(const TrackStore& ts, int d8, const int* blk, const unsigned int* lengths, int n, int hist_cap,
                        float* out_rows, unsigned char* out_present, cudaStream_t st);

constexpr int kXferChunk = 32 * 1024;
struct XferSeg { const char* src; char* dst; unsigned long long bytes; };
int launch_xfer_copy(const XferSeg* d_segs, const long long* d_cpre, int n_seg, long long chunks, int num_sms,
                     cudaStream_t st);
int launch_xfer_hist(const TrackStore& ts, int d8, const int* d_slots, const int* d_pre, int n, int total, int dir,
                     float* rows, unsigned char* pres, int base, int num_sms, cudaStream_t st);
struct XferSlot { int slot, n_tracks, n_free, arena_top, push, push_off; };
struct XferCheck { const void* p; const unsigned char* aux; long long n; int lo, hi, kind; };
int launch_xfer_check(const XferCheck* d_ck, int n, int K, int* bad, cudaStream_t st);
int launch_xfer_slots(const XferSlot* d_tab, int n, int* d_n_tracks, int* d_n_free, int* d_arena_top,
                      const TrackStore& ts, int free0, int free_add, int top_add, unsigned long long* id_counter,
                      unsigned long long id_min, cudaStream_t st);

void launch_kalman_ops(int op, float pw, float vw, const float* in30, const float* boxes, int n, float* out30,
                       cudaStream_t st);
void launch_kalman_distance(float pw, const float* in30, const float* boxes, int n, float* out, cudaStream_t st);
void launch_point_kalman(int op, float pw, float vw, const float* in12, const float* points, int n, float* out,
                         cudaStream_t st);
void launch_box_vertices(const float* boxes6, int n, double* out8, cudaStream_t st);
void launch_clip_polygons(const float* subjects6, const float* clippings6, int n, double* out_xy, int* out_counts,
                          double* out_areas, int* d_status, cudaStream_t st);
void launch_intersection_areas(const double* a_vert, int m, const double* b_vert, int n, double* out_mn, int* d_status,
                               cudaStream_t st);

__device__ __forceinline__ bool compat_ok(const Params& p, unsigned int cand_epoch, unsigned int trk_epoch, float cx,
                                          float cy, float cr, float tx, float ty, float tr) {
  unsigned int delta = cand_epoch > trk_epoch ? cand_epoch - trk_epoch : trk_epoch - cand_epoch;
  if ((unsigned int)p.max_idle_epochs < delta) return false;
  for (int i = 0; i < p.n_constraints; ++i) {
    if ((unsigned int)p.constraint_epochs[i] >= delta) {
      float d = dist_in_2r(cx, cy, cr, tx, ty, tr);
      return d <= p.constraint_max_dist[i];
    }
  }
  return true;
}

}
```

Before: 60.49 billion.

## Store track features in an indirected row pool with device free stacks

Track feature rows move out of a dense per-slot block array into a shared pool addressed through an obs_row indirection table. Free rows come from double-buffered device stacks. The prep kernel writes each detection's features straight into a pool row during normalisation, so the feature store kernel can link rows instead of copying full vectors. This removes the per-frame feature copy and the dense over-allocation, but adds an extra indirection on every feature read, host-side stack bookkeeping, and occasional synchronizations when the pool grows or must be reread.

```diff
diff --git a/similari_b200/csrc/engine.cu b/similari_b200/csrc/engine.cu
--- a/similari_b200/csrc/engine.cu
+++ b/similari_b200/csrc/engine.cu
@@ -37,7 +37,7 @@
 
 enum ColRows { kRowTrack, kRowBlock, kRowFree, kRowWasted, kRowHistTop, kRowHistFree, kRowTrackHist };
 enum ColBlob { kBlobNo, kBlobAll, kBlobTrackerOnly };
-enum ColTag { kTagNone, kTagFblk, kTagHblk, kTagObsN, kTagObsPhys, kTagOwner, kTagFree };
+enum ColTag { kTagNone, kTagFblk, kTagHblk, kTagObsN, kTagObsPhys, kTagOwner, kTagFree, kTagFeatRows };
 struct Col {
   DBuf* buf;
   void (*point)(sb200_tracker&, void*);
@@ -132,13 +132,15 @@
     int dense_scenes;
     int hpool[2];
     int screen[3];
+    int row_n, pad;
   };
-  static_assert(offsetof(FrameBack, dense_scenes) == sizeof(sb::FrameDyn) && sizeof(FrameBack) == sizeof(sb::FrameDyn) + 24,
+  static_assert(offsetof(FrameBack, dense_scenes) == sizeof(sb::FrameDyn) && sizeof(FrameBack) == sizeof(sb::FrameDyn) + 32,
                 "FrameBack: FrameDyn followed by the counters, without padding");
   static size_t back_offset(int n_scenes) { return ((size_t)n_scenes * 16 + 15) / 16 * 16; }
   struct Pending {
     bool active = false;
     int n_scenes = 0, total = 0;
+    int row_set = -1;
     std::vector<int> slots, m;
     long long live_ub = 0;
     HBuf h_req;
@@ -192,6 +194,10 @@
   long long hpool_top = 0;
   long long hpool_free = 0;
   long long hpool_pend = 0;
+  DBuf b_obs_row, b_rstack[2], b_rn;
+  long long row_cap = 0;
+  long long row_known[2]{};
+  long long row_pend[2]{};
   enum InColumn { kBoxes, kFeat, kHasf, kQuality, kCustom, kOwn, kInCols };
   using InPtrs = std::array<const void*, kInCols>;
   InPtrs in_ptrs(const void* boxes, const void* feat, const void* hasf, const void* quality, const void* custom,
@@ -230,7 +236,7 @@
     bool read_pending = false;
   } stg[2];
   int stg_last = 1;
-  struct CandBufs { DBuf box, radius, conf, vert, flags, norm2, bf16, decided, fp8, scale; } cand[2];
+  struct CandBufs { DBuf box, radius, conf, vert, flags, norm2, bf16, decided, fp8, scale, row; } cand[2];
   DBuf f_winner, f_cvt, f_pos, f_vis, f_scenes, f_newcount,
       f_status, f_featdst, f_apprank, f_appmeta, f_frameout, f_excl, f_prewin, f_own, f_ownovf, f_dyn, f_ws, f_tmeta, f_rowinfo, f_slabc, f_slabm, f_slabmask,
       f_dscene, f_maxc, f_maxcval, f_drowb, f_dcolb, f_slabk, f_scene_max, f_tiles, f_pairs, f_colmeta, f_colgeo, f_colb, f_colvalid, f_rowmeta, f_poslist, f_counters, f_visval, f_colsb;
@@ -289,7 +295,8 @@
       c.push_back({&b_feat_cnt, in_ts<&TS::feat_cnt>, 1});
       c.push_back({&b_fblk, in_ts<&TS::fblk>, 4, false, kRowTrack, kBlobAll, kTagFblk});
       if (fhist_on) c.push_back({&b_hblk, in_ts<&TS::hblk>, 4, false, kRowTrack, kBlobTrackerOnly, kTagHblk});
-      c.push_back({&b_feat, in_ts<&TS::feat>, 4 * K * d8, true, kRowBlock});
+      c.push_back({&b_feat, nullptr, 4 * K * d8, false, kRowBlock, kBlobAll, kTagFeatRows});
+      c.push_back({&b_obs_row, in_ts<&TS::obs_row>, 4 * K, true, kRowBlock, kBlobNo});
       c.push_back({&b_feat_bf16, in_ts<&TS::feat_bf16>, 2 * K * d8, true, kRowBlock});
       c.push_back({&b_fnorm2, in_ts<&TS::fnorm2>, 4 * K, false, kRowBlock});
       if (P.d8 <= sb::kFp8MaxD8) {
@@ -359,7 +366,8 @@
   int regen_fp8(int slot, int top) {
     if (!ts.feat_fp8 || top <= 0) return 0;
     const long long r0 = (long long)slot * track_cap * P.max_obs, rows = (long long)top * P.max_obs;
-    sb::launch_to_fp8(ts.feat + r0 * P.d8, P.d8, P.d8, P.d8, rows, ts.feat_fp8 + r0 * sb::fp8_pitch(P.d8), ts.fscale + r0, stream);
+    sb::launch_to_fp8(ts.feat, P.d8, P.d8, P.d8, rows, ts.feat_fp8 + r0 * sb::fp8_pitch(P.d8), ts.fscale + r0, stream,
+                      ts.obs_row + r0);
     return cudaGetLastError() == cudaSuccess ? 0 : fail(SB200_ERR_CUDA, "e4m3 row conversion failed");
   }
 
@@ -376,6 +384,62 @@
     return cudaGetLastError() == cudaSuccess ? 0 : fail(SB200_ERR_CUDA, "BF16 row conversion failed");
   }
 
+  int ensure_rows(int c, long long need, long long frame) {
+    if (row_known[c] >= need) return 0;
+    const int o = c ^ 1;
+    const long long mv = std::min(std::max<long long>(0, row_known[o] - need), need - row_known[c]);
+    if (mv > 0 && row_cap > 0) {
+      CU(cudaMemcpyAsync(b_rstack[c].as<int>() + row_known[c], b_rstack[o].as<int>() + row_known[o] - mv, 4 * (size_t)mv,
+                         cudaMemcpyDeviceToDevice, stream));
+      row_known[c] += mv;
+      row_known[o] -= mv;
+    }
+    if (row_known[c] < need) {
+      const long long add = need - row_known[c];
+      const long long base = std::max<long long>(row_cap, 1);
+      long long cap = std::max(base + add, row_cap + row_cap / 2);
+      cap = std::max(cap, 1 + (long long)scene_cap * track_cap * P.max_obs + 2 * kDepth * frame);
+      if (cap >= (1ll << 31)) return fail(SB200_ERR_CAPACITY, "the feature row pool needs %lld rows", cap);
+      DBuf nf;
+      int rc = nf.ensure(std::max<size_t>(1, (size_t)cap * P.d8 * 4));
+      if (rc) return rc;
+      if (row_cap > 0) CU(cudaMemcpyAsync(nf.p, b_feat.p, (size_t)row_cap * P.d8 * 4, cudaMemcpyDeviceToDevice, stream));
+      else CU(cudaMemsetAsync(nf.p, 0, (size_t)P.d8 * 4, stream));
+      for (int k = 0; k < 2; ++k) {
+        DBuf ns;
+        if ((rc = ns.ensure((size_t)cap * 4))) return rc;
+        if (row_known[k] > 0) CU(cudaMemcpyAsync(ns.p, b_rstack[k].p, 4 * (size_t)row_known[k], cudaMemcpyDeviceToDevice, stream));
+        CU(cudaStreamSynchronize(stream));
+        b_rstack[k] = std::move(ns);
+      }
+      std::vector<int> fresh((size_t)(cap - base));
+      for (size_t i = 0; i < fresh.size(); ++i) fresh[i] = (int)(cap - 1 - (long long)i);
+      const long long give_c = add + (cap - base - add) / 2, give_o = cap - base - give_c;
+      CU(cudaMemcpyAsync(b_rstack[c].as<int>() + row_known[c], fresh.data(), 4 * (size_t)give_c, cudaMemcpyHostToDevice, stream));
+      CU(cudaMemcpyAsync(b_rstack[o].as<int>() + row_known[o], fresh.data() + give_c, 4 * (size_t)give_o, cudaMemcpyHostToDevice, stream));
+      CU(cudaStreamSynchronize(stream));
+      row_known[c] += give_c;
+      row_known[o] += give_o;
+      b_feat = std::move(nf);
+      row_cap = cap;
+      ts.feat = b_feat.as<float>();
+    }
+    if (!b_rn.p) { int rc = b_rn.ensure(2 * sizeof(int)); if (rc) return rc; }
+    const int cnt[2] = {(int)row_known[0], (int)row_known[1]};
+    CU(cudaMemcpyAsync(b_rn.p, cnt, sizeof(cnt), cudaMemcpyHostToDevice, stream));
+    CU(cudaStreamSynchronize(stream));
+    return 0;
+  }
+  int read_rows() {
+    if (!b_rn.p) return 0;
+    int cnt[2];
+    CU(cudaMemcpyAsync(cnt, b_rn.p, sizeof(cnt), cudaMemcpyDeviceToHost, stream));
+    CU(cudaStreamSynchronize(stream));
+    row_known[0] = cnt[0];
+    row_known[1] = cnt[1];
+    return 0;
+  }
+
   int ensure_store(int need_scenes, int need_tracks) {
     if (need_scenes <= scene_cap && need_tracks <= track_cap) return 0;
     int ns = scene_cap, nt = track_cap;
@@ -383,7 +447,9 @@
     if (need_tracks > nt) nt = std::max(need_tracks, std::max(64, nt * 2));
     int rc = regen_bf16();
     if (rc) return rc;
-    rc = grow(store_table(), ns, nt, scene_cap, track_cap);
+    std::vector<Col> cols = store_table();
+    cols.erase(std::remove_if(cols.begin(), cols.end(), [](const Col& c) { return c.tag == kTagFeatRows; }), cols.end());
+    rc = grow(cols, ns, nt, scene_cap, track_cap);
     if (rc) return rc;
     if (ns != scene_cap && (rc = grow(slot_table(), ns, 1, scene_cap, 1))) return rc;
     ts.kst_stride = sb::kStateStride;
@@ -583,6 +649,7 @@
     for (int s = 0; s < q.n_scenes; ++s) pending_add[q.slots[s]] -= q.m[s];
     inflight_live_ub -= q.live_ub;
     if (fhist_on) hpool_pend -= q.total;
+    if (q.row_set >= 0) row_pend[q.row_set] -= q.total;
     q.active = false;
     pend_count -= 1;
   }
@@ -679,6 +746,14 @@
       if ((rc = drain("feature history pool bound"))) return rc;
       const long long want = hpool_top + std::max<long long>(0, frames * total - hpool_free);
       if (want > hpool_cap && (rc = ensure_hpool(std::max<long long>(want, hpool_cap + hpool_cap / 2)))) return rc;
+    }
+    if (P.is_visual && rq.in[kFeat] && total > 0) {
+      const int c = (int)(frame_seq & 1);
+      if (row_known[c] - row_pend[c] < total) {
+        if ((rc = drain("feature row pool bound")) || (rc = read_rows())) return rc;
+        const long long frame = std::max<long long>(total, hint_dets(n_scenes));
+        if ((rc = ensure_rows(c, kDepth * frame, frame))) return rc;
+      }
     }
     if (!b_idc.p) {
       if ((rc = b_idc.ensure(8))) return rc;
@@ -858,6 +933,12 @@
     f.c_bf16 = tc.use_tc && !tc.fp8 ? cb.bf16.p : nullptr;
     f.c_fp8 = tc.fp8 ? cb.fp8.as<unsigned char>() : nullptr;
     f.c_scale = tc.fp8 ? cb.scale.as<float>() : nullptr;
+    if (P.is_visual && f.in_feat && total > 0) {
+      if ((rc = ENS(cb.row, T * 4, f.c_row))) return rc;
+      f.row_pool = ts.feat;
+      f.row_stack = b_rstack[pl.cset].as<int>();
+      f.row_n = b_rn.as<int>() + pl.cset;
+    }
     if ((rc = ENS(f_poslist, sizeof(sb::PosEntry) * (size_t)std::max<long long>(1, std::max(pl.posl_total, hint_dets(n_scenes) * 32)), f.pos_list)) ||
         (rc = ENS(f_counters, sizeof(int) * sb::counter_ints(n_scenes))))
       return rc;
@@ -901,6 +982,11 @@
     for (int s = 0; s < n_scenes; ++s) pending_add[last_req_slots[s]] += pl.m_of[s];
     inflight_live_ub += pl.live_ub;
     if (fhist_on) hpool_pend += rq.total;
+    q.row_set = -1;
+    if (P.is_visual && rq.in[kFeat] && rq.total > 0) {
+      q.row_set = pl.cset;
+      row_pend[pl.cset] += rq.total;
+    }
     pend_count += 1;
     last_n_scenes = n_scenes;
     return Rollback{this, &q, true};
@@ -1028,6 +1114,7 @@
     CU(cudaMemcpyAsync(&back->dyn, f_dyn.p, sizeof(back->dyn), cudaMemcpyDeviceToHost, stream));
     CU(cudaMemcpyAsync(&back->dense_scenes, cnt.dense_cnt, sizeof(back->dense_scenes), cudaMemcpyDeviceToHost, stream));
     if (fhist_on) CU(cudaMemcpyAsync(back->hpool, ts.hpool, sizeof(back->hpool), cudaMemcpyDeviceToHost, stream));
+    if (f.c_row) CU(cudaMemcpyAsync(&back->row_n, f.row_n, sizeof(int), cudaMemcpyDeviceToHost, stream));
     CU(cudaMemcpyAsync(back->screen, cnt.screen_cnt, sizeof(back->screen), cudaMemcpyDeviceToHost, stream));
     static const bool trace_dense = getenv("SB200_TRACE") != nullptr && atoi(getenv("SB200_TRACE")) >= 2;
     if (trace_dense && tc.dense && tc.n_tiles > 0) {
@@ -1097,6 +1184,7 @@
       n_hidden[slot] += h_fo[3 * s + 2];
       wasted_count += h_fo[3 * s + 2];
     }
+    if (q.row_set >= 0) row_known[q.row_set] = back.row_n;
     if (fhist_on) {
       hpool_free = back.hpool[0];
       hpool_top = back.hpool[1];
@@ -1340,7 +1428,7 @@
   auto d8_cols = [t] {
     std::vector<std::pair<Col, size_t>> v;
     for (const Col& c : t->store_table())
-      if (c.buf == &t->b_feat || c.buf == &t->b_feat_bf16 || c.buf == &t->b_feat_fp8 || c.buf == &t->b_fscale)
+      if (c.buf == &t->b_feat_bf16 || c.buf == &t->b_feat_fp8 || c.buf == &t->b_fscale)
         v.push_back({c, (size_t)t->scene_cap * t->track_cap});
     if (t->fhist_on)
       for (const Col& c : t->pool_table()) if (c.buf == &t->b_hrows) v.push_back({c, (size_t)t->hpool_cap});
@@ -1348,6 +1436,12 @@
   };
   for (const auto& [c, rows] : d8_cols()) { c.buf->release(); c.point(*t, nullptr); }
   for (auto& cb : t->cand) { cb.bf16.release(); cb.fp8.release(); }
+  t->b_feat.release();
+  for (auto& b : t->b_rstack) b.release();
+  t->b_rn.release();
+  t->ts.feat = nullptr;
+  t->row_cap = t->row_known[0] = t->row_known[1] = 0;
+  if (t->b_obs_row.p) CU(cudaMemsetAsync(t->b_obs_row.p, 0, t->b_obs_row.bytes, t->stream));
   t->P.feature_dim = feature_dim;
   t->P.d8 = (feature_dim + 7) / 8 * 8;
   t->P.vis_rel_err = sb::screen_rel_err(feature_dim);
@@ -1849,9 +1943,14 @@
   std::vector<sb::XferSeg> segs;
   const std::vector<Col> cols = blob_cols(t, type);
   size_t hist_sec = 0;
+  char* feat_sec = nullptr;
   for (size_t c = 0; c < cols.size(); ++c) {
     const Col& col = cols[c];
     char* sec = dblob + h.sec_off[1 + c];
+    if (col.tag == kTagFeatRows) {
+      feat_sec = sec;
+      continue;
+    }
     if (col.rows == kRowTrackHist) {
       if (!hist_sec) hist_sec = 1 + c;
       continue;
@@ -1870,6 +1969,37 @@
   }
   const cudaStream_t st = t->stream;
   if (int rc = sb::copy_segments(segs, t->num_sms, st)) return rc;
+  if (feat_sec && h.blk_total > 0 && dir == 0 && !t->ts.feat) {
+    CU(cudaMemsetAsync(feat_sec, 0, (size_t)h.blk_total * t->P.max_obs * t->P.d8 * 4, st));
+    CU(cudaStreamSynchronize(st));
+  } else if (feat_sec && h.blk_total > 0) {
+    const long long K = t->P.max_obs, n = (long long)rows.size();
+    std::vector<long long> tab(2 * n + 1, 0);
+    for (long long i = 0; i < n; ++i) {
+      tab[i] = (long long)rows[i].slot * (long long)tc * K;
+      tab[n + i + 1] = tab[n + i] + (long long)rows[i].blk * K;
+    }
+    const long long total = tab[2 * n];
+    int rc = 0;
+    const int* fresh = nullptr;
+    if (dir == 1) {
+      if ((rc = t->ensure_rows(0, total, 0))) return rc;
+      fresh = t->b_rstack[0].as<int>() + (t->row_known[0] - total);
+    }
+    DBuf d_tab;
+    if ((rc = d_tab.ensure(tab.size() * sizeof(long long)))) return rc;
+    CU(cudaMemcpyAsync(d_tab.p, tab.data(), tab.size() * sizeof(long long), cudaMemcpyHostToDevice, st));
+    const int e = sb::launch_xfer_feat(t->ts, t->P.d8, d_tab.as<long long>(), d_tab.as<long long>() + n, (int)n, total, dir,
+                                       reinterpret_cast<float*>(feat_sec), fresh, t->num_sms, st);
+    if (e) return fail(SB200_ERR_CUDA, "feature row copy launch failed: %s", cudaGetErrorString((cudaError_t)e));
+    CU(cudaStreamSynchronize(st));
+    if (dir == 1) {
+      t->row_known[0] -= total;
+      const int cnt = (int)t->row_known[0];
+      CU(cudaMemcpyAsync(t->b_rn.p, &cnt, sizeof(int), cudaMemcpyHostToDevice, st));
+      CU(cudaStreamSynchronize(st));
+    }
+  }
   if (type == kBlobScenes && t->fhist_on && h.live_total > 0) {
     std::vector<int> tab(2 * rows.size() + 1, 0);
     for (size_t i = 0; i < rows.size(); ++i) { tab[i] = rows[i].slot; tab[rows.size() + i + 1] = tab[rows.size() + i] + rows[i].n; }
@@ -2190,6 +2320,15 @@
     pushed += n;
   }
   if ((rc = set_slots(t, st, (int)t->hpool_free, pushed, 0, 0, false))) return rc;
+  if (t->b_rn.p) {
+    for (int s : slots) {
+      const long long K = t->P.max_obs;
+      const int e = sb::launch_free_feat_rows(t->ts.obs_row, (long long)s * t->track_cap * K, (long long)t->arena_top[s] * K,
+                                              t->b_rstack[0].as<int>(), t->b_rn.as<int>(), t->stream);
+      if (e) return fail(SB200_ERR_CUDA, "feature row release launch failed: %s", cudaGetErrorString((cudaError_t)e));
+    }
+    if ((rc = t->read_rows())) return rc;
+  }
   for (int s : slots) { t->n_tracks[s] = 0; t->arena_top[s] = 0; t->epoch[s] = 0; }
   t->hpool_free += pushed;
   return 0;
diff --git a/similari_b200/csrc/kernels_cost.cu b/similari_b200/csrc/kernels_cost.cu
--- a/similari_b200/csrc/kernels_cost.cu
+++ b/similari_b200/csrc/kernels_cost.cu
@@ -11,6 +11,7 @@
 __global__ void prep_kernel(Params p, Frame f) {
   int i = blockIdx.x * blockDim.x + threadIdx.x;
   if (i >= f.total) return;
+  if (f.c_row) f.c_row[f.det0 + i] = f.row_stack[*f.row_n - 1 - i];
   i += f.det0;
   if (f.decided) f.decided[i] = 0;
   const float* b = f.in_boxes + (size_t)i * 6;
@@ -36,8 +37,10 @@
   int w = (blockIdx.x * blockDim.x + threadIdx.x) >> 5;
   int lane = threadIdx.x & 31;
   if (w >= f.total) return;
+  if (f.c_row && w == 0 && lane == 0) *f.row_n -= f.total;
   w += f.det0;
   const int nblk = p.d8 / 8;
+  float* prow = f.c_row ? f.row_pool + (size_t)f.c_row[w] * p.d8 : nullptr;
   const T* __restrict__ row = static_cast<const T*>(f.in_feat) + (size_t)w * p.feature_dim;
   constexpr bool kF32 = std::is_same<T, float>::value;
   const bool vec = (p.feature_dim % (kF32 ? 4 : 8) == 0) && (reinterpret_cast<uintptr_t>(f.in_feat) & 15) == 0;
@@ -79,6 +82,11 @@
 #pragma unroll
         for (int l = 0; l < 8; ++l) t[l] = x[h][l] * x[h][l];
         bs = reduce_add8(t);
+        if (prow) {
+          float4* o = reinterpret_cast<float4*>(prow + blk * 8);
+          o[0] = make_float4(x[h][0], x[h][1], x[h][2], x[h][3]);
+          o[1] = make_float4(x[h][4], x[h][5], x[h][6], x[h][7]);
+        }
         if (bf16_out) {
           __nv_bfloat162 hh[4];
 #pragma unroll
@@ -565,7 +573,7 @@
       int d = k0 + c;
       float v = 0.0f;
       int row = col_row[r];
-      if (row >= 0 && d < D8) v = ts.feat[(size_t)row * D8 + d];
+      if (row >= 0 && d < D8) v = feat_row(ts, row, D8)[d];
       sb_[r][c] = v;
     }
     __syncthreads();
diff --git a/similari_b200/csrc/kernels_feat_dense.cu b/similari_b200/csrc/kernels_feat_dense.cu
--- a/similari_b200/csrc/kernels_feat_dense.cu
+++ b/similari_b200/csrc/kernels_feat_dense.cu
@@ -492,7 +492,7 @@
   for (int pi = wid; pi < nq * nr; pi += 8) {
     const int g = s_q[pi / nr], fr = s_r[pi % nr];
     const T* a = static_cast<const T*>(f.in_feat) + (size_t)g * D;
-    const float* b = ts.feat + (size_t)fr * p.d8;
+    const float* b = feat_row(ts, fr, p.d8);
     float dot = 0.0f;
     for (int d = lane; d < D; d += 32) dot = __fmaf_rn(feat_elem(a, d), b[d], dot);
 #pragma unroll
diff --git a/similari_b200/csrc/kernels_feat_tc.cu b/similari_b200/csrc/kernels_feat_tc.cu
--- a/similari_b200/csrc/kernels_feat_tc.cu
+++ b/similari_b200/csrc/kernels_feat_tc.cu
@@ -554,6 +554,7 @@
     VisPair mine;
     mine.g = 0; mine.row = 0; mine.scene = 0; mine.outcol = 0;
     if (lane < npair) mine = f.vis_pairs[sc.vis_lbase + i0 + lane];
+    const float* mine_b = feat_row(ts, mine.row, p.d8);
     float acc = 0.0f;
     for (int seg0 = 0; seg0 < nblk; seg0 += RF_SEG) {
       const int segn = min(RF_SEG, nblk - seg0);
@@ -562,8 +563,8 @@
 #pragma unroll 4
       for (int pp = 0; pp < npair; ++pp) {
         const int g = __shfl_sync(0xffffffffu, mine.g, pp);
-        const int row = __shfl_sync(0xffffffffu, mine.row, pp);
-        const float* b = ts.feat + (size_t)row * p.d8;
+        const float* b = reinterpret_cast<const float*>(
+            __shfl_sync(0xffffffffu, reinterpret_cast<unsigned long long>(mine_b), pp));
         if (g != g_prev) {
           const T* a = static_cast<const T*>(f.in_feat) + (size_t)g * D;
 #pragma unroll
@@ -659,17 +660,18 @@
   note_launch();
 }
 
-__global__ void to_fp8_kernel(const float* src, int src_pitch, int d, int d8, long long rows, unsigned char* dst, float* scale) {
+__global__ void to_fp8_kernel(const float* src, int src_pitch, int d, int d8, long long rows, unsigned char* dst, float* scale,
+                              const int* map) {
   const long long r = ((long long)blockIdx.x * blockDim.x + threadIdx.x) >> 5;
   if (r >= rows) return;
-  const float s = fp8_row_from(src + r * src_pitch, d, d8, dst + r * fp8_pitch(d8));
+  const float s = fp8_row_from(src + (map ? map[r] : r) * src_pitch, d, d8, dst + r * fp8_pitch(d8));
   if ((threadIdx.x & 31) == 0) scale[r] = s;
 }
 
 void launch_to_fp8(const float* src, int src_pitch, int d, int d8, long long rows, unsigned char* dst, float* scale,
-                   cudaStream_t st) {
+                   cudaStream_t st, const int* map) {
   if (rows == 0) return;
-  to_fp8_kernel<<<(unsigned)((rows * 32 + 255) / 256), 256, 0, st>>>(src, src_pitch, d, d8, rows, dst, scale);
+  to_fp8_kernel<<<(unsigned)((rows * 32 + 255) / 256), 256, 0, st>>>(src, src_pitch, d, d8, rows, dst, scale, map);
   note_launch();
 }
 
diff --git a/similari_b200/csrc/kernels_state.cu b/similari_b200/csrc/kernels_state.cu
--- a/similari_b200/csrc/kernels_state.cu
+++ b/similari_b200/csrc/kernels_state.cu
@@ -343,148 +343,101 @@
   }
 }
 
-template <class T>
-__global__ void feat_store_kernel(Params p, TrackStore ts, Frame f) {
-  int w = (blockIdx.x * blockDim.x + threadIdx.x) >> 5;
-  int lane = threadIdx.x & 31;
-  if (w >= f.total) return;
-  if (lane == 0 && f.bf16_log) f.bf16_log[w] = f.feat_dst[f.det0 + w];
-  w += f.det0;
-  const int dst = f.feat_dst[w];
-  const int hdst = f.hist_dst ? f.hist_dst[w] : -1;
-  if (dst < 0 && hdst < 0) return;
-  const T* src = static_cast<const T*>(f.in_feat) + (size_t)w * p.feature_dim;
-  float* d = ts.feat + (size_t)max(dst, 0) * p.d8;
-  __nv_bfloat16* db = reinterpret_cast<__nv_bfloat16*>(ts.feat_bf16) + (size_t)max(dst, 0) * p.d8;
-  const bool wb = dst >= 0 && !f.skip_bf16;
-  float* hd = hdst >= 0 ? ts.hrows + (size_t)hdst * p.d8 : nullptr;
-  unsigned char* d8p = dst >= 0 && ts.feat_fp8 ? ts.feat_fp8 + (size_t)dst * fp8_pitch(p.d8) : nullptr;
-  if constexpr (!std::is_same<T, float>::value) {
-    if (p.feature_dim == p.d8 && (reinterpret_cast<uintptr_t>(f.in_feat) & 15) == 0) {
-      const uint4* s8 = reinterpret_cast<const uint4*>(src);
-      float4* d4 = reinterpret_cast<float4*>(d);
-      float4* h4 = reinterpret_cast<float4*>(hd);
-      uint4* b8 = reinterpret_cast<uint4*>(db);
-      const int n8 = p.d8 >> 3;
-      uint4 r[4];
-      for (int i0 = 0; i0 < n8; i0 += 128) {
-#pragma unroll
-        for (int u = 0; u < 4; ++u) {
-          const int i = i0 + u * 32 + lane;
-          if (i < n8) r[u] = __ldcs(s8 + i);
+constexpr int kLinkRows = 256;
+__global__ void __launch_bounds__(kLinkRows) feat_store_kernel(Params p, TrackStore ts, Frame f) {
+  __shared__ int s_dst[kLinkRows], s_hdst[kLinkRows], s_row[kLinkRows];
+  __shared__ int s_cnt, s_base;
+  const int t = threadIdx.x, lane = t & 31, warp = t >> 5;
+  const int i0 = blockIdx.x * kLinkRows;
+  if (t == 0) s_cnt = 0;
+  __syncthreads();
+  int freed = 0, slot = 0;
+  if (i0 + t < f.total) {
+    const int w = f.det0 + i0 + t;
+    const int dst = f.feat_dst[w], row = f.c_row[w];
+    if (f.bf16_log) f.bf16_log[i0 + t] = dst;
+    freed = row;
+    if (dst >= 0) {
+      freed = ts.obs_row[dst];
+      ts.obs_row[dst] = row;
+      ts.fnorm2[dst] = f.c_norm2[w];
+      if (ts.feat_fp8 && f.c_fp8) ts.fscale[dst] = f.c_scale[w];
+    }
+    if (freed != 0) slot = atomicAdd(&s_cnt, 1);
+    s_dst[t] = dst;
+    s_hdst[t] = f.hist_dst ? f.hist_dst[w] : -1;
+    s_row[t] = row;
+  } else {
+    s_dst[t] = -1;
+    s_hdst[t] = -1;
+  }
+  __syncthreads();
+  if (t == 0 && s_cnt > 0) s_base = atomicAdd(f.row_n, s_cnt);
+  __syncthreads();
+  if (freed != 0) f.row_stack[s_base + slot] = freed;
+  constexpr int kPerWarp = kLinkRows / 8, kBatch = 4;
+  const int d8 = p.d8, n8 = d8 >> 3, n4 = d8 >> 2;
+  if (ts.feat_fp8 && f.c_fp8) {
+    const int pitch = fp8_pitch(d8);
+    for (int j0 = 0; j0 < kPerWarp; j0 += kBatch) {
+      uint2 v[kBatch][2];
+#pragma unroll
+      for (int b = 0; b < kBatch; ++b) {
+        const int j = warp * kPerWarp + j0 + b;
+        if (s_dst[j] < 0) continue;
+        const uint2* c8 = reinterpret_cast<const uint2*>(f.c_fp8 + (size_t)(f.det0 + i0 + j) * pitch);
+#pragma unroll
+        for (int h = 0; h < 2; ++h)
+          if (h * 32 + lane < n8) v[b][h] = c8[h * 32 + lane];
+      }
+#pragma unroll
+      for (int b = 0; b < kBatch; ++b) {
+        const int j = warp * kPerWarp + j0 + b;
+        if (s_dst[j] < 0) continue;
+        uint2* d = reinterpret_cast<uint2*>(ts.feat_fp8 + (size_t)s_dst[j] * pitch);
+#pragma unroll
+        for (int h = 0; h < 2; ++h)
+          if (h * 32 + lane < n8) d[h * 32 + lane] = v[b][h];
+      }
+    }
+  }
+  for (int jj = 0; jj < kPerWarp; ++jj) {
+    const int j = warp * kPerWarp + jj;
+    const int dst = s_dst[j], hdst = s_hdst[j];
+    if (dst < 0 && hdst < 0) continue;
+    const int w = f.det0 + i0 + j;
+    const float* prow = ts.feat + (size_t)s_row[j] * d8;
+    const float4* s4 = reinterpret_cast<const float4*>(prow);
+    if (hdst >= 0) {
+      float4* h4 = reinterpret_cast<float4*>(ts.hrows + (size_t)hdst * d8);
+      for (int i = lane; i < n4; i += 32) __stcs(h4 + i, s4[i]);
+    }
+    if (dst < 0) continue;
+    if (ts.feat_fp8 && !f.c_fp8) {
+      const float s = fp8_row_from(prow, d8, d8, ts.feat_fp8 + (size_t)dst * fp8_pitch(d8));
+      if (lane == 0) ts.fscale[dst] = s;
+    }
+    if (!f.skip_bf16) {
+      if (f.c_bf16) {
+        const uint4* c = reinterpret_cast<const uint4*>(static_cast<const __nv_bfloat16*>(f.c_bf16) + (size_t)w * d8);
+        uint4* b = reinterpret_cast<uint4*>(reinterpret_cast<__nv_bfloat16*>(ts.feat_bf16) + (size_t)dst * d8);
+        for (int i = lane; i < n8; i += 32) b[i] = c[i];
+      } else {
+        uint2* b4 = reinterpret_cast<uint2*>(reinterpret_cast<__nv_bfloat16*>(ts.feat_bf16) + (size_t)dst * d8);
+        for (int i = lane; i < n4; i += 32) {
+          const float4 v = s4[i];
+          const __nv_bfloat162 lo = __floats2bfloat162_rn(v.x, v.y), hi = __floats2bfloat162_rn(v.z, v.w);
+          b4[i] = make_uint2(*reinterpret_cast<const unsigned int*>(&lo), *reinterpret_cast<const unsigned int*>(&hi));
         }
-#pragma unroll
-        for (int u = 0; u < 4; ++u) {
-          const int i = i0 + u * 32 + lane;
-          if (i < n8) {
-            float x[8];
-            feat_widen8(r[u], src, x);
-            const float4 lo = make_float4(x[0], x[1], x[2], x[3]), hi = make_float4(x[4], x[5], x[6], x[7]);
-            if (dst >= 0) {
-              d4[2 * i] = lo;
-              d4[2 * i + 1] = hi;
-            }
-            if (wb) {
-              __nv_bfloat162 bb[4];
-#pragma unroll
-              for (int l = 0; l < 4; ++l) bb[l] = __floats2bfloat162_rn(x[2 * l], x[2 * l + 1]);
-              b8[i] = *reinterpret_cast<const uint4*>(bb);
-            }
-            if (h4) { __stcs(h4 + 2 * i, lo); __stcs(h4 + 2 * i + 1, hi); }
-          }
-        }
-      }
-      if (d8p) {
-        float x[2][8];
-#pragma unroll
-        for (int h = 0; h < 2; ++h) {
-          if (h * 32 + lane < n8) feat_widen8(r[h], src, x[h]);
-          else
-#pragma unroll
-            for (int l = 0; l < 8; ++l) x[h][l] = 0.0f;
-        }
-        const float s = fp8_row_store(x, p.d8, d8p);
-        if (lane == 0) ts.fscale[dst] = s;
-      }
-    } else {
-      for (int i = lane; i < p.d8; i += 32) {
-        float x = i < p.feature_dim ? feat_elem(src, i) : 0.0f;
-        if (dst >= 0) d[i] = x;
-        if (wb) db[i] = __float2bfloat16_rn(x);
-        if (hd) hd[i] = x;
-      }
-      if (d8p) {
-        __syncwarp();
-        const float s = fp8_row_from(d, p.d8, p.d8, d8p);
-        if (lane == 0) ts.fscale[dst] = s;
-      }
-    }
-  } else if (p.feature_dim == p.d8 && (reinterpret_cast<uintptr_t>(f.in_feat) & 15) == 0) {
-    const float4* s4 = reinterpret_cast<const float4*>(src);
-    float4* d4 = reinterpret_cast<float4*>(d);
-    float4* h4 = reinterpret_cast<float4*>(hd);
-    uint2* b4 = reinterpret_cast<uint2*>(db);
-    const int n4 = p.d8 >> 2;
-    float4 v[4];
-    for (int i0 = 0; i0 < n4; i0 += 128) {
-#pragma unroll
-      for (int u = 0; u < 4; ++u) {
-        const int i = i0 + u * 32 + lane;
-        if (i < n4) v[u] = __ldcs(s4 + i);
-      }
-#pragma unroll
-      for (int u = 0; u < 4; ++u) {
-        const int i = i0 + u * 32 + lane;
-        if (i < n4) {
-          if (dst >= 0) d4[i] = v[u];
-          if (wb) {
-            const __nv_bfloat162 lo = __floats2bfloat162_rn(v[u].x, v[u].y), hi = __floats2bfloat162_rn(v[u].z, v[u].w);
-            uint2 pk;
-            pk.x = *reinterpret_cast<const unsigned int*>(&lo);
-            pk.y = *reinterpret_cast<const unsigned int*>(&hi);
-            b4[i] = pk;
-          }
-          if (h4) __stcs(h4 + i, v[u]);
-        }
-      }
-    }
-    if (d8p) {
-      float amax = 0.0f;
-#pragma unroll
-      for (int u = 0; u < 4; ++u)
-        if (u * 32 + lane < n4)
-          amax = fmaxf(amax, fmaxf(fmaxf(fabsf(v[u].x), fabsf(v[u].y)), fmaxf(fabsf(v[u].z), fabsf(v[u].w))));
-#pragma unroll
-      for (int o = 16; o > 0; o >>= 1) amax = fmaxf(amax, __shfl_xor_sync(0xffffffffu, amax, o));
-      const float s = fp8_row_scale(amax);
-      unsigned int* o4 = reinterpret_cast<unsigned int*>(d8p);
-#pragma unroll
-      for (int u = 0; u < 4; ++u) {
-        const int i = u * 32 + lane;
-        if (i < n4) o4[i] = fp8_pack4(v[u].x, v[u].y, v[u].z, v[u].w, s);
-      }
-      if (lane == 0) ts.fscale[dst] = s;
-    }
-  } else {
-    for (int i = lane; i < p.d8; i += 32) {
-      float x = i < p.feature_dim ? src[i] : 0.0f;
-      if (dst >= 0) d[i] = x;
-      if (wb) db[i] = __float2bfloat16_rn(x);
-      if (hd) hd[i] = x;
-    }
-    if (d8p) {
-      __syncwarp();
-      const float s = fp8_row_from(d, p.d8, p.d8, d8p);
-      if (lane == 0) ts.fscale[dst] = s;
-    }
-  }
-  if (lane == 0 && dst >= 0) ts.fnorm2[dst] = f.c_norm2[w];
+      }
+    }
+  }
 }
 
 __global__ void bf16_regen_kernel(TrackStore ts, int d8, int K, const int* __restrict__ rows, long long n, int n_slots) {
   const int lane = threadIdx.x & 31, wpb = blockDim.x >> 5;
   auto convert = [&](long long r) {
-    const float4* s4 = reinterpret_cast<const float4*>(ts.feat + (size_t)r * d8);
+    const float4* s4 = reinterpret_cast<const float4*>(feat_row(ts, r, d8));
     uint2* b4 = reinterpret_cast<uint2*>(reinterpret_cast<__nv_bfloat16*>(ts.feat_bf16) + (size_t)r * d8);
     for (int k = lane; k < (d8 >> 2); k += 32) {
       const float4 v = s4[k];
@@ -562,10 +515,7 @@
 
 bool launch_feat_store(const Params& p, const TrackStore& ts, const Frame& f, cudaStream_t st) {
   if (!(p.is_visual && f.in_feat && f.total > 0)) return false;
-  long long threads = (long long)f.total * 32;
-  feat_dispatch(f.feat_type, [&](auto t) {
-    feat_store_kernel<decltype(t)><<<(unsigned)((threads + 255) / 256), 256, 0, st>>>(p, ts, f);
-  });
+  feat_store_kernel<<<(unsigned)((f.total + kLinkRows - 1) / kLinkRows), kLinkRows, 0, st>>>(p, ts, f);
   note_launch();
   return true;
 }
diff --git a/similari_b200/csrc/kernels_xfer.cu b/similari_b200/csrc/kernels_xfer.cu
--- a/similari_b200/csrc/kernels_xfer.cu
+++ b/similari_b200/csrc/kernels_xfer.cu
@@ -146,4 +146,53 @@
   return (int)cudaGetLastError();
 }
 
+__global__ void xfer_feat_kernel(TrackStore ts, int d8, const long long* __restrict__ r0, const long long* __restrict__ pre,
+                                 int n, int dir, float* sec, const int* __restrict__ fresh) {
+  const int lane = threadIdx.x & 31;
+  const long long total = pre[n], ws = (long long)gridDim.x * (blockDim.x >> 5);
+  for (long long j = ((long long)blockIdx.x * blockDim.x + threadIdx.x) >> 5; j < total; j += ws) {
+    int lo = 0, hi = n - 1;
+    while (lo < hi) {
+      const int mid = (lo + hi + 1) >> 1;
+      if (pre[mid] <= j) lo = mid; else hi = mid - 1;
+    }
+    const long long r = r0[lo] + (j - pre[lo]);
+    float4* b = reinterpret_cast<float4*>(sec + (size_t)j * d8);
+    if (dir == 0) {
+      const float4* a = reinterpret_cast<const float4*>(feat_row(ts, r, d8));
+      for (int e = lane; e < (d8 >> 2); e += 32) b[e] = a[e];
+    } else {
+      const int row = fresh[j];
+      if (lane == 0) ts.obs_row[r] = row;
+      float4* a = reinterpret_cast<float4*>(ts.feat + (size_t)row * d8);
+      for (int e = lane; e < (d8 >> 2); e += 32) a[e] = b[e];
+    }
+  }
 }
+
+__global__ void free_feat_rows_kernel(int* obs_row, long long r0, long long rows, int* stack, int* count) {
+  for (long long i = (long long)blockIdx.x * blockDim.x + threadIdx.x; i < rows; i += (long long)gridDim.x * blockDim.x) {
+    const int row = obs_row[r0 + i];
+    obs_row[r0 + i] = 0;
+    if (row != 0) stack[atomicAdd(count, 1)] = row;
+  }
+}
+
+int launch_xfer_feat(const TrackStore& ts, int d8, const long long* d_r0, const long long* d_pre, int n, long long total,
+                     int dir, float* sec, const int* fresh, int num_sms, cudaStream_t st) {
+  if (n <= 0 || total <= 0) return 0;
+  const long long blocks = (total + 7) / 8;
+  xfer_feat_kernel<<<(unsigned)(blocks < num_sms * 8 ? blocks : num_sms * 8), 256, 0, st>>>(ts, d8, d_r0, d_pre, n, dir, sec, fresh);
+  note_launch();
+  return (int)cudaGetLastError();
+}
+
+int launch_free_feat_rows(int* obs_row, long long r0, long long rows, int* stack, int* count, cudaStream_t st) {
+  if (rows <= 0) return 0;
+  const long long blocks = (rows + 255) / 256;
+  free_feat_rows_kernel<<<(unsigned)(blocks < 1024 ? blocks : 1024), 256, 0, st>>>(obs_row, r0, rows, stack, count);
+  note_launch();
+  return (int)cudaGetLastError();
+}
+
+}
diff --git a/similari_b200/csrc/sb_engine.cuh b/similari_b200/csrc/sb_engine.cuh
--- a/similari_b200/csrc/sb_engine.cuh
+++ b/similari_b200/csrc/sb_engine.cuh
@@ -180,6 +180,7 @@
   float* hist_pred;
   float* hist_obs;
   float* feat;
+  int* obs_row;
   void* feat_bf16;
   unsigned char* feat_fp8;
   float* fscale;
@@ -204,6 +205,10 @@
 
 __device__ __forceinline__ size_t feat_block(const TrackStore& ts, int slot, size_t ti) {
   return ts.fblk ? (size_t)slot * ts.track_cap + (size_t)ts.fblk[ti] : ti;
+}
+
+__device__ __forceinline__ const float* feat_row(const TrackStore& ts, size_t r, int d8) {
+  return ts.feat + (size_t)(ts.obs_row ? ts.obs_row[r] : (long long)r) * d8;
 }
 
 constexpr int kFeatF32 = 0, kFeatF16 = 1, kFeatBF16 = 2;
@@ -260,6 +265,10 @@
   void* c_bf16;
   unsigned char* c_fp8;
   float* c_scale;
+  int* c_row;
+  float* row_pool;
+  int* row_stack;
+  int* row_n;
   int* screen_cnt;
   unsigned int* scene_max;
   int* winner;
@@ -399,7 +408,7 @@
 void launch_vis_densify(const Params& p, const Frame& f, int n_scenes, cudaStream_t st);
 void launch_to_bf16(const float* src, int src_pitch, int d, int d8, long long rows, void* dst, cudaStream_t st);
 void launch_to_fp8(const float* src, int src_pitch, int d, int d8, long long rows, unsigned char* dst, float* scale,
-                   cudaStream_t st);
+                   cudaStream_t st, const int* map = nullptr);
 constexpr int kFp8MaxD8 = 512;
 void launch_scene_max(const Params& p, const Frame& f, int n_scenes, bool init_only, cudaStream_t st);
 void launch_scene_mode(const Params& p, const Frame& f, int n_scenes, bool tc_used, cudaStream_t st);
@@ -439,6 +448,9 @@
                      cudaStream_t st);
 int launch_xfer_hist(const TrackStore& ts, int d8, const int* d_slots, const int* d_pre, int n, int total, int dir,
                      float* rows, unsigned char* pres, int base, int num_sms, cudaStream_t st);
+int launch_xfer_feat(const TrackStore& ts, int d8, const long long* d_r0, const long long* d_pre, int n, long long total,
+                     int dir, float* sec, const int* fresh, int num_sms, cudaStream_t st);
+int launch_free_feat_rows(int* obs_row, long long r0, long long rows, int* stack, int* count, cudaStream_t st);
 struct XferSlot { int slot, n_tracks, n_free, arena_top, push, push_off; };
 struct XferCheck { const void* p; const unsigned char* aux; long long n; int lo, hi, kind; };
 int launch_xfer_check(const XferCheck* d_ck, int n, int K, int* bad, cudaStream_t st);
```

Measured after the change: 61.40 billion (median of 6 runs). +1.5%, better.
